# osqp/osqp-python

Hardware: AMD Instinct MI355X
Metric: ADMM iterations/sec, n=100000 m=200000 nnz(A)=1000000 sparse QP (indirect PCG) (higher is better)
Workload: dtype f64

## Files before the change

### include/osqp_hip.h

```cpp
#ifndef OSQP_HIP_H
#define OSQP_HIP_H

#ifdef __cplusplus
extern "C" {
#endif

typedef int    OSQPInt;
typedef double OSQPFloat;

#define OSQP_INFTY ((OSQPFloat)1e30)

enum osqp_linsys_solver_type { OSQP_UNKNOWN_SOLVER = 0, OSQP_DIRECT_SOLVER, OSQP_INDIRECT_SOLVER };

enum osqp_status_type {
  OSQP_SOLVED = 1, OSQP_SOLVED_INACCURATE, OSQP_PRIMAL_INFEASIBLE, OSQP_PRIMAL_INFEASIBLE_INACCURATE,
  OSQP_DUAL_INFEASIBLE, OSQP_DUAL_INFEASIBLE_INACCURATE, OSQP_MAX_ITER_REACHED, OSQP_TIME_LIMIT_REACHED,
  OSQP_NON_CVX, OSQP_SIGINT, OSQP_UNSOLVED
};

enum osqp_error_type {
  OSQP_NO_ERROR = 0, OSQP_DATA_VALIDATION_ERROR, OSQP_SETTINGS_VALIDATION_ERROR, OSQP_LINSYS_SOLVER_INIT_ERROR,
  OSQP_NONCVX_ERROR, OSQP_MEM_ALLOC_ERROR, OSQP_WORKSPACE_NOT_INIT_ERROR, OSQP_ALGEBRA_LOAD_ERROR,
  OSQP_CODEGEN_DEFINES_ERROR, OSQP_DATA_NOT_INITIALIZED, OSQP_FUNC_NOT_IMPLEMENTED
};

enum osqp_precond_type { OSQP_NO_PRECONDITIONER = 0, OSQP_DIAGONAL_PRECONDITIONER };

enum osqp_capabilities_type {
  OSQP_CAPABILITY_DIRECT_SOLVER = 0x01, OSQP_CAPABILITY_INDIRECT_SOLVER = 0x02, OSQP_CAPABILITY_CODEGEN = 0x04,
  OSQP_CAPABILITY_UPDATE_MATRICES = 0x08, OSQP_CAPABILITY_DERIVATIVES = 0x10
};

typedef struct {
  OSQPInt    m;
  OSQPInt    n;
  OSQPInt   *p;
  OSQPInt   *i;
  OSQPFloat *x;
  OSQPInt    nzmax;
  OSQPInt    nz;
} OSQPCscMatrix;

typedef struct {
  OSQPInt device;
  enum osqp_linsys_solver_type linsys_solver;
  OSQPInt verbose;
  OSQPInt warm_starting;
  OSQPInt scaling;
  OSQPInt polishing;
  OSQPFloat rho;
  OSQPInt   rho_is_vec;
  OSQPFloat sigma;
  OSQPFloat alpha;
  OSQPInt   cg_max_iter;
  OSQPInt   cg_tol_reduction;
  OSQPFloat cg_tol_fraction;
  enum osqp_precond_type cg_precond;
  OSQPInt   adaptive_rho;
  OSQPInt   adaptive_rho_interval;
  OSQPFloat adaptive_rho_fraction;
  OSQPFloat adaptive_rho_tolerance;
  OSQPInt   max_iter;
  OSQPFloat eps_abs;
  OSQPFloat eps_rel;
  OSQPFloat eps_prim_inf;
  OSQPFloat eps_dual_inf;
  OSQPInt   scaled_termination;
  OSQPInt   check_termination;
  OSQPInt   check_dualgap;
  OSQPFloat time_limit;
  OSQPFloat delta;
  OSQPInt   polish_refine_iter;
} OSQPSettings;

typedef struct {
  char      status[32];
  OSQPInt   status_val;
  OSQPInt   status_polish;
  OSQPFloat obj_val;
  OSQPFloat dual_obj_val;
  OSQPFloat prim_res;
  OSQPFloat dual_res;
  OSQPFloat duality_gap;
  OSQPInt   iter;
  OSQPInt   rho_updates;
  OSQPFloat rho_estimate;
  OSQPFloat setup_time;
  OSQPFloat solve_time;
  OSQPFloat update_time;
  OSQPFloat polish_time;
  OSQPFloat run_time;
  OSQPFloat primdual_int;
  OSQPFloat rel_kkt_error;
} OSQPInfo;

typedef struct {
  OSQPFloat *x;
  OSQPFloat *y;
  OSQPFloat *prim_inf_cert;
  OSQPFloat *dual_inf_cert;
} OSQPSolution;

typedef struct OSQPWorkspace_ OSQPWorkspace;

typedef struct {
  OSQPSettings  *settings;
  OSQPSolution  *solution;
  OSQPInfo      *info;
  OSQPWorkspace *work;
} OSQPSolver;

typedef struct {
  OSQPInt embedded_mode, float_type, printing_enable, profiling_enable, interrupt_enable, derivatives_enable;
} OSQPCodegenDefines;

OSQPInt osqp_capabilities(void);
void    osqp_set_default_settings(OSQPSettings *settings);
const char *osqp_version(void);

OSQPInt osqp_setup(OSQPSolver **solverp, const OSQPCscMatrix *P, const OSQPFloat *q, const OSQPCscMatrix *A,
                   const OSQPFloat *l, const OSQPFloat *u, OSQPInt m, OSQPInt n, const OSQPSettings *settings);
OSQPInt osqp_solve(OSQPSolver *solver);
OSQPInt osqp_cleanup(OSQPSolver *solver);
OSQPInt osqp_warm_start(OSQPSolver *solver, const OSQPFloat *x, const OSQPFloat *y);
OSQPInt osqp_cold_start(OSQPSolver *solver);
OSQPInt osqp_update_data_vec(OSQPSolver *solver, const OSQPFloat *q_new, const OSQPFloat *l_new,
                             const OSQPFloat *u_new);
OSQPInt osqp_update_data_mat(OSQPSolver *solver, const OSQPFloat *Px_new, const OSQPInt *Px_new_idx, OSQPInt P_new_n,
                             const OSQPFloat *Ax_new, const OSQPInt *Ax_new_idx, OSQPInt A_new_n);
OSQPInt osqp_update_settings(OSQPSolver *solver, const OSQPSettings *new_settings);
OSQPInt osqp_update_rho(OSQPSolver *solver, OSQPFloat rho_new);
void    osqp_get_dimensions(OSQPSolver *solver, OSQPInt *m, OSQPInt *n);

OSQPInt osqp_adjoint_derivative_compute(OSQPSolver *solver, OSQPFloat *dx, OSQPFloat *dy);
OSQPInt osqp_adjoint_derivative_get_mat(OSQPSolver *solver, OSQPCscMatrix *dP, OSQPCscMatrix *dA);
OSQPInt osqp_adjoint_derivative_get_vec(OSQPSolver *solver, OSQPFloat *dq, OSQPFloat *dl, OSQPFloat *du);
OSQPInt osqp_codegen(OSQPSolver *solver, const char *output_dir, const char *prefix, OSQPCodegenDefines *defines);
void    osqp_set_default_codegen_defines(OSQPCodegenDefines *defines);


typedef struct {
  double pcg_iters_total;
  double pcg_iters_max;
  double pcg_unconverged;
  double kernel_launches;
  double graph_launches;
  double gpu_solve_ms;
  double nnzA, nnzB;
  double pcg_fused;
  double batch_direct_bw;
  double cg_cap_escalations;
  double windowed_blocks;
  double row_blocks;
  double slot_topups;
  double f1_replicas;
  double woodbury_rows;
  double woodbury_direct;
  double preconditioner;
  double woodbury_factorisations, woodbury_factor_ms;
  double reordered;
  double reorder_ms;
  double woodbury_cache_hits;
  double f1_far_columns;
  double woodbury_dual_cols;
  double woodbury_fused_iteration;
  double woodbury_one_launch;
  double kform_nnz;
  double batch_wave_split;
} OSQPHipStats;
enum { OSQP_HIP_PRECOND_NONE = 0, OSQP_HIP_PRECOND_JACOBI = 1, OSQP_HIP_PRECOND_JACOBI_WOODBURY = 2, OSQP_HIP_PRECOND_JACOBI_WOODBURY_DENSE = 3 };
OSQPInt osqp_hip_get_stats(OSQPSolver *solver, OSQPHipStats *out);

OSQPInt osqp_hip_time_kernel(OSQPSolver *solver, OSQPInt which, OSQPInt reps, double *mean_ms);

#define OSQP_HIP_BATCH_REC 12
OSQPInt osqp_hip_batch_solve(OSQPSolver *solver, OSQPInt nbatch, const OSQPFloat *q, const OSQPFloat *l, const OSQPFloat *u,
                             OSQPFloat *x, OSQPFloat *y, OSQPFloat *rec, OSQPInt warm);
OSQPInt osqp_hip_batch_solve_device(OSQPSolver *solver, OSQPInt nbatch, const OSQPFloat *q_dev, const OSQPFloat *l_dev, const OSQPFloat *u_dev,
                                    OSQPFloat *x_dev, OSQPFloat *y_dev, OSQPFloat *rec_dev, OSQPInt warm_start, void *stream);

OSQPInt osqp_hip_batch_solve_mat(OSQPSolver *solver, OSQPInt nbatch, const OSQPFloat *Px, const OSQPFloat *Ax, const OSQPFloat *q, const OSQPFloat *l,
                                 const OSQPFloat *u, OSQPFloat *x, OSQPFloat *y, OSQPFloat *rec, OSQPInt warm);
OSQPInt osqp_hip_batch_solve_mat_device(OSQPSolver *solver, OSQPInt nbatch, const OSQPFloat *Px_dev, const OSQPFloat *Ax_dev, const OSQPFloat *q_dev,
                                        const OSQPFloat *l_dev, const OSQPFloat *u_dev, OSQPFloat *x_dev, OSQPFloat *y_dev, OSQPFloat *rec_dev,
                                        OSQPInt warm_start, void *stream);

#define OSQP_HIP_LOCKSTEP_WIDTH 64
#define OSQP_HIP_LOCKSTEP_LAST_REC 8
#define OSQP_HIP_LOCKSTEP_POLISH_LAST_REC 8
OSQPInt osqp_hip_batch_solve_lockstep(OSQPSolver *solver, OSQPInt nbatch, const OSQPFloat *q, const OSQPFloat *l, const OSQPFloat *u,
                                      OSQPFloat *x, OSQPFloat *y, OSQPFloat *rec, OSQPInt warm);
OSQPInt osqp_hip_batch_solve_lockstep_device(OSQPSolver *solver, OSQPInt nbatch, const OSQPFloat *q_dev, const OSQPFloat *l_dev, const OSQPFloat *u_dev,
                                             OSQPFloat *x_dev, OSQPFloat *y_dev, OSQPFloat *rec_dev, OSQPInt warm_start, void *stream);
OSQPInt osqp_hip_lockstep_last_record(OSQPSolver *solver, OSQPFloat *rec);
OSQPInt osqp_hip_lockstep_polish_last_record(OSQPSolver *solver, OSQPFloat *rec);
#define OSQP_HIP_LOCKSTEP_MAT_LAST_REC 8
OSQPInt osqp_hip_batch_solve_lockstep_mat(OSQPSolver *solver, OSQPInt nbatch, const OSQPFloat *Px, const OSQPFloat *Ax, const OSQPFloat *q, const OSQPFloat *l,
                                          const OSQPFloat *u, OSQPFloat *x, OSQPFloat *y, OSQPFloat *rec, OSQPInt warm);
OSQPInt osqp_hip_batch_solve_lockstep_mat_device(OSQPSolver *solver, OSQPInt nbatch, const OSQPFloat *Px_dev, const OSQPFloat *Ax_dev, const OSQPFloat *q_dev,
                                                 const OSQPFloat *l_dev, const OSQPFloat *u_dev, OSQPFloat *x_dev, OSQPFloat *y_dev, OSQPFloat *rec_dev,
                                                 OSQPInt warm_start, void *stream);
OSQPInt osqp_hip_lockstep_mat_last_record(OSQPSolver *solver, OSQPFloat *rec);
OSQPInt osqp_hip_lockstep_mat_scaling(OSQPSolver *solver, OSQPInt b, OSQPFloat *D, OSQPFloat *E, OSQPFloat *c);
#define OSQP_HIP_LOCKSTEP_DIRECT_LAST_REC 8
OSQPInt osqp_hip_batch_solve_lockstep_direct(OSQPSolver *solver, OSQPInt nbatch, const OSQPFloat *q, const OSQPFloat *l, const OSQPFloat *u,
                                             OSQPFloat *x, OSQPFloat *y, OSQPFloat *rec, OSQPInt warm);
OSQPInt osqp_hip_batch_solve_lockstep_direct_device(OSQPSolver *solver, OSQPInt nbatch, const OSQPFloat *q_dev, const OSQPFloat *l_dev, const OSQPFloat *u_dev,
                                                    OSQPFloat *x_dev, OSQPFloat *y_dev, OSQPFloat *rec_dev, OSQPInt warm_start, void *stream);
OSQPInt osqp_hip_lockstep_direct_last_record(OSQPSolver *solver, OSQPFloat *rec);
#define OSQP_HIP_LOCKSTEP_ADJOINT_LAST_REC 8
OSQPInt osqp_hip_batch_adjoint_lockstep(OSQPSolver *solver, OSQPInt nbatch, const OSQPFloat *l, const OSQPFloat *u, const OSQPFloat *x, const OSQPFloat *y,
                                        const OSQPFloat *dx, const OSQPFloat *dy, OSQPFloat *dP, OSQPFloat *dq, OSQPFloat *dA, OSQPFloat *dl, OSQPFloat *du,
                                        OSQPFloat *arec);
OSQPInt osqp_hip_batch_adjoint_lockstep_device(OSQPSolver *solver, OSQPInt nbatch, const OSQPFloat *l_dev, const OSQPFloat *u_dev, const OSQPFloat *x_dev,
                                               const OSQPFloat *y_dev, const OSQPFloat *dx_dev, const OSQPFloat *dy_dev, OSQPFloat *dP_dev, OSQPFloat *dq_dev,
                                               OSQPFloat *dA_dev, OSQPFloat *dl_dev, OSQPFloat *du_dev, OSQPFloat *arec_dev, void *stream);
OSQPInt osqp_hip_lockstep_adjoint_last_record(OSQPSolver *solver, OSQPFloat *rec);
#define OSQP_HIP_LOCKSTEP_DIRECT_ADJOINT_LAST_REC 8
OSQPInt osqp_hip_batch_adjoint_lockstep_direct(OSQPSolver *solver, OSQPInt nbatch, const OSQPFloat *l, const OSQPFloat *u, const OSQPFloat *x, const OSQPFloat *y,
                                               const OSQPFloat *dx, const OSQPFloat *dy, OSQPFloat *dP, OSQPFloat *dq, OSQPFloat *dA, OSQPFloat *dl, OSQPFloat *du,
                                               OSQPFloat *arec);
OSQPInt osqp_hip_batch_adjoint_lockstep_direct_device(OSQPSolver *solver, OSQPInt nbatch, const OSQPFloat *l_dev, const OSQPFloat *u_dev, const OSQPFloat *x_dev,
                                                      const OSQPFloat *y_dev, const OSQPFloat *dx_dev, const OSQPFloat *dy_dev, OSQPFloat *dP_dev, OSQPFloat *dq_dev,
                                                      OSQPFloat *dA_dev, OSQPFloat *dl_dev, OSQPFloat *du_dev, OSQPFloat *arec_dev, void *stream);
OSQPInt osqp_hip_lockstep_direct_adjoint_last_record(OSQPSolver *solver, OSQPFloat *rec);

#define OSQP_HIP_ADJOINT_REC 4
#define OSQP_HIP_ADJOINT_TOL 1e-6
OSQPInt osqp_hip_batch_adjoint(OSQPSolver *solver, OSQPInt nbatch, const OSQPFloat *Px, const OSQPFloat *Ax, const OSQPFloat *l, const OSQPFloat *u,
                               const OSQPFloat *x, const OSQPFloat *y, const OSQPFloat *dx, const OSQPFloat *dy, OSQPFloat *dP, OSQPFloat *dq,
                               OSQPFloat *dA, OSQPFloat *dl, OSQPFloat *du, OSQPFloat *arec);
OSQPInt osqp_hip_batch_adjoint_device(OSQPSolver *solver, OSQPInt nbatch, const OSQPFloat *Px_dev, const OSQPFloat *Ax_dev, const OSQPFloat *l_dev,
                                      const OSQPFloat *u_dev, const OSQPFloat *x_dev, const OSQPFloat *y_dev, const OSQPFloat *dx_dev,
                                      const OSQPFloat *dy_dev, OSQPFloat *dP_dev, OSQPFloat *dq_dev, OSQPFloat *dA_dev, OSQPFloat *dl_dev,
                                      OSQPFloat *du_dev, OSQPFloat *arec_dev, void *stream);
#define OSQP_HIP_ADJOINT_LAST_REC 8
OSQPInt osqp_hip_adjoint_compute_at(OSQPSolver *solver, const OSQPFloat *x, const OSQPFloat *y, const OSQPFloat *dx, const OSQPFloat *dy);
OSQPInt osqp_hip_adjoint_last_record(OSQPSolver *solver, OSQPFloat *rec);
OSQPInt osqp_hip_capabilities(void);

OSQPInt osqp_hip_update_data_vec_device(OSQPSolver *solver, const OSQPFloat *q_dev, const OSQPFloat *l_dev, const OSQPFloat *u_dev, void *stream);
OSQPInt osqp_hip_warm_start_device(OSQPSolver *solver, const OSQPFloat *x_dev, const OSQPFloat *y_dev, void *stream);


typedef struct OSQPHipLinSysSolver_ OSQPHipLinSysSolver;
struct OSQPHipLinSysSolver_ {
  enum osqp_linsys_solver_type type;
  const char *(*name)(OSQPHipLinSysSolver *self);
  OSQPInt (*solve)(OSQPHipLinSysSolver *self, OSQPFloat *b, OSQPInt admm_iter);
  void (*update_settings)(OSQPHipLinSysSolver *self, const OSQPSettings *settings);
  void (*warm_start)(OSQPHipLinSysSolver *self, const OSQPFloat *x);
  OSQPInt (*adjoint_derivative)(OSQPHipLinSysSolver *self);
  void (*free)(OSQPHipLinSysSolver *self);
  OSQPInt (*update_matrices)(OSQPHipLinSysSolver *self, const OSQPCscMatrix *P, const OSQPInt *Px_new_idx, OSQPInt P_new_n,
                             const OSQPCscMatrix *A, const OSQPInt *Ax_new_idx, OSQPInt A_new_n);
  OSQPInt (*update_rho_vec)(OSQPHipLinSysSolver *self, const OSQPFloat *rho_vec, OSQPFloat rho_sc);
  OSQPInt nthreads;
  OSQPInt pcg_iters;
  void *impl;
};
OSQPInt osqp_hip_linsys_init(OSQPHipLinSysSolver **self, const OSQPCscMatrix *P, const OSQPCscMatrix *A, const OSQPFloat *rho_vec,
                             const OSQPSettings *settings, const OSQPFloat *scaled_prim_res, const OSQPFloat *scaled_dual_res,
                             OSQPInt polishing);

typedef struct {
  OSQPInt graph;
  OSQPInt slots;
  OSQPInt pcg_fused;
  OSQPInt f1;
  OSQPInt window;
  OSQPInt woodbury;
  OSQPInt woodbury_direct;
  OSQPInt woodbury_large;
  OSQPInt device_driven;
  OSQPInt small_direct;
  OSQPInt batch_reorder;
  OSQPInt batch_variant;
  OSQPFloat extrap;
  OSQPFloat rho_eq_factor;
  OSQPInt rho_window;
  OSQPFloat rho_window_tol;
  OSQPInt rho_persist;
  OSQPFloat rho_tol_exp;
  OSQPFloat budget_tolerate, budget_sigma; OSQPInt budget_slack, budget_full;
  OSQPInt cg_escalate;
  OSQPInt stall;
  OSQPFloat polish_delta_floor;
  OSQPFloat polish_pcg_tol;
  OSQPInt slot_poll; OSQPInt poll_low; OSQPFloat poll_first, poll_frac, poll_wait;
  OSQPInt finish_pairs; OSQPInt poll_sleep_us;
  OSQPInt slot_log, setup_timing, batch_timing, woodbury_log;
  OSQPFloat woodbury_direct_tol;
  OSQPInt woodbury_fused;
  OSQPInt debug_fail_refactor;
  OSQPInt reorder;
  OSQPInt woodbury_cache;
  OSQPInt kform;
  OSQPInt woodbury_dual;
  OSQPInt woodbury_vendor;
  OSQPInt batch_wave;
} OSQPHipPolicy;
void    osqp_hip_default_policy(OSQPHipPolicy *policy);
OSQPInt osqp_hip_set_policy(OSQPSolver *solver, const OSQPHipPolicy *policy);
OSQPInt osqp_hip_get_policy(OSQPSolver *solver, OSQPHipPolicy *policy);
void    osqp_hip_set_default_policy(const OSQPHipPolicy *policy);

OSQPInt osqp_hip_trace_read(OSQPSolver *solver, unsigned long long *out, OSQPInt count);
OSQPInt osqp_hip_test_spmv(OSQPSolver *solver, OSQPInt which, const OSQPFloat *in, OSQPFloat *out);
typedef struct {
  OSQPInt op, M, N, K;
  OSQPFloat alpha, beta;
  long long as_i, as_k, bs_k, bs_j, cs_i, cs_j;
  long long a_off, b_off, c_off;
  long long a_len, b_len, c_len;
  const OSQPFloat *A, *B;
  OSQPFloat *C;
  OSQPFloat minpiv;
} OSQPHipDenseTest;
OSQPInt osqp_hip_test_dense(OSQPSolver *solver, OSQPHipDenseTest *t);
OSQPInt osqp_hip_set_rho_eq_factor(OSQPSolver *solver, OSQPFloat factor);
OSQPInt osqp_hip_get_scaling(OSQPSolver *solver, OSQPFloat *D, OSQPFloat *E, OSQPFloat *c);
OSQPInt osqp_hip_get_reordering(OSQPSolver *solver, OSQPInt *perm_cols, OSQPInt *perm_rows);
typedef void (*osqp_hip_print_fn)(const char *text, void *user);
void    osqp_hip_set_default_print(osqp_hip_print_fn fn, void *user);
OSQPInt osqp_hip_set_print(OSQPSolver *solver, osqp_hip_print_fn fn, void *user);
const char *osqp_hip_backend(void);

#ifdef __cplusplus
}
#endif
#endif
```

### osqp-python_amd/csrc/backend.h

```cpp
#pragma once
#include <cstddef>
#include <cstdint>
#include <stdexcept>

#include "band_ldl.h"

namespace osqp_hip {

struct DeviceError : std::runtime_error { using std::runtime_error::runtime_error; };

#ifndef OSQP_HIP_KBLOCK
#define OSQP_HIP_KBLOCK 256
#define OSQP_HIP_KGRID 1024
#endif
constexpr int kBlock = OSQP_HIP_KBLOCK;
constexpr int kGrid = OSQP_HIP_KGRID;
constexpr int kChunk = 8 * kBlock;
constexpr int kLongRow = 128;
constexpr int kMaxRowsPerBlock = 1024;
constexpr int kPartSlots = 40;
constexpr int kMaxCg = 1024;
constexpr int kWinCap = 1472;
constexpr int kF1Win = 512;
constexpr int kF1MaxD = 4;
// ... 256 lines not shown
  const double *x = nullptr, *y = nullptr, *dx = nullptr, *dy = nullptr;
  int *code = nullptr;
  double *rx = nullptr, *ry = nullptr;
  double *dP = nullptr, *dA = nullptr, *dl = nullptr, *du = nullptr;
  double *rec = nullptr;
  double c = 1.0, cinv = 1.0;
  int rho_is_vec = 1;
};

constexpr int kLsW = 64;
constexpr int kLsSlots = 32;
constexpr int kLsScal = 16, kLsInt = 12;
inline int lockstep_grid(int n, int m) { const int r = n > m ? n : m, g = (r + 15) / 16; return g < 1 ? 1 : (g > 256 ? 256 : g); }
inline size_t lockstep_ws_doubles(int n, int m) {
  return (size_t)kLsW * (8 * (size_t)n + 9 * (size_t)m + (size_t)kLsSlots * lockstep_grid(n, m) + (size_t)(m + 63) / 64 + 1 + kLsScal + kBatchRec + kLsInt) + 64;
}
struct LockstepParams : BatchSettings {
  int n = 0, m = 0, count = 0;
  DevCsr A, B;
  const double *D = nullptr, *Dinv = nullptr, *E = nullptr, *Einv = nullptr;
  double time_limit = 0;
  const double *q = nullptr, *l = nullptr, *u = nullptr;
  const double *q0 = nullptr, *l0 = nullptr, *u0 = nullptr;
  double *x = nullptr, *y = nullptr, *rec = nullptr;
  const int *pc = nullptr, *pr = nullptr;
  double *ws = nullptr;
  double pcg_rel = 0;
  double rho_tol_single = 0; int rho_persist = 0;
  int polish = 0, pol_min_steps = 1, pol_cg_max = 0;
  double pol_rho = 0, pol_pcg_rel = 0;
  double *pol_ws = nullptr, *pol_stat = nullptr;
  double *mat_ws = nullptr, *mat_stat = nullptr;
  const double *Px = nullptr, *Ax = nullptr;
  const int *pvmap = nullptr, *avmap = nullptr;
  int mat_iters = 0;
};
constexpr int kLsPolStat = 7;
constexpr int kLsMatStat = 2;
constexpr int kLsMatScalC = 11;
inline size_t lockstep_sc_offset(int n, int m) {
  const size_t tm = (size_t)(m + 63) / 64;
  return (size_t)kLsW * (8 * (size_t)n + 9 * (size_t)m + (size_t)kLsSlots * lockstep_grid(n, m) + (tm > 0 ? tm : 1));
}
inline size_t lockstep_mat_ws_doubles(int n, int m, int nzA, int nzB) { return (size_t)kLsW * ((size_t)nzA + (size_t)nzB + 2 * (size_t)n + 2 * (size_t)m) + 64; }
inline size_t lockstep_polish_ws_doubles(int n, int m) { return (size_t)kLsW * ((size_t)n + 4 * (size_t)m) + 64; }

struct LockstepAdjointParams : LockstepParams {
  int nzP = 0, nzA = 0;
  const int *Pi = nullptr, *Pj = nullptr, *Ai = nullptr, *Aj = nullptr;
  const int *Pmap = nullptr, *Amap = nullptr;
  const double *sx = nullptr, *sy = nullptr, *gx = nullptr, *gy = nullptr;
  double *dP = nullptr, *dq = nullptr, *dA = nullptr, *dl = nullptr, *du = nullptr, *arec = nullptr;
  int min_steps = 1, max_steps = 60; double gain = 0.9;
};
inline size_t lockstep_adjoint_ws_doubles(int n, int m) {
  return lockstep_ws_doubles(n, m) + (size_t)kLsW * (3 * (size_t)n + 3 * (size_t)m + ((size_t)m + 1) / 2) + 64;
}

struct LockstepDirectParams : LockstepParams {
  int r = 0;
  DevCsr Av;
  const double *WT = nullptr; const int *rows = nullptr; const unsigned char *islong = nullptr;
};
inline int lockstep_direct_colblock(int n) { const int t = (n + 63) / 64; return 64 * ((t + 127) / 128 > 0 ? (t + 127) / 128 : 1); }
inline size_t lockstep_direct_ws_doubles(int n, int m, int r) {
  const size_t gc = ((size_t)n + lockstep_direct_colblock(n) - 1) / lockstep_direct_colblock(n);
  return (size_t)kLsW * (3 * ((size_t)n + r) + 4 * (size_t)n + 9 * (size_t)m + (size_t)kLsSlots * lockstep_grid(n, m) + (size_t)(m + 63) / 64 + 1 + kLsScal + kBatchRec + kLsInt +
                         (size_t)r * r + 2 * gc * r + r + 1) + 64;
}

struct LockstepDirectAdjointParams : LockstepAdjointParams {
  int r = 0;
  DevCsr Av;
  const double *WT = nullptr; const int *rows = nullptr; const unsigned char *islong = nullptr;
};
inline size_t lockstep_direct_adjoint_ws_doubles(int n, int m, int r) {
  return lockstep_direct_ws_doubles(n, m, r) + (size_t)kLsW * (3 * (size_t)n + 3 * (size_t)m + ((size_t)m + 1) / 2) + 64;
}

namespace be {

int lockstep_direct_chunk(Dev &d, const LockstepDirectParams &p, void *stream, double *stat) __attribute__((weak));
int lockstep_direct_values(Dev &d, int nv, const int *src, double *out, void *stream) __attribute__((weak));
int lockstep_direct_adjoint_chunk(Dev &d, const LockstepDirectAdjointParams &p, void *stream, double *stat) __attribute__((weak));

int lockstep_chunk(Dev &d, const LockstepParams &p, void *stream, double *stat) __attribute__((weak));
int lockstep_adjoint_chunk(Dev &d, const LockstepAdjointParams &p, void *stream, double *stat) __attribute__((weak));

void adjoint_load(Dev &d, const AdjointPcg &a) __attribute__((weak));
void adjoint_residual(Dev &d, const AdjointPcg &a) __attribute__((weak));
void adjoint_gradients(Dev &d, const AdjointPcg &a) __attribute__((weak));

int batch_adjoint(Dev &d, const AdjointParams &p, void *stream) __attribute__((weak));
size_t batch_lds_bytes(int n, int m);
int batch_solve(Dev &d, const BatchParams &p, void *stream = nullptr);
size_t batch_direct_lds_bytes(int n, int m, int nnz, int bw);
bool batch_direct_selected(const BatchParams &p);
void batch_release(Dev &d);
size_t batch_wave_lds_bytes(int n, int m, int steps);
void batch_products(Dev &d, int nprod, const int *a, const int *b, double *out);
int batch_prepare(Dev &d, const BatchParams &p, const double *Px_b, const double *Ax_b, int scaling_iters, void *stream);
void batch_order(Dev &d, int nbatch, const int *iters, int *order, void *stream);

const char *name();
int init(Dev &d, int device);
void destroy(Dev &d);
void *alloc(Dev &d, size_t bytes);
void dfree(Dev &d, void *p);
void h2d(Dev &d, void *dst, const void *src, size_t bytes);
void d2h(Dev &d, void *dst, const void *src, size_t bytes);
void zero(Dev &d, void *dst, size_t bytes);
void sync(Dev &d);
void ev_mark(Dev &d, int which);
double ev_ms(Dev &d);
void activate(Dev &d);
void ext_record(Dev &d, void *stream);
void ext_wait(Dev &d);

void kb_rhs(Dev &d);
void k1(Dev &d, int i);
void k2(Dev &d, int i);
void kv(Dev &d, int i);
void ka(Dev &d, int budget);
bool slots_supported(const Dev &d);
void slot_begin(Dev &d, int target, int cap);
void slot_pair(Dev &d);
int slot_done(Dev &d);
int slot_seq(Dev &d);
inline double slot_launches(const Dev &d, double pcg) { return (d.wb.on && d.wb.exact && d.wb.x.on && d.wb.x.slots) ? 2.16 : (d.f1.on ? pcg + 2.0 : (d.kf.on ? pcg + 3.0 : 2.0 * (pcg + 2.0))); }
bool kf_supported();
void kf_values(Dev &d, int cond = 0);
void f1_refresh(Dev &d);
bool wb_supported();
bool wbx_supported();
void wbx_init(Dev &d);
void wbx_refresh(Dev &d);
void wbx_factor(Dev &d, int cond = 0);
void wbx_slot_pair(Dev &d);
inline bool wbx_active(const Dev &d) { return d.wb.on && d.wb.exact && d.wb.x.on; }
inline bool wbx_slots(const Dev &d) { return wbx_active(d) && d.wb.x.slots; }
void wbx_chunk(Dev &d, int niter);
bool wb_large_supported();
void wb_refresh(Dev &d);
void wb_direct(Dev &d);
inline bool wbf_active(const Dev &d) { return d.wb.on && d.wb.exact && d.wb.dual && d.wb.fused; }
void wbf_iteration(Dev &d);
void wb_apply(Dev &d, int parity, int direct = 0);
bool ctl_supported(const Dev &d);
void ctl_upload(Dev &d, const Ctl &c);
void ctl_begin(Dev &d);
void ctl_group(Dev &d, int diagonal);
void ctl_poll(Dev &d, Ctl *out, int *seq, int *done);
void ctl_download(Dev &d, Ctl *out);
constexpr int kSlotInts = 24;
void slot_poll(Dev &d, int *seq, int *done);

void residuals(Dev &d);
void infeas_primal(Dev &d);
void infeas_dual(Dev &d, double thr, int unscaled);
void fetch_res(Dev &d, double *host_res);
void fetch_flags(Dev &d, int *host_flags);
void fetch_res_flags(Dev &d, double *host_res, int *host_flags);

void set_rho(Dev &d, double rho_bar);
void precond(Dev &d, int diagonal);
void set_pcg_tol(Dev &d, double tol_rel, double tol_abs);

void init_iterates(Dev &d, int full);

void project_normalcone(Dev &d);

bool pcg_fused(const Dev &d);

bool graphs_supported();
void graph_begin(Dev &d);
void *graph_end(Dev &d);
void graph_launch(Dev &d, void *g);
void graph_free(Dev &d, void *g);

bool device_assembly();
void assemble(Dev &d, int scaled, double c, int with_sigma);
double ruiz(Dev &d, int iters);

bool device_vec_updates();
void copy_in(Dev &d, void *dst, const void *src, size_t bytes, int src_on_device);
void stream_wait(Dev &d, void *caller_stream);
void gather(Dev &d, double *dst_dev, const double *src_dev, const int *idx_dev, int cnt);
void scale_q(Dev &d, double c);
void scale_bounds(Dev &d, int rho_is_vec);
int count_bad_bounds(Dev &d, const double *l_dev, const double *u_dev);
void scale_warm(Dev &d, const double *x_dev, const double *y_dev, double c);

bool ktrace_read(Dev &d, unsigned long long *out, int count);
void test_spmv(Dev &d, int which, const double *in_dev, double *out_dev);
struct DenseProbe { int op, M, N, K; double alpha, beta; long as_i, as_k, bs_k, bs_j, cs_i, cs_j; const double *A, *B; double *C; };
double test_dense(Dev &d, const DenseProbe &p) __attribute__((weak));
float time_kernel(Dev &d, int which, int reps);

}
}
```

### osqp-python_amd/csrc/backend_hip.hip

```cpp
#include "hip_common.h"

namespace osqp_hip {
namespace be {

namespace {

struct EKr1 : NoPrefetch {
  const double *z, *y, *dy, *l, *u, *E, *Einv;
  double pu = 0, au = 0, zu = 0, ps = 0, as = 0, zs = 0, du = 0, ds = 0, lhs = 0, sup = 0;
  __device__ __forceinline__ void operator()(int i, const double (&s)[1]) {
    const double ax = s[0], zi = z[i], pr = ax - zi, ei = Einv[i], dyi = dy[i], yi = y[i], li = l[i], ui = u[i];
    pu = nanmax(pu, fabs(ei * pr)); au = nanmax(au, fabs(ei * ax)); zu = nanmax(zu, fabs(ei * zi));
    ps = nanmax(ps, fabs(pr)); as = nanmax(as, fabs(ax)); zs = nanmax(zs, fabs(zi));
    du = nanmax(du, fabs(E[i] * dyi)); ds = nanmax(ds, fabs(dyi));
    lhs += support_term(li, ui, dyi);
    sup += support_finite(li, ui, yi);
  }
};
__device__ __forceinline__ bool ctl_res_due(const Dev &d) { return d.ctl->chunk_done && d.ctl->ch_at_check && d.ctl->status == CTL_RUNNING; }
__global__ __launch_bounds__(kBlock) void k_res_m(Dev d, int cond) {
  __shared__ StreamLdsW<1, double> lds;
  if (cond && !ctl_res_due(d)) return;
  GVec g{d.x};
  EKr1 e{{}, d.z, d.y, d.dy, d.l, d.u, d.E, d.Einv};
  process_rows<1>(d.A, g, e, lds);
  __syncthreads();
  double *red = lds.red;
  put_partial(d.part, SL_RES0 + R_PRI_U, block_max(e.pu, red)); put_partial(d.part, SL_RES0 + R_AX_U, block_max(e.au, red));
  put_partial(d.part, SL_RES0 + R_Z_U, block_max(e.zu, red)); put_partial(d.part, SL_RES0 + R_PRI_S, block_max(e.ps, red));
  put_partial(d.part, SL_RES0 + R_AX_S, block_max(e.as, red)); put_partial(d.part, SL_RES0 + R_Z_S, block_max(e.zs, red));
  put_partial(d.part, SL_RES0 + R_DY_U, block_max(e.du, red)); put_partial(d.part, SL_RES0 + R_DY_S, block_max(e.ds, red));
  put_partial(d.part, SL_RES0 + R_PINF_LHS, block_sum(e.lhs, red)); put_partial(d.part, SL_RES0 + R_SUPP, block_sum(e.sup, red));
}

struct GTwo {
  const double *pn, *pm; int n;
  __device__ __forceinline__ void operator()(int c, double a, double (&pr)[2]) const {
    if (c < n) { pr[0] = a * pn[c]; pr[1] = 0.0; } else { pr[0] = 0.0; pr[1] = a * pm[c - n]; }
  }
};
struct EKr2 : NoPrefetch {
  const double *x, *q, *dx, *D, *Dinv; double sigma;
  double du = 0, pu = 0, au = 0, ds = 0, ps = 0, as = 0, xu = 0, xs = 0, xpx = 0, qx = 0, qdx = 0, qns = 0, qnu = 0;
  __device__ __forceinline__ void operator()(int j, const double (&s)[2]) {
    const double xj = x[j], px = s[0] - sigma * xj, aty = s[1], qj = q[j], dr = px + qj + aty, di = Dinv[j], dxj = dx[j];
    qns = nanmax(qns, fabs(qj)); qnu = nanmax(qnu, fabs(di * qj));
    du = nanmax(du, fabs(di * dr)); pu = nanmax(pu, fabs(di * px)); au = nanmax(au, fabs(di * aty));
    ds = nanmax(ds, fabs(dr)); ps = nanmax(ps, fabs(px)); as = nanmax(as, fabs(aty));
    xu = nanmax(xu, fabs(D[j] * dxj)); xs = nanmax(xs, fabs(dxj));
    xpx += xj * px; qx += qj * xj; qdx += qj * dxj;
  }
};
__global__ __launch_bounds__(kBlock) void k_res_n(Dev d, int cond) {
  __shared__ StreamLds<2> lds;
  if (cond && !ctl_res_due(d)) return;
  GTwo g{d.x, d.y, d.n};
  EKr2 e{{}, d.x, d.q, d.dx, d.D, d.Dinv, d.sigma};
  process_rows<2>(d.B, g, e, lds);
  __syncthreads();
  double *red = lds.red;
  put_partial(d.part, SL_RES0 + R_DUA_U, block_max(e.du, red)); put_partial(d.part, SL_RES0 + R_PX_U, block_max(e.pu, red));
  put_partial(d.part, SL_RES0 + R_ATY_U, block_max(e.au, red)); put_partial(d.part, SL_RES0 + R_DUA_S, block_max(e.ds, red));
  put_partial(d.part, SL_RES0 + R_PX_S, block_max(e.ps, red)); put_partial(d.part, SL_RES0 + R_ATY_S, block_max(e.as, red));
  put_partial(d.part, SL_RES0 + R_DX_U, block_max(e.xu, red)); put_partial(d.part, SL_RES0 + R_DX_S, block_max(e.xs, red));
  put_partial(d.part, SL_RES0 + R_XPX, block_sum(e.xpx, red)); put_partial(d.part, SL_RES0 + R_QX, block_sum(e.qx, red));
  put_partial(d.part, SL_RES0 + R_QDX, block_sum(e.qdx, red));
  put_partial(d.part, SL_RES0 + R_QN_S, block_max(e.qns, red)); put_partial(d.part, SL_RES0 + R_QN_U, block_max(e.qnu, red));
}

__device__ __forceinline__ bool res_is_sum(int q) {
  return q == R_PINF_LHS || q == R_SUPP || q == R_XPX || q == R_QX || q == R_QDX || q == R_ADX_VIOL;
}
__device__ __forceinline__ bool ctl_stage2_due(const Dev &d, int bits) { return d.ctl->status == CTL_RUNNING && (d.ctl->stage2 & bits) != 0; }
__global__ __launch_bounds__(kBlock) void k_res_final(Dev d, int q0, int cond) {
  __shared__ double sred[2 * kWaves];
  if (cond == 1 && !ctl_res_due(d)) return;
  if (cond == 2 && !ctl_stage2_due(d, NEED_PINF | NEED_DINF)) return;
  const int q = q0 + blockIdx.x;
  const double *slot = d.part + (SL_RES0 + q) * kGrid;
  const double v = res_is_sum(q) ? partial_sum(slot, sred) : partial_max(slot, sred);
  if (threadIdx.x == 0) d.res[q] = v;
}

struct GAtOnly { const double *pm; int n; __device__ __forceinline__ void operator()(int c, double a, double (&pr)[1]) const { pr[0] = c >= n ? a * pm[c - n] : 0.0; } };
struct GPOnly { const double *pn; int n; __device__ __forceinline__ void operator()(int c, double a, double (&pr)[1]) const { pr[0] = c < n ? a * pn[c] : 0.0; } };
struct EAbs2 : NoPrefetch {
  const double *scale, *sub; double sigma; double mu = 0, ms = 0;
  __device__ __forceinline__ void operator()(int j, const double (&s)[1]) {
    const double v = s[0] - (sub ? sigma * sub[j] : 0.0);
    mu = nanmax(mu, fabs(scale[j] * v)); ms = nanmax(ms, fabs(v));
  }
};
__global__ __launch_bounds__(kBlock) void k_inf_primal(Dev d, int cond) {
  __shared__ StreamLds<1> lds;
  if (cond && !ctl_stage2_due(d, NEED_PINF)) return;
  GAtOnly g{d.dy, d.n};
  EAbs2 e{{}, d.Dinv, nullptr, 0.0};
  process_rows<1>(d.B, g, e, lds);
  __syncthreads();
  put_partial(d.part, SL_RES0 + R_ATDY_U, block_max(e.mu, lds.red)); put_partial(d.part, SL_RES0 + R_ATDY_S, block_max(e.ms, lds.red));
}
__global__ __launch_bounds__(kBlock) void k_inf_dual_p(Dev d, int cond) {
  __shared__ StreamLds<1> lds;
  if (cond && !ctl_stage2_due(d, NEED_DINF)) return;
  GPOnly g{d.dx, d.n};
  EAbs2 e{{}, d.Dinv, d.dx, d.sigma};
  process_rows<1>(d.B, g, e, lds);
  __syncthreads();
  put_partial(d.part, SL_RES0 + R_PDX_U, block_max(e.mu, lds.red)); put_partial(d.part, SL_RES0 + R_PDX_S, block_max(e.ms, lds.red));
}
struct EViol : NoPrefetch {
  const double *l, *u, *Einv; double thr; int unscaled; double viol = 0;
  __device__ __forceinline__ void operator()(int i, const double (&s)[1]) {
    const double a = unscaled ? Einv[i] * s[0] : s[0];
    if (adx_violates(a, l[i], u[i], thr)) viol += 1.0;
  }
};
__global__ __launch_bounds__(kBlock) void k_inf_dual_a(Dev d, double thr, int unscaled, int cond) {
  __shared__ StreamLdsW<1, double> lds;
  if (cond) { if (!ctl_stage2_due(d, NEED_DINF)) return; thr = d.ctl->inf_thr_d; unscaled = d.ctl->inf_unscaled; }
  GVec g{d.dx};
  EViol e{{}, d.l, d.u, d.Einv, thr, unscaled};
  process_rows<1>(d.A, g, e, lds);
  __syncthreads();
  put_partial(d.part, SL_RES0 + R_ADX_VIOL, block_sum(e.viol, lds.red));
}

__global__ __launch_bounds__(kBlock) void k_set_rho(Dev d, double rho_bar, int cond) {
  if (cond) { if (!d.ctl->rho_flag) return; rho_bar = d.ctl->rho_bar; }
  const int stride = gridDim.x * kBlock;
  for (int i = blockIdx.x * kBlock + threadIdx.x; i < d.m; i += stride) {
    const int t = d.ctype[i];
    const double eqf = d.eq_from_cnt ? eq_weight(d.cnt[0] == 0, d.rho_eq_mixed) : d.rho_eq_factor;
    const double r = row_rho(t, rho_bar, eqf * rho_bar);
    d.rho[i] = r; d.rho_inv[i] = 1.0 / r;
    d.v[i] = r * d.z[i] - d.y[i]; d.ztg[i] = d.zt[i]; d.t0[i] = r * d.zt[i];
  }
}
struct GPrec { const double *rho; int n; __device__ __forceinline__ void operator()(int c, double a, double (&pr)[1]) const { pr[0] = c >= n ? rho[c - n] * a * a : 0.0; } };
__global__ __launch_bounds__(kBlock) void k_precond(Dev d, int cond) {
  __shared__ StreamLds<1> lds;
  if (cond && !d.ctl->rho_flag) return;
  GPrec g{d.rho, d.n};
  EPrec e{{}, d.B.val, d.Bdiag, d.Minv};
  process_rows<1>(d.B, g, e, lds);
}
__global__ __launch_bounds__(kBlock) void k_fill(double *p, int n, double v) {
  const int stride = gridDim.x * kBlock;
  for (int i = blockIdx.x * kBlock + threadIdx.x; i < n; i += stride) p[i] = v;
}
__global__ __launch_bounds__(kBlock) void k_init_n(Dev d) {
  const int stride = gridDim.x * kBlock;
  for (int j = blockIdx.x * kBlock + threadIdx.x; j < d.n; j += stride) { d.xs[j] = d.x[j]; d.dx[j] = 0.0; }
// ... 13 lines not shown
};
__global__ __launch_bounds__(kBlock) void k_init_m(Dev d, int full) {
  __shared__ StreamLdsW<1, double> lds;
  GVec g{d.xs};
  EInit e{{}, d.rho, d.y, d.z, d.zt, d.t0, d.v, d.dy, full, d.ztg};
  process_rows<1>(d.A, g, e, lds);
}
__global__ __launch_bounds__(kBlock) void k_normalcone(Dev d) {
  const int stride = gridDim.x * kBlock;
  for (int i = blockIdx.x * kBlock + threadIdx.x; i < d.m; i += stride) {
    const ConeRow c = normal_cone(d.z[i] + d.y[i], d.l[i], d.u[i]);
    d.z[i] = c.z; d.y[i] = c.y;
  }
}
__global__ void k_set_scal(double *scal, double rel, double ab) { scal[S_TOL_REL] = rel; scal[S_TOL_ABS] = ab; }
__global__ __launch_bounds__(kBlock) void k_scale_q(Dev d, double c) {
  for (int j = blockIdx.x * kBlock + threadIdx.x; j < d.n; j += gridDim.x * kBlock) d.q[j] = c * d.D[j] * d.qraw[j];
}
__global__ __launch_bounds__(kBlock) void k_scale_bounds(Dev d, int rho_is_vec) {
  int ineq = 0;
  for (int i = blockIdx.x * kBlock + threadIdx.x; i < d.m; i += gridDim.x * kBlock) {
    const double ls = d.E[i] * d.lraw[i], us = d.E[i] * d.uraw[i];
    d.l[i] = ls; d.u[i] = us;
    const int t = row_class(ls, us, rho_is_vec);
    d.ctype[i] = t;
    ineq += (t == 0);
  }
  for (int o = 32; o > 0; o >>= 1) ineq += __shfl_down(ineq, o, 64);
  if ((threadIdx.x & 63) == 0 && ineq) atomicAdd(&d.cnt[0], ineq);
}
__global__ __launch_bounds__(kBlock) void k_count_bad(int m, const double *l, const double *u, int *cnt) {
  int bad = 0;
  for (int i = blockIdx.x * kBlock + threadIdx.x; i < m; i += gridDim.x * kBlock) bad += !(l[i] <= u[i]);
  for (int o = 32; o > 0; o >>= 1) bad += __shfl_down(bad, o, 64);
  if ((threadIdx.x & 63) == 0 && bad) atomicAdd(&cnt[1], bad);
}
__global__ __launch_bounds__(kBlock) void k_gather(double *dst, const double *src, const int *idx, int cnt) {
  for (int k = blockIdx.x * kBlock + threadIdx.x; k < cnt; k += gridDim.x * kBlock) dst[k] = src[idx[k]];
}
__global__ __launch_bounds__(kBlock) void k_scale_warm(Dev d, const double *xin, const double *yin, double c) {
  const int stride = gridDim.x * kBlock;
  if (xin) for (int j = blockIdx.x * kBlock + threadIdx.x; j < d.n; j += stride) d.x[j] = d.Dinv[j] * xin[j];
  if (yin) for (int i = blockIdx.x * kBlock + threadIdx.x; i < d.m; i += stride) d.y[i] = c * d.Einv[i] * yin[i];
}



__device__ __forceinline__ double limit_scaling_dev(double v) { return v < 1e-4 ? 1.0 : (v > 1e4 ? 1e4 : v); }
__global__ __launch_bounds__(kBlock) void k_asm_diag(Dev d, double sigma) {
  for (int j = blockIdx.x * kBlock + threadIdx.x; j < d.n; j += gridDim.x * kBlock) d.B.val[d.Bdiag[j]] = sigma;
}
__global__ __launch_bounds__(kBlock) void k_asm_scatter(Dev d, int scaled, double c, double sigma) {
  const int stride = gridDim.x * kBlock;
  for (int k = blockIdx.x * kBlock + threadIdx.x; k < d.nzA; k += stride) {
    double v = d.Araw[k];
    if (scaled) v *= d.E[d.Ai[k]] * d.D[d.Aj[k]];
    d.A.val[d.AmA[k]] = v; d.B.val[d.AmB[k]] = v;
  }
  for (int k = blockIdx.x * kBlock + threadIdx.x; k < d.nzP; k += stride) {
    const int i = d.Pi[k], j = d.Pj[k];
    double v = d.Praw[k];
    if (scaled) v *= c * d.D[i] * d.D[j];
    if (i == j) atomicAdd(&d.B.val[d.Pm1[k]], v);
    else { d.B.val[d.Pm1[k]] = v; d.B.val[d.Pm2[k]] = v; }
  }
}
template <class F>
__device__ __forceinline__ void for_long_rows(const DevCsr &M, F &&f) {
  const int4 *desc = reinterpret_cast<const int4 *>(M.blkdesc);
  for (int b = blockIdx.x; b < M.nblk; b += gridDim.x) { const int4 ds = desc[b]; if (ds.y < 0) f(ds.x, ds.z, ds.w); }
}
__global__ __launch_bounds__(kBlock) void k_rowmax(DevCsr M, int climit, double *out) {
  __shared__ double sred[2 * kWaves];
  for (int r = blockIdx.x * kBlock + threadIdx.x; r < M.nrows; r += gridDim.x * kBlock) {
    const int k0 = M.rowptr[r], k1 = M.rowptr[r + 1];
    if (k1 - k0 > kLongRow) continue;
    double mx = 0.0;
    for (int k = k0; k < k1; k++) if (M.col[k] < climit) mx = fmax(mx, fabs(M.val[k]));
    out[r] = mx;
  }
  for_long_rows(M, [&](int r, int k0, int k1) {
    double mx = 0.0;
    for (int k = k0 + threadIdx.x; k < k1; k += kBlock) if (M.col[k] < climit) mx = fmax(mx, fabs(M.val[k]));
    mx = block_max(mx, sred);
    if (threadIdx.x == 0) out[r] = mx;
  });
}
__global__ __launch_bounds__(kBlock) void k_ruiz_delta(double *v, int cnt) {
  for (int i = blockIdx.x * kBlock + threadIdx.x; i < cnt; i += gridDim.x * kBlock) v[i] = 1.0 / sqrt(limit_scaling_dev(v[i]));
}
__global__ __launch_bounds__(kBlock) void k_ruiz_scale_A(Dev d, const double *dt, const double *et) {
  for (int i = blockIdx.x * kBlock + threadIdx.x; i < d.m; i += gridDim.x * kBlock) {
    const double ei = et[i];
    const int k0 = d.A.rowptr[i], k1 = d.A.rowptr[i + 1];
    if (k1 - k0 <= kLongRow) for (int k = k0; k < k1; k++) d.A.val[k] *= ei * dt[d.A.col[k]];
    d.E[i] *= ei;
  }
  for_long_rows(d.A, [&](int i, int k0, int k1) {
    const double ei = et[i];
    for (int k = k0 + threadIdx.x; k < k1; k += kBlock) d.A.val[k] *= ei * dt[d.A.col[k]];
  });
}
__global__ __launch_bounds__(kBlock) void k_ruiz_scale_B(Dev d, const double *dt, const double *et) {
  for (int j = blockIdx.x * kBlock + threadIdx.x; j < d.n; j += gridDim.x * kBlock) {
    const double dj = dt[j];
    const int k0 = d.B.rowptr[j], k1 = d.B.rowptr[j + 1];
    if (k1 - k0 <= kLongRow)
      for (int k = k0; k < k1; k++) {
        const int c = d.B.col[k];
        d.B.val[k] *= c < d.n ? dt[c] * dj : et[c - d.n] * dj;
      }
    d.q[j] *= dj; d.D[j] *= dj;
  }
  for_long_rows(d.B, [&](int j, int k0, int k1) {
    const double dj = dt[j];
    for (int k = k0 + threadIdx.x; k < k1; k += kBlock) { const int c = d.B.col[k]; d.B.val[k] *= c < d.n ? dt[c] * dj : et[c - d.n] * dj; }
  });
}
__global__ __launch_bounds__(kBlock) void k_ruiz_cost(Dev d, const double *np) {
  __shared__ double sred[2 * kWaves];
  double sum = 0.0, nq = 0.0;
  for (int j = threadIdx.x; j < d.n; j += kBlock) { sum += np[j]; nq = fmax(nq, fabs(d.q[j])); }
  block_sum_max(sum, nq, sred);
  if (threadIdx.x == 0) {
    const double mean = sum / (double)(d.n > 0 ? d.n : 1);
    const double ct = 1.0 / limit_scaling_dev(fmax(limit_scaling_dev(nq), mean));
    d.cs[1] = ct; d.cs[0] *= ct;
  }
}
__global__ __launch_bounds__(kBlock) void k_ruiz_cost_apply(Dev d) {
  const double ct = d.cs[1];
  for (int j = blockIdx.x * kBlock + threadIdx.x; j < d.n; j += gridDim.x * kBlock) {
    for (int k = d.B.rowptr[j]; k < d.B.rowptr[j + 1] && d.B.col[k] < d.n; k++) d.B.val[k] *= ct;
    d.q[j] *= ct;
  }
}
__global__ __launch_bounds__(kBlock) void k_ruiz_finish(Dev d, double sigma) {
  const int stride = gridDim.x * kBlock;
  for (int j = blockIdx.x * kBlock + threadIdx.x; j < d.n; j += stride) { d.Dinv[j] = 1.0 / d.D[j]; d.B.val[d.Bdiag[j]] += sigma; }
  for (int i = blockIdx.x * kBlock + threadIdx.x; i < d.m; i += stride) d.Einv[i] = 1.0 / d.E[i];
}

__device__ __forceinline__ void ctl_begin_chunk(const Dev &d, const Ctl &c, int seq) {
  int *r = d.slot;
  r[SR_PHASE] = P_KB; r[SR_K] = 0; r[SR_ADMM] = 0; r[SR_TARGET] = c.ch_next - c.iter; r[SR_USED] = 0; r[SR_CONV] = 0;
  r[SR_CAP] = c.budget[c.ch_tight]; r[SR_SEQ] = seq;
  r[SR_WORDS + SR_SEQ] = seq - 1; r[SR_WORDS + SR_ADMM] = 0;
  d.scal[S_TOL_REL] = c.tol_rel; d.scal[S_TOL_ABS] = ctl_chunk_tol_abs(c);
  for (int q = F_STAT_SUM; q < F_COUNT; q++) d.flags[q] = 0;
}
__global__ void k_ctl_begin(Dev d, int epoch) {
  Ctl &c = *d.ctl;
  c.chunk_done = 0; c.rho_flag = 0; c.stage2 = 0; c.status = CTL_RUNNING; c.seq_begin = 0;
  ctl_begin_chunk(d, c, 0);
  d.slot[2 * SR_WORDS] = epoch;
}
__global__ __launch_bounds__(64) void k_decide(Dev d, int stage) {
  __shared__ Ctl c;
  __shared__ double res[R_COUNT];
  __shared__ int fl[F_COUNT];
  Ctl *g = d.ctl;
  if (g->status != CTL_RUNNING) return;
  if (stage == 1 ? !g->chunk_done : !g->stage2) {
    if (stage == 1 && threadIdx.x == 0) g->rho_flag = 0;
    return;
  }
  static_assert(sizeof(Ctl) % sizeof(int) == 0, "Ctl is copied word by word");
  constexpr int W = sizeof(Ctl) / sizeof(int);
  const int *gi = reinterpret_cast<const int *>(g);
  int *ci = reinterpret_cast<int *>(&c);
  for (int i = threadIdx.x; i < W; i += 64) ci[i] = gi[i];
  for (int i = threadIdx.x; i < R_COUNT; i += 64) res[i] = d.res[i];
  for (int i = threadIdx.x; i < F_COUNT; i += 64) fl[i] = d.flags[i];
  __syncthreads();
  if (threadIdx.x == 0) {
    int st;
    if (stage == 1) {
      c.chunk_done = 0;
      if (c.boundaries >= 0 && c.boundaries < kCtlHist) c.hist[c.boundaries] = c.seq_end - c.seq_begin;
      for (int q = 0; q < F_COUNT; q++) c.last_flags[q] = fl[q];
      st = ctl_boundary(c, res, fl);
    } else st = ctl_boundary_stage2(c, res, c.last_flags);
    c.status = st;
    if (st == CTL_RUNNING && !c.stage2) { c.seq_begin = d.slot[SR_SEQ]; ctl_begin_chunk(d, c, d.slot[SR_SEQ]); }
  }
  __syncthreads();
  int *go = reinterpret_cast<int *>(g);
  for (int i = threadIdx.x; i < W; i += 64) go[i] = ci[i];
}


}

const char *name() { return "hip-gfx950"; }

int init(Dev &d, int device) {
  int count = 0;
  if (hipGetDeviceCount(&count) != hipSuccess || count <= 0) {
    std::fprintf(stderr, "osqp_hip: no HIP device available -- this engine has no CPU fallback\n");
    return OSQP_ALGEBRA_LOAD_ERROR;
  }
  if (device >= count) return OSQP_SETTINGS_VALIDATION_ERROR;
  d.device = device;
  HIP_CHECK(hipSetDevice(device));
  hipStream_t s;
  HIP_CHECK(hipStreamCreateWithFlags(&s, hipStreamNonBlocking));
  d.stream = s;
  Impl *p = new Impl();
  HIP_CHECK(hipEventCreate(&p->ev0)); HIP_CHECK(hipEventCreate(&p->ev1)); HIP_CHECK(hipEventCreate(&p->ev_s0)); HIP_CHECK(hipEventCreate(&p->ev_s1)); HIP_CHECK(hipEventCreateWithFlags(&p->ev_ext, hipEventDisableTiming)); HIP_CHECK(hipEventCreateWithFlags(&p->ev_wait, hipEventDisableTiming));
  HIP_CHECK(hipHostMalloc(reinterpret_cast<void **>(&p->pin_res), sizeof(double) * R_COUNT, hipHostMallocDefault));
  HIP_CHECK(hipHostMalloc(reinterpret_cast<void **>(&p->pin_flags), sizeof(int) * (F_COUNT + 16), hipHostMallocDefault));
  HIP_CHECK(hipHostMalloc(reinterpret_cast<void **>(&p->pin_poll), sizeof(int) * kSlotInts, hipHostMallocDefault));
  HIP_CHECK(hipStreamCreateWithFlags(&p->side, hipStreamNonBlocking));
  HIP_CHECK(hipHostMalloc(reinterpret_cast<void **>(&p->pin_ctl), sizeof(Ctl), hipHostMallocDefault));
  HIP_CHECK(hipHostMalloc(reinterpret_cast<void **>(&p->pin_ctl2), sizeof(Ctl), hipHostMallocDefault));
  d.impl = p;
  return OSQP_NO_ERROR;
}
void destroy(Dev &d) {
  if (!d.impl) return;
  (void)hipSetDevice(d.device);
  Impl &p = im(d);
  (void)hipEventDestroy(p.ev0); (void)hipEventDestroy(p.ev1); (void)hipEventDestroy(p.ev_s0); (void)hipEventDestroy(p.ev_s1); (void)hipEventDestroy(p.ev_ext); (void)hipEventDestroy(p.ev_wait); (void)hipHostFree(p.pin_res); (void)hipHostFree(p.pin_flags);
  (void)hipHostFree(p.pin_poll); if (p.side) (void)hipStreamDestroy(p.side);
  (void)hipHostFree(p.pin_ctl); (void)hipHostFree(p.pin_ctl2);
  if (p.blas) wb_release_blas(p.blas);
  batch_release(d);
  for (int k = 1; k < DevWb::kCache; k++) if (d.wb.cache_buf[k]) { (void)hipFree(d.wb.cache_buf[k]); d.wb.cache_buf[k] = nullptr; }
  dev_release(d);
  delete &p; d.impl = nullptr;
  if (d.stream) { (void)hipStreamDestroy(st(d)); d.stream = nullptr; }
}
void *alloc(Dev &d, size_t bytes) {
  HIP_CHECK(hipSetDevice(d.device));
  void *p = nullptr;
  HIP_CHECK(hipMalloc(&p, bytes));
  HIP_CHECK(hipMemsetAsync(p, 0, bytes, st(d)));
  return p;
}
void dfree(Dev &d, void *p) { (void)hipSetDevice(d.device); (void)hipFree(p); }
void h2d(Dev &d, void *dst, const void *src, size_t b) {
  if (!b) return;
  HIP_CHECK(hipSetDevice(d.device));
  HIP_CHECK(hipMemcpyAsync(dst, src, b, hipMemcpyHostToDevice, st(d)));
  HIP_CHECK(hipStreamSynchronize(st(d)));
}
void d2h(Dev &d, void *dst, const void *src, size_t b) {
  if (!b) return;
  HIP_CHECK(hipSetDevice(d.device));
  HIP_CHECK(hipMemcpyAsync(dst, src, b, hipMemcpyDeviceToHost, st(d)));
  HIP_CHECK(hipStreamSynchronize(st(d)));
}
void zero(Dev &d, void *dst, size_t b) { if (!b) return; HIP_CHECK(hipSetDevice(d.device)); HIP_CHECK(hipMemsetAsync(dst, 0, b, st(d))); }
void sync(Dev &d) { HIP_CHECK(hipSetDevice(d.device)); HIP_CHECK(hipStreamSynchronize(st(d))); }
void ev_mark(Dev &d, int which) { HIP_CHECK(hipSetDevice(d.device)); Impl &p = im(d); HIP_CHECK(hipEventRecord(which ? p.ev_s1 : p.ev_s0, st(d))); }
double ev_ms(Dev &d) { Impl &p = im(d); float ms = 0.f; HIP_CHECK(hipEventSynchronize(p.ev_s1)); HIP_CHECK(hipEventElapsedTime(&ms, p.ev_s0, p.ev_s1)); return (double)ms; }
void activate(Dev &d) { HIP_CHECK(hipSetDevice(d.device)); }
void ext_record(Dev &d, void *stream) {
  if (!stream || !d.impl) return;
  HIP_CHECK(hipSetDevice(d.device));
  HIP_CHECK(hipEventRecord(im(d).ev_ext, static_cast<hipStream_t>(stream)));
  im(d).ext_pending = true;
}
void ext_wait(Dev &d) {
  if (!d.impl || !im(d).ext_pending) return;
  HIP_CHECK(hipSetDevice(d.device));
  HIP_CHECK(hipEventSynchronize(im(d).ev_ext));
  im(d).ext_pending = false;
}

bool ctl_supported(const Dev &d) { return d.ctl != nullptr && d.slot != nullptr; }
void ctl_upload(Dev &d, const Ctl &c) {
  HIP_CHECK(hipSetDevice(d.device));
  Impl &p = im(d);
  std::memcpy(p.pin_ctl, &c, sizeof(Ctl));
  HIP_CHECK(hipMemcpyAsync(d.ctl, p.pin_ctl, sizeof(Ctl), hipMemcpyHostToDevice, st(d)));
  HIP_CHECK(hipStreamSynchronize(st(d)));
}
void ctl_begin(Dev &d) { HIP_CHECK(hipSetDevice(d.device)); dev_publish(d); hipLaunchKernelGGL(k_ctl_begin, dim3(1), dim3(1), 0, st(d), d, ++im(d).epoch); }
void ctl_group(Dev &d, int diagonal) {
  LAUNCH(k_res_m, d, d, 1);
  LAUNCH(k_res_n, d, d, 1);
  hipLaunchKernelGGL(k_res_final, dim3(R_QN_U + 1), dim3(kBlock), 0, st(d), d, 0, 1);
  hipLaunchKernelGGL(k_decide, dim3(1), dim3(64), 0, st(d), d, 1);
  LAUNCH(k_inf_primal, d, d, 1);
  LAUNCH(k_inf_dual_p, d, d, 1);
  LAUNCH(k_inf_dual_a, d, d, 0.0, 0, 1);
  hipLaunchKernelGGL(k_res_final, dim3(5), dim3(kBlock), 0, st(d), d, (int)R_ATDY_U, 2);
  hipLaunchKernelGGL(k_decide, dim3(1), dim3(64), 0, st(d), d, 2);
  LAUNCH(k_set_rho, d, d, 0.0, 1);
  LAUNCH(k_init_guess, d, d, 1);
  if (diagonal) LAUNCH(k_precond, d, d, 1);
  kf_values(d, 1);
  if (wbx_slots(d)) wb_factor_device(d, 1);
}
void ctl_poll(Dev &d, Ctl *out, int *seq, int *done) {
  HIP_CHECK(hipSetDevice(d.device));
  Impl &p = im(d);
  HIP_CHECK(hipMemcpyAsync(p.pin_poll, d.slot, sizeof(int) * kSlotInts, hipMemcpyDeviceToHost, p.side));
  HIP_CHECK(hipMemcpyAsync(p.pin_ctl2, d.ctl, sizeof(Ctl), hipMemcpyDeviceToHost, p.side));
  HIP_CHECK(hipStreamSynchronize(p.side));
  std::memcpy(out, p.pin_ctl2, sizeof(Ctl));
  if (p.pin_poll[2 * SR_WORDS] != p.epoch) { *seq = 0; *done = 0; out->status = CTL_RUNNING; return; }
  const int *ra = p.pin_poll, *rb = p.pin_poll + SR_WORDS;
  const int *nw = ra[SR_SEQ] >= rb[SR_SEQ] ? ra : rb;
  *seq = nw[SR_SEQ]; *done = nw[SR_ADMM];
}
void ctl_download(Dev &d, Ctl *out) {
  HIP_CHECK(hipSetDevice(d.device));
  Impl &p = im(d);
  HIP_CHECK(hipMemcpyAsync(p.pin_ctl2, d.ctl, sizeof(Ctl), hipMemcpyDeviceToHost, st(d)));
  HIP_CHECK(hipStreamSynchronize(st(d)));
  std::memcpy(out, p.pin_ctl2, sizeof(Ctl));
}

void residuals(Dev &d) {
  HIP_CHECK(hipSetDevice(d.device));
  LAUNCH(k_res_m, d, d, 0);
  LAUNCH(k_res_n, d, d, 0);
  hipLaunchKernelGGL(k_res_final, dim3(R_QN_U + 1), dim3(kBlock), 0, st(d), d, 0, 0);
}
void infeas_primal(Dev &d) {
  HIP_CHECK(hipSetDevice(d.device));
  LAUNCH(k_inf_primal, d, d, 0);
  hipLaunchKernelGGL(k_res_final, dim3(2), dim3(kBlock), 0, st(d), d, (int)R_ATDY_U, 0);
}
void infeas_dual(Dev &d, double thr, int unscaled) {
  HIP_CHECK(hipSetDevice(d.device));
  LAUNCH(k_inf_dual_p, d, d, 0);
  LAUNCH(k_inf_dual_a, d, d, thr, unscaled, 0);
  hipLaunchKernelGGL(k_res_final, dim3(3), dim3(kBlock), 0, st(d), d, (int)R_PDX_U, 0);
}
void fetch_res(Dev &d, double *h) {
  HIP_CHECK(hipSetDevice(d.device));
  HIP_CHECK(hipMemcpyAsync(im(d).pin_res, d.res, sizeof(double) * R_COUNT, hipMemcpyDeviceToHost, st(d)));
  HIP_CHECK(hipStreamSynchronize(st(d)));
  std::memcpy(h, im(d).pin_res, sizeof(double) * R_COUNT);
}
void fetch_flags(Dev &d, int *h) {
  HIP_CHECK(hipSetDevice(d.device));
  HIP_CHECK(hipMemcpyAsync(im(d).pin_flags, d.flags, sizeof(int) * F_COUNT, hipMemcpyDeviceToHost, st(d)));
  if (d.slot) HIP_CHECK(hipMemcpyAsync(im(d).pin_flags + F_COUNT, d.slot, sizeof(int) * 16, hipMemcpyDeviceToHost, st(d)));
  HIP_CHECK(hipMemsetAsync(d.flags + F_STAT_SUM, 0, sizeof(int) * (F_COUNT - F_STAT_SUM), st(d)));
  HIP_CHECK(hipStreamSynchronize(st(d)));
  std::memcpy(h, im(d).pin_flags, sizeof(int) * F_COUNT);
}
void fetch_res_flags(Dev &d, double *hr, int *hf) {
  HIP_CHECK(hipSetDevice(d.device));
  HIP_CHECK(hipMemcpyAsync(im(d).pin_res, d.res, sizeof(double) * R_COUNT, hipMemcpyDeviceToHost, st(d)));
  HIP_CHECK(hipMemcpyAsync(im(d).pin_flags, d.flags, sizeof(int) * F_COUNT, hipMemcpyDeviceToHost, st(d)));
  if (d.slot) HIP_CHECK(hipMemcpyAsync(im(d).pin_flags + F_COUNT, d.slot, sizeof(int) * 16, hipMemcpyDeviceToHost, st(d)));
  HIP_CHECK(hipMemsetAsync(d.flags + F_STAT_SUM, 0, sizeof(int) * (F_COUNT - F_STAT_SUM), st(d)));
  HIP_CHECK(hipStreamSynchronize(st(d)));
  std::memcpy(hr, im(d).pin_res, sizeof(double) * R_COUNT);
  std::memcpy(hf, im(d).pin_flags, sizeof(int) * F_COUNT);
}

void set_rho(Dev &d, double rho_bar) { HIP_CHECK(hipSetDevice(d.device)); d.wb.rho_key = rho_bar; LAUNCH(k_set_rho, d, d, rho_bar, 0); LAUNCH(k_init_guess, d, d, 0); }
void precond(Dev &d, int diagonal) {
  HIP_CHECK(hipSetDevice(d.device));
  if (diagonal) LAUNCH(k_precond, d, d, 0);
  else LAUNCH(k_fill, d, d.Minv, d.n, 1.0);
  kf_values(d, 0);
  if (d.wb.on) wb_factor(d);
}
void set_pcg_tol(Dev &d, double rel, double ab) {
  HIP_CHECK(hipSetDevice(d.device));
  hipLaunchKernelGGL(k_set_scal, dim3(1), dim3(1), 0, st(d), d.scal, rel, ab);
}
void init_iterates(Dev &d, int full) {
  HIP_CHECK(hipSetDevice(d.device));
  if (full) LAUNCH(k_init_n, d, d);
  LAUNCH(k_init_guess, d, d, 0);
  LAUNCH(k_init_m, d, d, full == 1 ? 1 : 0);
}

bool device_vec_updates() { return true; }
void copy_in(Dev &d, void *dst, const void *src, size_t bytes, int src_on_device) {
  if (!bytes) return;
  HIP_CHECK(hipSetDevice(d.device));
  HIP_CHECK(hipMemcpyAsync(dst, src, bytes, src_on_device ? hipMemcpyDeviceToDevice : hipMemcpyHostToDevice, st(d)));
  if (!src_on_device) HIP_CHECK(hipStreamSynchronize(st(d)));
}
void stream_wait(Dev &d, void *caller_stream) {
  if (!caller_stream || caller_stream == d.stream) return;
  HIP_CHECK(hipSetDevice(d.device));
  HIP_CHECK(hipEventRecord(im(d).ev_wait, static_cast<hipStream_t>(caller_stream)));
  HIP_CHECK(hipStreamWaitEvent(st(d), im(d).ev_wait, 0));
}
void gather(Dev &d, double *dst, const double *src, const int *idx, int cnt) { if (cnt <= 0) return; HIP_CHECK(hipSetDevice(d.device)); LAUNCH(k_gather, d, dst, src, idx, cnt); }
void scale_q(Dev &d, double c) { HIP_CHECK(hipSetDevice(d.device)); LAUNCH(k_scale_q, d, d, c); }
void scale_bounds(Dev &d, int rho_is_vec) {
  HIP_CHECK(hipSetDevice(d.device));
  HIP_CHECK(hipMemsetAsync(d.cnt, 0, sizeof(int), st(d)));
  if (d.m > 0) LAUNCH(k_scale_bounds, d, d, rho_is_vec);
}
int count_bad_bounds(Dev &d, const double *l, const double *u) {
  if (d.m == 0) return 0;
  HIP_CHECK(hipSetDevice(d.device));
  HIP_CHECK(hipMemsetAsync(d.cnt + 1, 0, sizeof(int), st(d)));
  LAUNCH(k_count_bad, d, d.m, l, u, d.cnt);
  int bad = 0;
  HIP_CHECK(hipMemcpyAsync(&bad, d.cnt + 1, sizeof(int), hipMemcpyDeviceToHost, st(d)));
  HIP_CHECK(hipStreamSynchronize(st(d)));
  return bad;
}
void scale_warm(Dev &d, const double *x, const double *y, double c) { HIP_CHECK(hipSetDevice(d.device)); LAUNCH(k_scale_warm, d, d, x, y, c); }

void project_normalcone(Dev &d) { HIP_CHECK(hipSetDevice(d.device)); LAUNCH(k_normalcone, d, d); }


bool device_assembly() { return true; }
void assemble(Dev &d, int scaled, double c, int with_sigma) {
  HIP_CHECK(hipSetDevice(d.device));
  const double sg = with_sigma ? d.sigma : 0.0;
  LAUNCH(k_asm_diag, d, d, sg);
  LAUNCH(k_asm_scatter, d, d, scaled, c, sg);
}
double ruiz(Dev &d, int iters) {
  HIP_CHECK(hipSetDevice(d.device));
  const double one[2] = {1.0, 1.0};
  HIP_CHECK(hipMemcpyAsync(d.cs, one, sizeof(one), hipMemcpyHostToDevice, st(d)));
  LAUNCH(k_fill, d, d.D, d.n, 1.0);
  if (d.m > 0) LAUNCH(k_fill, d, d.E, d.m, 1.0);
  double *dt = d.w, *np = d.p, *et = d.t;
  for (int it = 0; it < iters; it++) {
    LAUNCH(k_rowmax, d, d.B, d.n + d.m, dt);
    LAUNCH(k_ruiz_delta, d, dt, d.n);
    if (d.m > 0) { LAUNCH(k_rowmax, d, d.A, d.n, et); LAUNCH(k_ruiz_delta, d, et, d.m); LAUNCH(k_ruiz_scale_A, d, d, dt, et); }
    LAUNCH(k_ruiz_scale_B, d, d, dt, et);
    LAUNCH(k_rowmax, d, d.B, d.n, np);
    hipLaunchKernelGGL(k_ruiz_cost, dim3(1), dim3(kBlock), 0, st(d), d, np);
    LAUNCH(k_ruiz_cost_apply, d, d);
  }
  LAUNCH(k_ruiz_finish, d, d, d.sigma);
  double cs[2];
  HIP_CHECK(hipMemcpyAsync(cs, d.cs, sizeof(cs), hipMemcpyDeviceToHost, st(d)));
  HIP_CHECK(hipStreamSynchronize(st(d)));
  return cs[0];
}

bool graphs_supported() { return true; }
void graph_begin(Dev &d) { HIP_CHECK(hipSetDevice(d.device)); HIP_CHECK(hipStreamBeginCapture(st(d), hipStreamCaptureModeThreadLocal)); }
void *graph_end(Dev &d) {
  hipGraph_t g = nullptr; hipGraphExec_t ex = nullptr;
  HIP_CHECK(hipStreamEndCapture(st(d), &g));
  HIP_CHECK(hipGraphInstantiate(&ex, g, nullptr, nullptr, 0));
  HIP_CHECK(hipGraphDestroy(g));
  return ex;
}
void graph_launch(Dev &d, void *g) { HIP_CHECK(hipSetDevice(d.device)); HIP_CHECK(hipGraphLaunch(static_cast<hipGraphExec_t>(g), st(d))); }
void graph_free(Dev &d, void *g) { if (g) { (void)hipSetDevice(d.device); (void)hipGraphExecDestroy(static_cast<hipGraphExec_t>(g)); } }

void test_spmv(Dev &d, int which, const double *in, double *out) {
  HIP_CHECK(hipSetDevice(d.device));
  LAUNCH(k_test_spmv, d, which == 0 ? d.A : d.B, in, out);
}


}
}
```

### osqp-python_amd/csrc/engine.cpp

```cpp


#include "engine_internal.hpp"

#include <atomic>
#include <cstdarg>

namespace osqp_hip {

const BatchEnv &batch_env() {
  static const BatchEnv e = [] {
    auto num = [](const char *name, int dflt) { const char *v = std::getenv(name); return v ? std::atoi(v) : dflt; };
    return BatchEnv{num("OSQP_HIP_WAVE_SPLIT", -1), num("OSQP_HIP_WAVE_CUS", -1), num("OSQP_HIP_BATCH_WIDE_ROUNDS", 1 << 20)};
  }();
  return e;
}
namespace {
thread_local OSQPHipPolicy g_default_policy;
thread_local bool g_default_policy_set = false;

void policy_from_env(OSQPHipPolicy &p, bool runtime_only) {
  if (!runtime_only) { if (g_default_policy_set) p = g_default_policy; else Engine::default_policy(&p); }
  auto on = [](const char *name, OSQPInt &v) { if (const char *e = std::getenv(name)) v = e[0] != '0'; };
  auto num = [](const char *name, OSQPInt &v) { if (const char *e = std::getenv(name)) v = std::atoi(e); };
  auto real = [](const char *name, OSQPFloat &v) { if (const char *e = std::getenv(name)) v = std::atof(e); };
  on("OSQP_HIP_SMALL_DIRECT", p.small_direct); num("OSQP_HIP_DEVICE_DRIVEN", p.device_driven); on("OSQP_HIP_BATCH_REORDER", p.batch_reorder);
  num("OSQP_HIP_BATCH_WAVE", p.batch_wave);
  num("OSQP_HIP_RHO_WINDOW", p.rho_window); real("OSQP_HIP_RHO_WINDOW_TOL", p.rho_window_tol); on("OSQP_HIP_RHO_PERSIST", p.rho_persist);
  if (const char *e = std::getenv("OSQP_HIP_RHO_TOL_EXP")) { const double v = std::atof(e); p.rho_tol_exp = v > 0 && v <= 1 ? v : 0.5; }
  real("OSQP_HIP_BUDGET_TOLERATE", p.budget_tolerate); real("OSQP_HIP_BUDGET_SIGMA", p.budget_sigma); num("OSQP_HIP_BUDGET_SLACK", p.budget_slack);
  if (std::getenv("OSQP_HIP_BUDGET_FULL")) p.budget_full = 1;
  on("OSQP_HIP_CG_ESCALATE", p.cg_escalate); on("OSQP_HIP_STALL", p.stall);
  real("OSQP_HIP_POLISH_DELTA_FLOOR", p.polish_delta_floor); real("OSQP_HIP_POLISH_PCG_TOL", p.polish_pcg_tol);
  on("OSQP_HIP_SLOT_POLL", p.slot_poll); num("OSQP_HIP_POLL_LOW", p.poll_low); real("OSQP_HIP_POLL_FIRST", p.poll_first);
  real("OSQP_HIP_POLL_FRAC", p.poll_frac); real("OSQP_HIP_POLL_WAIT", p.poll_wait);
  num("OSQP_HIP_FINISH_PAIRS", p.finish_pairs); num("OSQP_HIP_POLL_SLEEP_US", p.poll_sleep_us);
  if (std::getenv("OSQP_HIP_SLOT_LOG")) p.slot_log = 1;
  if (std::getenv("OSQP_HIP_BATCH_TIMING")) p.batch_timing = 1;
  if (std::getenv("OSQP_HIP_WB_LOG")) p.woodbury_log = 1;
  if (const char *e = std::getenv("OSQP_HIP_BATCH_VARIANT")) {
    static const char *names[] = {"", "direct", "direct256", "w64", "w256", "generic"};
    p.batch_variant = 0;
    for (int k = 1; k <= 5; k++) if (!std::strcmp(e, names[k])) p.batch_variant = k;
  }
  if (runtime_only) return;
  num("OSQP_HIP_WOODBURY_FUSED", p.woodbury_fused); real("OSQP_HIP_WOODBURY_DIRECT_TOL", p.woodbury_direct_tol);
  on("OSQP_HIP_WOODBURY", p.woodbury); on("OSQP_HIP_WOODBURY_DIRECT", p.woodbury_direct); on("OSQP_HIP_WOODBURY_LARGE", p.woodbury_large);
  num("OSQP_HIP_REORDER", p.reorder); on("OSQP_HIP_WOODBURY_CACHE", p.woodbury_cache); on("OSQP_HIP_KFORM", p.kform); on("OSQP_HIP_WOODBURY_DUAL", p.woodbury_dual); on("OSQP_HIP_WOODBURY_VENDOR", p.woodbury_vendor);
  on("OSQP_HIP_GRAPH", p.graph); on("OSQP_HIP_SLOTS", p.slots); on("OSQP_HIP_PCG_FUSED", p.pcg_fused); num("OSQP_HIP_F1", p.f1); on("OSQP_HIP_WINDOW", p.window);
  real("OSQP_HIP_EXTRAP", p.extrap);
  if (const char *e = std::getenv("OSQP_HIP_RHO_EQ_FACTOR")) { const double v = std::atof(e); if (v >= 1.0) p.rho_eq_factor = v; }
  if (std::getenv("OSQP_HIP_SETUP_TIMING")) p.setup_timing = 1;
}
}

void Engine::default_policy(OSQPHipPolicy *p) {
  if (!p) return;
  *p = OSQPHipPolicy();
  p->graph = p->slots = p->pcg_fused = p->f1 = p->window = p->device_driven = p->small_direct = p->batch_reorder = 1; p->batch_variant = 0;
  p->extrap = 0.9; p->rho_eq_factor = 0.0;
  p->rho_window = 10; p->rho_window_tol = 0.1; p->rho_persist = 1; p->rho_tol_exp = 0.5;
  p->budget_tolerate = 0.0; p->budget_sigma = 3.0; p->budget_slack = 0; p->budget_full = 0; p->cg_escalate = 1; p->stall = 1;
  p->polish_delta_floor = 1e-3; p->polish_pcg_tol = 1e-15; p->woodbury = 1; p->woodbury_direct = 1; p->woodbury_large = 1; p->woodbury_cache = 1;
  p->slot_poll = 1; p->poll_low = 6; p->poll_first = 0.8; p->poll_frac = 0.75; p->poll_wait = 0.7;
  p->finish_pairs = 12; p->poll_sleep_us = 30;
  p->reorder = 1; p->kform = 0; p->woodbury_dual = 1; p->woodbury_vendor = 0; p->woodbury_fused = 1; p->woodbury_direct_tol = 1e-6; p->debug_fail_refactor = 0; p->batch_wave = 0;
}
void Engine::set_default_policy(const OSQPHipPolicy *p) {
  g_default_policy_set = p != nullptr;
  if (p) g_default_policy = *p;
}
int Engine::get_policy(OSQPHipPolicy *p) const { if (!p) return OSQP_DATA_VALIDATION_ERROR; *p = pol_; return OSQP_NO_ERROR; }
int Engine::set_policy(const OSQPHipPolicy *p) {
  if (!p) return OSQP_DATA_VALIDATION_ERROR;
  if (!(p->extrap >= 0 && p->extrap <= 2) || p->rho_window < 0 || !(p->rho_window_tol > 0) || !(p->rho_tol_exp > 0 && p->rho_tol_exp <= 1) ||
      !(p->budget_sigma >= 0) || p->finish_pairs < 1 || p->batch_variant < 0 || p->batch_variant > 5 || p->batch_wave < -1 || p->batch_wave > 1 ||
      !(p->rho_eq_factor == 0 || p->rho_eq_factor >= 1) || p->reorder < 0 || p->reorder > 2 || !(p->woodbury_direct_tol > 0 && p->woodbury_direct_tol < 1) || !(p->polish_delta_floor > 0) || !(p->polish_pcg_tol > 0 && p->polish_pcg_tol < 1))
    return OSQP_SETTINGS_VALIDATION_ERROR;
  const OSQPHipPolicy old = pol_;
  pol_ = *p; pol_explicit_ = true;
  pol_.slots = old.slots; pol_.pcg_fused = old.pcg_fused; pol_.f1 = old.f1; pol_.window = old.window; pol_.woodbury = old.woodbury; pol_.woodbury_direct = old.woodbury_direct; pol_.woodbury_large = old.woodbury_large; pol_.reorder = old.reorder; pol_.woodbury_cache = old.woodbury_cache; pol_.woodbury_fused = old.woodbury_fused; pol_.woodbury_direct_tol = old.woodbury_direct_tol; pol_.kform = old.kform; pol_.woodbury_dual = old.woodbury_dual; pol_.woodbury_vendor = old.woodbury_vendor;
  if (pol_.graph != old.graph) { use_graph_ = pol_.graph != 0; if (dev_ready_) { be::activate(d_); be::sync(d_); drop_graphs(); } }
  if (dev_ready_) d_.theta = pol_.extrap;
  if (dev_ready_ && d_.wb.dbg && pol_.debug_fail_refactor != old.debug_fail_refactor) { be::activate(d_); const int v = pol_.debug_fail_refactor; be::h2d(d_, d_.wb.dbg, &v, sizeof(int)); }
  if (dev_ready_ && pol_.rho_eq_factor >= 1.0 && pol_.rho_eq_factor != old.rho_eq_factor) return set_rho_eq_factor(pol_.rho_eq_factor);
  return OSQP_NO_ERROR;
}

namespace {
std::atomic<osqp_hip_print_fn> g_print_fn{nullptr};
std::atomic<void *> g_print_user{nullptr};
}
void Engine::set_default_print(osqp_hip_print_fn fn, void *user) { g_print_user.store(user); g_print_fn.store(fn); }
void Engine::say(const char *fmt, ...) const {
  char buf[1024];
  va_list ap;
  va_start(ap, fmt);
  std::vsnprintf(buf, sizeof(buf), fmt, ap);
  va_end(ap);
  if (print_fn_) print_fn_(buf, print_user_);
  else { std::fputs(buf, stdout); std::fflush(stdout); }
}
void Engine::print_summary_line(int iter, double obj, double pri, double dua, double rho, double t0) const {
  say("%4d  %11.4e   %8.2e   %8.2e   %8.2e  %8.2es\n", iter, obj, pri, dua, rho, (first_run_ ? info.setup_time : info.update_time) + (now_s() - t0));
}
void Engine::print_log(const Ctl &c, double t0) {
  if (!settings.verbose) return;
  if (c.nlog - log_printed_ > kCtlLog) log_printed_ = c.nlog - kCtlLog;
  for (; log_printed_ < c.nlog; log_printed_++) {
    const double *e = c.log[log_printed_ % kCtlLog];
    print_summary_line((int)e[0], e[1], e[2], e[3], e[4], t0);
  }
}

Engine::Engine() {
  print_fn_ = g_print_fn.load(); print_user_ = g_print_user.load();
  pub.settings = &settings; pub.solution = &solution; pub.info = &info; pub.work = reinterpret_cast<OSQPWorkspace *>(this);
  policy_from_env(pol_, false);
  use_graph_ = pol_.graph != 0; use_slots_ = pol_.slots != 0;
  if (pol_.rho_eq_factor >= 1.0) { eq_factor_mixed_ = pol_.rho_eq_factor; eq_factor_env_ = true; }
}
Engine::~Engine() { free_all(); }

void Engine::drop_graphs() {
  for (auto &kv : graphs_) be::graph_free(d_, kv.second);
  graphs_.clear();
  for (auto &kv : sgraphs_) be::graph_free(d_, kv.second);
  sgraphs_.clear();
}

void Engine::sync_graph_scalars() {
  const double sig[7] = {d_.theta, d_.alpha, d_.sigma, d_.rho_eq_factor, d_.rho_eq_mixed, (double)d_.eq_from_cnt, (double)reinterpret_cast<uintptr_t>(d_.wb.Sinv)};
  if (std::memcmp(sig, graph_sig_, sizeof(sig)) == 0) return;
  if (!graphs_.empty() || !sgraphs_.empty()) { be::sync(d_); drop_graphs(); }
  std::memcpy(graph_sig_, sig, sizeof(sig));
}

void Engine::free_all() {
  if (!dev_ready_) return;
  try { be::activate(d_); be::ext_wait(d_); be::sync(d_); } catch (const DeviceError &) {}
  drop_graphs();
  if (bbuf_) { be::dfree(d_, bbuf_); bbuf_ = nullptr; bbuf_cap_ = 0; }
  if (bmat_) { be::dfree(d_, bmat_); bmat_ = nullptr; bmat_cap_ = 0; }
  if (abuf_) { be::dfree(d_, abuf_); abuf_ = nullptr; abuf_cap_ = 0; }
  if (adjw_) { be::dfree(d_, adjw_); adjw_ = nullptr; adjw_cap_ = 0; }
  adj_ok_ = false;
  if (d_batch_order_) { be::dfree(d_, d_batch_order_); d_batch_order_ = nullptr; batch_order_cap_ = 0; }
  if (d_batch_iters_) { be::dfree(d_, d_batch_iters_); d_batch_iters_ = nullptr; d_batch_iters_n_ = 0; }
  batch_order_.clear();
  if (ckpt_) { be::dfree(d_, ckpt_); ckpt_ = nullptr; }
  if (lsw_) { be::dfree(d_, lsw_); lsw_ = nullptr; }
  if (lspw_) { be::dfree(d_, lspw_); lspw_ = nullptr; }
  if (lsmw_) { be::dfree(d_, lsmw_); lsmw_ = nullptr; }
  lsm_last_count_ = 0; std::fill(lsm_rec_, lsm_rec_ + OSQP_HIP_LOCKSTEP_MAT_LAST_REC, 0.0);
  if (lsaw_) { be::dfree(d_, lsaw_); lsaw_ = nullptr; }
  if (lsdw_) { be::dfree(d_, lsdw_); lsdw_ = nullptr; }
  if (lsdaw_) { be::dfree(d_, lsdaw_); lsdaw_ = nullptr; }
  if (lsdabuf_) { be::dfree(d_, lsdabuf_); lsdabuf_ = nullptr; lsdabuf_cap_ = 0; }
  if (lsd_vval_) { be::dfree(d_, lsd_vval_); lsd_vval_ = nullptr; }
  if (lsd_vrp_) { be::dfree(d_, lsd_vrp_); be::dfree(d_, lsd_vcol_); be::dfree(d_, lsd_vsrc_); lsd_vrp_ = lsd_vcol_ = lsd_vsrc_ = nullptr; lsd_nv_ = 0; }
  wb_k0diag_ = false;
  if (lsabuf_) { be::dfree(d_, lsabuf_); lsabuf_ = nullptr; lsabuf_cap_ = 0; }
  if (d_pvmap_) { be::dfree(d_, d_pvmap_); d_pvmap_ = nullptr; }
  if (d_avmap_) { be::dfree(d_, d_avmap_); d_avmap_ = nullptr; }
  free_batch_direct(); free_batch_spectral(); free_batch_wave();
  if (d_.f1.va) {
    d_.Minv = d_.xs = d_.p = d_.r = d_.s = d_.rho = d_.f1.pval = nullptr; d_.f1.pcol = d_.f1.prp = nullptr; d_.f1.cptr = nullptr;
  }
  if (d_.wb.cache_buf[0]) d_.wb.Sinv = d_.wb.cache_buf[0];
  void *ptrs[] = {d_.A.rowptr, d_.A.col, d_.A.blkdesc, d_.A.val, d_.B.rowptr, d_.B.col, d_.B.blkdesc, d_.B.val, d_.Bdiag, d_.A.runinfo, d_.B.runinfo, d_.A.blkwin, d_.B.blkwin, d_.A.lcol, d_.B.lcol, d_.qraw, d_.lraw, d_.uraw, d_.cnt,
                  d_.q, d_.l, d_.u, d_.D, d_.Dinv, d_.E, d_.Einv, d_.rho, d_.rho_inv, d_.ctype, d_.x, d_.z, d_.y, d_.dx,
                  d_.dy, d_.xs, d_.xg, d_.xsp, d_.ztg, d_.zt, d_.t0, d_.v, d_.r, d_.uu, d_.p, d_.s, d_.w, d_.t, d_.Minv, d_.uu2, d_.ms, d_.part, d_.res,
                  d_.scal, d_.flags, d_.slot, d_.Praw, d_.Araw, d_.cs, d_.Pi, d_.Pj, d_.Pm1, d_.Pm2, d_.Ai, d_.Aj, d_.AmA, d_.AmB,
                  d_.wb.AL.rowptr, d_.wb.AL.col, d_.wb.AL.blkdesc, d_.wb.AL.runinfo, d_.wb.AL.val, d_.wb.ALT.rowptr, d_.wb.ALT.col, d_.wb.ALT.blkdesc, d_.wb.ALT.runinfo, d_.wb.ALT.val,
                  d_.wb.al_src, d_.wb.alt_src, d_.wb.islong, d_.wb.rows, d_.wb.WT, d_.wb.S, d_.wb.Sinv, d_.wb.g, d_.wb.h, d_.wb.Dinv0, d_.wb.colmap, d_.wb.W, d_.wb.pv, d_.wb.info, d_.wb.dbg, d_.wb.x.tile, d_.wb.x.tile2, d_.wb.x.partG, d_.wb.x.partZ, d_.wb.x.ls0, d_.wb.x.ls1, d_.wb.x.lz0, d_.wb.x.lz1, d_.wb.x.sinvp, d_.wb.x.sc_ptr, d_.wb.x.sc_row, d_.wb.x.sc_src, d_.wb.x.sc_val, d_.wb.x.bjj,
                  d_.ctl, d_.f1.blk, d_.f1.stream, d_.f1.cptr, d_.f1.prp, d_.f1.pcol, d_.f1.psrc, d_.f1.pval, d_.f1.va, d_.f1.fcol, d_.f1.fq, d_.f1.sp_ptr, d_.f1.spk, d_.f1.spill, d_pc_, d_pr_,
                  d_.wb.gjwork, d_.wb.cc, d_.wb.sig, d_.wb.lidx, d_.wb.Ad, d_.wb.ud, d_.wb.ccd, d_.wb.gp, d_.wb.bq_ptr, d_.wb.bq_idx, d_.wb.bq_col, d_.wb.Bd.blkdesc, d_.wb.Bn.blkdesc, d_.wb.As.blkdesc, d_.wb.kind, d_.wb.dcol, d_.wb.srow, d_.wb.ssrc, d_.wb.sval, d_.wb.sg_ptr, d_.wb.sg_col, d_.wb.wv, d_.wb.den, d_.wb.beta, d_.wb.wbeta, d_.wb.rt, d_.wb.uz,
                  d_.kf.K.rowptr, d_.kf.K.col, d_.kf.K.blkdesc, d_.kf.K.runinfo, d_.kf.K.val, d_.kf.tptr, d_.kf.trow, d_.kf.ta, d_.kf.tb, d_.kf.rec};
  for (void *p : ptrs) if (p) be::dfree(d_, p);
  be::destroy(d_);
  d_ = Dev(); d_pc_ = d_pr_ = nullptr;
  dev_ready_ = false;
}

int Engine::validate_settings(const OSQPSettings *s, bool at_setup) {
  if (!s) return OSQP_SETTINGS_VALIDATION_ERROR;
  bool ok = s->device >= 0 && s->scaling >= 0 && s->rho > 0 && s->sigma > 0 && s->alpha > 0 && s->alpha < 2 &&
            s->cg_max_iter > 0 && s->cg_tol_reduction > 0 && s->cg_tol_fraction > 0 && s->cg_tol_fraction < 1 &&
            s->adaptive_rho_interval >= 0 && s->adaptive_rho_fraction > 0 && s->adaptive_rho_tolerance >= 1 &&
// ... 117 lines not shown
  be::set_rho(d_, rho_bar_);
  be::precond(d_, settings.cg_precond == OSQP_DIAGONAL_PRECONDITIONER);
  return OSQP_NO_ERROR;
}

void Engine::upload_bounds_and_types() {
  std::vector<double> ls(m), us(m);
  for (int i = 0; i < m; i++) { ls[i] = E_[i] * l0_[i]; us[i] = E_[i] * u0_[i]; }
  apply_scaled_bounds(ls, us);
}

void Engine::apply_scaled_bounds(const std::vector<double> &ls, const std::vector<double> &us) {
  ls_ = ls; us_ = us;
  classify_constraints(ls, us);
  be::h2d(d_, d_.l, ls.data(), sizeof(double) * m);
  be::h2d(d_, d_.u, us.data(), sizeof(double) * m);
  be::h2d(d_, d_.ctype, ctype_.data(), sizeof(int) * m);
}

void Engine::upload_q() {
  std::vector<double> qs(n);
  for (int j = 0; j < n; j++) qs[j] = c_ * D_[j] * q0_[j];
  be::h2d(d_, d_.q, qs.data(), sizeof(double) * n);
}

void Engine::fill_matrix_values(const std::vector<double> &Px, const std::vector<double> &Ax) {
  std::fill(Bval_.begin(), Bval_.end(), 0.0);
  for (int j = 0; j < n; j++) Bval_[bdiag_[j]] = settings.sigma;
  for (int k = 0; k < P_.nnz(); k++) {
    Bval_[Pmap1_[k]] += Px[k];
    if (Pmap2_[k] >= 0) Bval_[Pmap2_[k]] = Px[k];
  }
  for (int k = 0; k < A_.nnz(); k++) { Aval_[AmapA_[k]] = Ax[k]; Bval_[AmapB_[k]] = Ax[k]; }
  be::h2d(d_, d_.A.val, Aval_.data(), sizeof(double) * Aval_.size());
  be::h2d(d_, d_.B.val, Bval_.data(), sizeof(double) * Bval_.size());
}


void Engine::set_status(int st) {
  info.status_val = st;
  const char *s = "unsolved";
  switch (st) {
    case OSQP_SOLVED: s = "solved"; break;
    case OSQP_SOLVED_INACCURATE: s = "solved inaccurate"; break;
    case OSQP_PRIMAL_INFEASIBLE: s = "primal infeasible"; break;
    case OSQP_PRIMAL_INFEASIBLE_INACCURATE: s = "primal infeasible inaccurate"; break;
    case OSQP_DUAL_INFEASIBLE: s = "dual infeasible"; break;
    case OSQP_DUAL_INFEASIBLE_INACCURATE: s = "dual infeasible inaccurate"; break;
    case OSQP_MAX_ITER_REACHED: s = "maximum iterations reached"; break;
    case OSQP_TIME_LIMIT_REACHED: s = "run time limit reached"; break;
    case OSQP_NON_CVX: s = "problem non convex"; break;
    case OSQP_SIGINT: s = "interrupted"; break;
    default: break;
  }
  std::snprintf(info.status, sizeof(info.status), "%s", s);
}

void Engine::run_chunk(int niter, int budget) {
  const bool fused = be::pcg_fused(d_), wb = d_.wb.on != 0;
  const bool xy = wb && d_.wb.exact && d_.wb.x.on;
  auto enqueue = [&](int count) {
    if (xy) { be::wbx_chunk(d_, count); return; }
    for (int it = 0; it < count; it++) {
      if (be::wbf_active(d_)) { be::wbf_iteration(d_); continue; }
      be::kb_rhs(d_);
      if (wb) be::wb_apply(d_, 0, d_.wb.exact);
      if (wb && d_.wb.exact) { be::ka(d_, budget); continue; }
      for (int i = 0; i < budget; i++) { be::k1(d_, i); be::k2(d_, i); if (!fused || i == budget - 1) { be::kv(d_, i); if (wb) be::wb_apply(d_, (i + 1) & 1); } }
      be::ka(d_, budget);
    }
  };
  stats_.kernel_launches += xy ? ((d_.wb.x.one && !d_.wb.x.slots) ? niter + 1.0 : 2.0 * niter + 1) : (double)niter * ((wb && d_.wb.exact) ? (d_.wb.dual ? 7 : 5) : (fused ? 3 + 2 * budget : 2 + 3 * budget + (wb ? 3 * (budget + 1) : 0)));
  if (!(use_graph_ && be::graphs_supported())) { enqueue(niter); return; }
  constexpr int kMaxGraphNodes = 8192;
  const int per = std::max(1, kMaxGraphNodes / (2 + 3 * budget + (wb ? 3 * (budget + 1) : 0)));
  for (int left = niter; left > 0;) {
    const int cnt = std::min(left, per);
    auto key = std::make_pair(cnt, budget | ((wb && d_.wb.exact) ? (1 << 24) : 0) | (xy ? (1 << 25) : 0) | (be::wbf_active(d_) ? (1 << 26) : 0));
    auto it = graphs_.find(key);
    if (it == graphs_.end()) {
      be::graph_begin(d_);
      enqueue(cnt);
      it = graphs_.emplace(key, be::graph_end(d_)).first;
    }
    be::graph_launch(d_, it->second);
    stats_.graph_launches += 1;
    left -= cnt;
  }
}

void Engine::run_slots(int begin_target, int pairs, int cap) {
  stats_.kernel_launches += 2.0 * pairs + (begin_target > 0 ? 1 : 0);
  if (begin_target > 0) be::slot_begin(d_, begin_target, cap);
  if (!(use_graph_ && be::graphs_supported())) { for (int k = 0; k < pairs; k++) be::slot_pair(d_); return; }
  for (int left = pairs; left > 0;) {
    int unit = 1;
    for (int u : {256, 192, 128, 96, 64, 48, 32, 24, 16, 12, 8, 6, 4, 3, 2}) if (left >= u) { unit = u; break; }
    const std::array<int, 3> key = {unit, 0, 0};
    auto it = sgraphs_.find(key);
    if (it == sgraphs_.end()) {
      be::graph_begin(d_);
      for (int k = 0; k < unit; k++) be::slot_pair(d_);
      it = sgraphs_.emplace(key, be::graph_end(d_)).first;
    }
    be::graph_launch(d_, it->second);
    stats_.graph_launches += 1;
    left -= unit;
  }
}

void Engine::finish(int st) {
  set_status(st);
  if (st == OSQP_NON_CVX) info.obj_val = kNaN;
  else if (term_is_pinf(st)) info.obj_val = OSQP_INFTY;
  else if (term_is_dinf(st)) info.obj_val = -OSQP_INFTY;
}

void Engine::run_stage2(int need, double *res) {
  if (need & NEED_PINF) be::infeas_primal(d_);
  if (need & NEED_DINF) be::infeas_dual(d_, ctl_.inf_thr_d, ctl_.inf_unscaled);
  double r2[R_COUNT]; be::fetch_res(d_, r2);
  for (int q = R_ATDY_U; q <= R_ADX_VIOL; q++) res[q] = r2[q];
}

void Engine::integrate_gap(double t0) {
  const double t = now_s() - t0;
  info.primdual_int += std::fabs(info.duality_gap) * std::max(0.0, t - gap_time_);
  gap_time_ = t;
}

int Engine::solve() {
  if (!dev_ready_) return OSQP_WORKSPACE_NOT_INIT_ERROR;
  be::activate(d_);
  be::ev_mark(d_, 0);
  const int err = solve_impl();
  be::ev_mark(d_, 1);
  stats_.gpu_solve_ms = be::ev_ms(d_);
  return err;
}

int Engine::solve_impl() {
  const double t0 = now_s();
  if (!pol_explicit_) policy_from_env(pol_, true);
  if (clear_update_time_) { info.update_time = 0; }
  info.update_time += update_time_acc_; update_time_acc_ = 0;
  if (!settings.warm_starting) cold_start();
  info.rho_updates = 0; info.status_polish = 0; info.polish_time = 0; info.primdual_int = 0; gap_time_ = 0;
  set_status(OSQP_UNSOLVED);
  if (small_direct_applicable()) {
    const int err = solve_small_direct(t0);
    if (err != OSQP_FUNC_NOT_IMPLEMENTED) return err;
  }
  stats_.pcg_iters_total = stats_.pcg_iters_max = stats_.pcg_unconverged = 0;
  stats_.kernel_launches = stats_.graph_launches = 0; stats_.cg_cap_escalations = 0; stats_.slot_topups = 0;
  stats_.woodbury_factorisations = 0; stats_.woodbury_factor_ms = 0; stats_.woodbury_cache_hits = 0;
  double res[R_COUNT];
  admm_core(t0, res);
  info.rho_estimate = pol_rho_estimate(rho_bar_, res);
  info.solve_time = now_s() - t0;
  if (settings.polishing && info.status_val == OSQP_SOLVED) polish();
  store_solution();
  be::sync(d_);
  info.run_time = (first_run_ ? info.setup_time : info.update_time) + info.solve_time + info.polish_time;
  first_run_ = false; clear_update_time_ = true;
  if (settings.verbose) print_footer();
  return OSQP_NO_ERROR;
}

void Engine::print_footer() const {
  say("\nstatus:               %s\n", info.status);
  if (settings.polishing && info.status_val == OSQP_SOLVED) {
    if (info.status_polish == 1) say("solution polish:      successful\n");
    else if (info.status_polish == -1) say("solution polish:      unsuccessful\n");
  }
  say("number of iterations: %d\n", info.iter);
  if (info.status_val == OSQP_SOLVED || info.status_val == OSQP_SOLVED_INACCURATE) {
    say("optimal objective:    %.4f\n", info.obj_val);
    say("run time:             %.2es\n", info.run_time);
  }
  say("optimal rho estimate: %.2e\n\n", info.rho_estimate);
}

int Engine::has_quad() const {
  for (double v : P_.x) if (v != 0.0) return 1;
  return 0;
}

void Engine::ctl_setup() {
  Ctl &c = ctl_;
  c = Ctl();
  const int ari = settings.adaptive_rho ? auto_rho_interval() : 0;
  c.ct = settings.check_termination; c.ari = ari; c.max_iter = settings.max_iter;
  c.tightW = (ari > 1 && pol_.rho_window > 0) ? std::min(pol_.rho_window, ari - 1) : 0;
  c.tightF = pol_.rho_window_tol; c.persist = pol_.rho_persist; c.tol_exp = pol_.rho_tol_exp;
  c.m = m; c.scaling = settings.scaling; c.scaled_termination = settings.scaled_termination; c.check_dualgap = settings.check_dualgap;
  c.has_quad = has_quad();
  c.esc_on = pol_.cg_escalate; c.stall_on = pol_.stall; c.full_budget = pol_.budget_full; c.cap_max = kMaxCg;
  c.cg_tol_fraction = settings.cg_tol_fraction; c.cg_tol_reduction = settings.cg_tol_reduction; c.rho_tolerance = settings.adaptive_rho_tolerance;
  c.eps_abs = settings.eps_abs; c.eps_rel = settings.eps_rel; c.eps_pinf = settings.eps_prim_inf; c.eps_dinf = settings.eps_dual_inf;
  c.c = c_; c.cinv = cinv_;
  c.budget_tolerate = pol_.budget_tolerate; c.budget_sigma = pol_.budget_sigma; c.budget_slack = pol_.budget_slack; c.budget_min = d_.wb.on ? 1 : 2;
  c.iter = 0; c.cap = std::min(settings.cg_max_iter, kMaxCg);
  c.budget[0] = c.budget[1] = c.cap;
  c.stall = 1.0; c.best_dua = INFINITY; c.prev_aobj = INFINITY; c.rho_bar = rho_bar_;
  c.status = CTL_RUNNING;
}

void Engine::apply_rho(double rho) {
  rho_bar_ = rho; settings.rho = rho;
  be::set_rho(d_, rho_bar_);
  const double tf = d_.wb.on ? now_s() : 0.0;
  struct Tally { Engine *e; double t0; int hits0; ~Tally() { if (t0 > 0) { if (e->d_.wb.cache_hits > hits0) e->stats_.woodbury_cache_hits += 1; else e->stats_.woodbury_factorisations += 1; e->stats_.woodbury_factor_ms += 1e3 * (now_s() - t0); } } } tally{this, tf, d_.wb.cache_hits};
  try { be::precond(d_, settings.cg_precond == OSQP_DIAGONAL_PRECONDITIONER); }
  catch (const DeviceError &err) {
    if (!d_.wb.on) throw;
    std::fprintf(stderr, "osqp_hip: Woodbury correction switched off for this handle at rho = %.3e (%s)\n", rho, err.what());
    d_.wb.on = 0; d_.wb.exact = 0;
    be::sync(d_); drop_graphs();
    be::precond(d_, settings.cg_precond == OSQP_DIAGONAL_PRECONDITIONER);
  }
}

void Engine::info_from_ctl() {
  const Ctl &c = ctl_;
  info.iter = c.iter; info.obj_val = c.obj_val; info.prim_res = c.prim_res; info.dual_res = c.dual_res;
  info.dual_obj_val = c.dual_obj_val; info.duality_gap = c.duality_gap; info.rel_kkt_error = c.rel_kkt_error;
  info.rho_updates = c.rho_updates;
  if (c.rho_estimate > 0) info.rho_estimate = c.rho_estimate;
  rho_at_last_check_ = rho_bar_;
}

void Engine::exec_chunk_sync(int cnt, int lim, bool with_res, int kind, double *res, int *flags) {
  sync_graph_scalars();
  const bool slots = use_slots_ && be::slots_supported(d_);
  if (!slots) {
    run_chunk(cnt, lim);
    if (with_res) { be::residuals(d_); be::fetch_res_flags(d_, res, flags); } else be::fetch_flags(d_, flags);
    return;
  }
  double *pred = slot_pred_;
  int tot[F_COUNT] = {0}, f[F_COUNT];
  int launched_pairs = 0;
  auto pairs_for = [&](double its, double pcg) { return 0.5 * its * be::slot_launches(d_, pcg); };
  const double t_chunk = now_s();
  const int max_pairs = (int)std::ceil(pairs_for(cnt, lim)) + 8;
  if (pol_.slot_poll) {
    const int kLow = pol_.poll_low; const double kFirst = pol_.poll_first, kFrac = pol_.poll_frac, kWait = pol_.poll_wait;
    const double p0 = std::min<double>(pred[kind], lim);
    { const int np = (int)std::ceil(pairs_for(cnt, 0)) + std::max(2, (int)std::floor(kFirst * (pairs_for(cnt, p0) - pairs_for(cnt, 0)))); run_slots(cnt, np, lim); launched_pairs += np; }
    double pair_s = 9e-6, t_prev = now_s();
    int seq_prev = 0;
    for (int seq = 0, done = 0;;) {
      be::slot_poll(d_, &seq, &done);
      if (done >= cnt) break;
      const double t_now = now_s();
      if (t_now - t_chunk > settings.time_limit || launched_pairs > max_pairs) break;
      if (seq - seq_prev >= 8) { pair_s = std::max(5e-6, 2.0 * (t_now - t_prev) / (seq - seq_prev)); t_prev = t_now; seq_prev = seq; }
      const int ahead = launched_pairs - seq / 2;
      if (ahead > kLow) {
        std::this_thread::sleep_for(std::chrono::duration<double>(std::min(2e-3, kWait * (ahead - kLow) * pair_s)));
        continue;
      }
      const int rem = cnt - done;
      const double rate = done > 0 ? std::min<double>(pairs_for(1, lim), (0.5 * seq) / done) : pairs_for(1, p0);
      const int need = (int)std::ceil(rem * rate) + 1 - ahead;
      const bool outrun = done == 0 && launched_pairs > 2 * (int)std::ceil(pairs_for(cnt, p0)) + 8;
      const int np = std::max(std::max(2, need > 12 ? (int)std::ceil(kFrac * need) : need), outrun ? launched_pairs / 4 : 0);
      run_slots(0, np, lim); launched_pairs += np;
      stats_.slot_topups += 1;
    }
  } else {
    const double pm = std::min<double>(pred[kind], lim);
    const int np = (int)std::ceil(pairs_for(cnt, 0) + 1.05 * (pairs_for(cnt, pm) - pairs_for(cnt, 0))) + 2; run_slots(cnt, np, lim); launched_pairs += np;
  }
  for (;;) {
    if (with_res) { be::residuals(d_); be::fetch_res_flags(d_, res, f); } else be::fetch_flags(d_, f);
    tot[F_STAT_SUM] += f[F_STAT_SUM]; tot[F_STAT_SUMSQ] += f[F_STAT_SUMSQ]; tot[F_STAT_N] += f[F_STAT_N]; tot[F_STAT_UNCONV] += f[F_STAT_UNCONV]; tot[F_STAT_STAG] += f[F_STAT_STAG];
    tot[F_STAT_MAX] = std::max(tot[F_STAT_MAX], f[F_STAT_MAX]);
    const int done = be::slot_done(d_);
    if (be::slot_seq(d_) != 2 * launched_pairs) {
      char msg[160];
      std::snprintf(msg, sizeof(msg), "osqp_hip: slot record hand-over broken: %d slots launched, record counts %d", 2 * launched_pairs, be::slot_seq(d_));
      throw DeviceError(msg);
    }
    if (done >= cnt) break;
    if (launched_pairs > max_pairs) throw DeviceError("osqp_hip: a chunk of ADMM iterations does not finish");
    const int rem = cnt - done;
    const double seen = tot[F_STAT_N] > 0 ? (double)tot[F_STAT_SUM] / tot[F_STAT_N] : pred[kind];
    const double pm = std::min<double>(std::max(seen, pred[kind]), lim);
    const int np = std::max((int)std::ceil(pairs_for(rem, 0) + 1.25 * (pairs_for(rem, pm) - pairs_for(rem, 0))) + 8, launched_pairs / 2);
    run_slots(0, np, lim); launched_pairs += np;
    stats_.slot_topups += 1;
  }
  for (int k = 0; k < F_COUNT; k++) flags[k] = tot[k];
  if (pol_.slot_log)
    std::fprintf(stderr, "chunk %p it %d cnt %d kind %d lim %d pred %.2f used-mean %.2f topups %d unconv %d rho %.4e\n", (void *)this, ctl_.iter, cnt, kind, lim, pred[kind],
                 tot[F_STAT_N] > 0 ? (double)tot[F_STAT_SUM] / tot[F_STAT_N] : 0.0, (int)stats_.slot_topups, tot[F_STAT_UNCONV], rho_bar_);
  if (tot[F_STAT_N] > 0) pred[kind] = (double)tot[F_STAT_SUM] / tot[F_STAT_N];
}

static int one_string(int want, int limit) {
  static const int units[] = {2, 3, 4, 6, 8, 12, 16, 24, 32, 48, 64, 96, 128, 192, 256};
  for (int u : units) if (u >= want) return u <= limit ? u : want;
  return want;
}

int Engine::run_device_driven(double t0, double *res, int *flags) {
  Ctl &c = ctl_;
  c.status = CTL_RUNNING; c.chunk_done = 0; c.rho_flag = 0; c.stage2 = 0;
  be::ctl_upload(d_, c);
  be::ctl_begin(d_);
  stats_.kernel_launches += 1;
  const int diagonal = settings.cg_precond == OSQP_DIAGONAL_PRECONDITIONER;
  auto pairs_for = [&](double its, double pcg) { return 0.5 * its * be::slot_launches(d_, pcg); };
  auto pred_for = [&](const Ctl &s, int kind, int tight) {
    const double pm = s.kind_n[kind] > 0 ? s.kind_sum[kind] / s.kind_n[kind] : slot_pred_[kind];
    return std::min<double>(pm, s.budget[tight]);
  };
  Ctl snap = c;
  long launched = 0;
  int seq = 0, done = 0;
  int kLow = pol_.poll_low, kFinish = pol_.finish_pairs;
  double cycle_s = 0.0, pair_s = 22e-6, t_cycle = now_s(), t_rate = t_cycle; long seq_rate = 0;
  bool timed_out = false;
  auto cycle_done = [&]() {
    const double t_now = now_s(), c = t_now - t_cycle;
    cycle_s = cycle_s > 0 ? 0.7 * cycle_s + 0.3 * c : c; t_cycle = t_now;
    kLow = std::min(96, std::max<int>(pol_.poll_low, (int)std::ceil(3.0 * cycle_s / pair_s)));
    kFinish = std::max<int>(pol_.finish_pairs, 2 * kLow);
  };
  bool use_hist = pol_.slot_poll != 0 && !feed_hist_.empty();
  int fed = snap.boundaries;
  long fed_end_seq = 0;
  auto feed_from_history = [&](int upto) {
    while (use_hist && fed < upto) {
      if (fed >= (int)feed_hist_.size()) break;
      if (feed_hist_[fed] <= 0) { use_hist = false; break; }
      const int np = (feed_hist_[fed] + 1) / 2;
      run_slots(0, np, 0); launched += np;
      run_group(diagonal);
      fed += 1; fed_end_seq = 2 * launched;
    }
  };
  if (pol_.slot_log) { std::fprintf(stderr, "feed: history of %zu chunks:", feed_hist_.size()); for (int h : feed_hist_) std::fprintf(stderr, " %d", h); std::fprintf(stderr, "\n"); }
  feed_from_history(snap.boundaries + 2);
  if (!use_hist && launched == 0) {
    const int cnt = snap.ch_next - snap.iter;
    const double full = pairs_for(cnt, pred_for(snap, snap.ch_kind, snap.ch_tight));
    const int np = one_string(std::max(2, (int)std::floor(pol_.poll_first * full)), (int)std::floor(0.95 * full));
    run_slots(0, np, 0); launched += np; }
  for (;;) {
    be::ctl_poll(d_, &snap, &seq, &done);
    print_log(snap, t0);
    if (snap.status != CTL_RUNNING) break;
    if (now_s() - t0 > settings.time_limit) { timed_out = true; break; }
    if (use_hist) {
      if ((snap.boundaries < fed && seq >= fed_end_seq && !snap.chunk_done) || (fed >= (int)feed_hist_.size() && snap.boundaries >= fed)) {
        use_hist = false;
        if (pol_.slot_log) std::fprintf(stderr, "feed: history mode ends: device in chunk %d (iter %d, %d of its iterations done), chunks fed %d, launches executed %d of %ld fed\n", snap.boundaries, snap.iter, done, fed, seq, fed_end_seq);
      }
      else {
        feed_from_history(snap.boundaries + 2);
        if (use_hist) { std::this_thread::sleep_for(std::chrono::microseconds(std::max(pol_.poll_sleep_us, 100))); continue; }
      }
    }
    const long ahead = launched - seq / 2;
    { const double t_now = now_s();
      if (seq - seq_rate >= 16) { pair_s = std::max(5e-6, 2.0 * (t_now - t_rate) / (double)(seq - seq_rate)); t_rate = t_now; seq_rate = seq; } }
    if (ahead > kLow) { std::this_thread::sleep_for(std::chrono::microseconds(pol_.poll_sleep_us)); t_cycle = now_s(); continue; }
    const int cnt = snap.ch_next - snap.iter, rem = std::max(0, cnt - done);
    const double pm = pred_for(snap, snap.ch_kind, snap.ch_tight);
    const double rate = done >= 2 ? std::min<double>(pairs_for(1, snap.budget[snap.ch_tight]), 0.5 * (double)std::max(0, seq - snap.seq_begin) / done) : 1.1 * pairs_for(1, pm);
    const int need = (int)std::ceil(rem * rate) + 2 - (int)ahead;
    if (need > kFinish) {
      const int np = one_string(std::max(2, (int)std::ceil(pol_.poll_frac * need)), need - 2);
      run_slots(0, np, 0); launched += np;
      stats_.slot_topups += 1;
      cycle_done();
      continue;
    }
    const int np = std::max(1, need);
    run_slots(0, np, 0); launched += np;
    run_group(diagonal);
    {
      Ctl nx = snap; nx.iter = snap.ch_next; ctl_next_chunk(nx);
      const int ncnt = nx.ch_next - nx.iter;
      if (ncnt > 0) {
        const double full = pairs_for(ncnt, pred_for(snap, nx.ch_kind, nx.ch_tight));
        const int nq = one_string(std::max(2, (int)std::floor(pol_.poll_first * full)), (int)std::floor(0.95 * full));
        run_slots(0, nq, 0); launched += nq;
      }
    }
    cycle_done();
    if (pol_.slot_log) std::fprintf(stderr, "group: device iter %d chunk %d..%d kind %d done %d rem %d rate %.2f ahead %ld pairs %d (launched %ld, seq %d) budget %d/%d tol %.3e rho %.4e; host cycle %.0f us, pair %.1f us, low-water %d\n",
                                    snap.iter, snap.iter, snap.ch_next, snap.ch_kind, done, rem, rate, ahead, np, launched, seq, snap.budget[0], snap.budget[1], snap.tol_abs, snap.rho_bar, 1e6 * cycle_s, 1e6 * pair_s, kLow);
  }
  be::sync(d_);
  be::ctl_download(d_, &c);
  for (int q = 0; q < R_COUNT; q++) res[q] = c.res[q];
  for (int q = 0; q < F_COUNT; q++) flags[q] = c.last_flags[q];
  for (int k = 0; k < 3; k++) if (c.kind_n[k] > 0) slot_pred_[k] = c.kind_sum[k] / c.kind_n[k];
  feed_hist_.assign(c.hist, c.hist + std::min(std::max(c.boundaries, 0), (int)kCtlHist));
  if (pol_.slot_log) { std::fprintf(stderr, "feed: this solve's chunks consumed:"); for (int h : feed_hist_) std::fprintf(stderr, " %d", h); std::fprintf(stderr, "  (boundaries %d, launches enqueued %ld)\n", c.boundaries, 2 * launched); }
  if (c.rho_bar != rho_bar_) { rho_bar_ = c.rho_bar; settings.rho = rho_bar_; }
  if (timed_out && c.status == CTL_RUNNING) return -2;
  return c.status;
}

void Engine::run_group(int diagonal) {
  stats_.kernel_launches += 11 + (diagonal ? 1 : 0);
  if (!(use_graph_ && be::graphs_supported())) { be::ctl_group(d_, diagonal); return; }
  const std::array<int, 3> key = {0, 1, diagonal};
  auto it = sgraphs_.find(key);
  if (it == sgraphs_.end()) {
    be::graph_begin(d_);
    be::ctl_group(d_, diagonal);
    it = sgraphs_.emplace(key, be::graph_end(d_)).first;
  }
  be::graph_launch(d_, it->second);
  stats_.graph_launches += 1;
}

void Engine::admm_core(double t0, double *res) {
  Ctl &c = ctl_;
  ctl_setup();
  sync_graph_scalars();
  be::zero(d_, d_.flags + F_STAT_SUM, sizeof(int) * (F_COUNT - F_STAT_SUM));
  {
    double r0[R_COUNT];
    be::residuals(d_); be::fetch_res(d_, r0);
    ctl_init_tol(c, r0);
  }
  have_tol_ = false;
  ctl_next_chunk(c);
  log_printed_ = 0;
  if (settings.verbose) say("iter   objective    pri res    dua res    rho       time\n");
  int flags[F_COUNT] = {0};
  for (;;) {
    int st;
    d_.wb.x.slots = (pol_.device_driven >= 2) ? 1 : 0;
    const bool slots = use_slots_ && be::slots_supported(d_);
    const bool device_driven = slots && pol_.device_driven && be::ctl_supported(d_);
    const bool first_chunk = c.iter == 0;
    if (first_chunk || !device_driven) {
      be::set_pcg_tol(d_, c.tol_rel, ctl_chunk_tol_abs(c));
      const bool ckpt_chunk = first_chunk && c.cap < kMaxCg && c.esc_on;
      if (ckpt_chunk) {
        if (!ckpt_) ckpt_ = dev_vec<double>(d_, 2 * (size_t)n + 2 * (size_t)m);
        be::copy_in(d_, ckpt_, d_.x, sizeof(double) * n, 1); be::copy_in(d_, ckpt_ + n, d_.xs, sizeof(double) * n, 1);
        be::copy_in(d_, ckpt_ + 2 * (size_t)n, d_.z, sizeof(double) * m, 1); be::copy_in(d_, ckpt_ + 2 * (size_t)n + m, d_.y, sizeof(double) * m, 1);
      }
      const int lim = c.budget[c.ch_tight], tight = c.ch_tight;
      const double rho_was = rho_bar_;
      exec_chunk_sync(c.ch_next - c.iter, lim, c.ch_at_check && !ckpt_chunk, c.ch_kind, res, flags);
      cg_budget_ = lim;
      if (ckpt_chunk) {
        if (lim >= c.cap && flags[F_STAT_STAG] * 2 > std::max(1, flags[F_STAT_N])) {
          be::copy_in(d_, d_.x, ckpt_, sizeof(double) * n, 1); be::copy_in(d_, d_.xs, ckpt_ + n, sizeof(double) * n, 1);
          be::copy_in(d_, d_.z, ckpt_ + 2 * (size_t)n, sizeof(double) * m, 1); be::copy_in(d_, d_.y, ckpt_ + 2 * (size_t)n + m, sizeof(double) * m, 1);
          be::zero(d_, d_.dx, sizeof(double) * n); be::zero(d_, d_.dy, sizeof(double) * m);
          be::init_iterates(d_, 0);
          c.cap = std::min(kMaxCg, 4 * c.cap); c.budget[0] = c.budget[1] = c.cap;
          c.escalations += 1;
          stats_.kernel_launches = 0; stats_.graph_launches = 0;
          continue;
        }
        if (c.ch_at_check) { be::residuals(d_); be::fetch_res(d_, res); }
      }
      const bool was_check = c.ch_at_check;
      st = ctl_boundary(c, res, flags);
      if (st == CTL_RUNNING && c.stage2) {
        run_stage2(c.stage2, res);
        st = ctl_boundary_stage2(c, res, flags);
      }
      if (was_check) {
        info_from_ctl(); integrate_gap(t0);
        print_log(c, t0);
      }
      (void)tight; (void)rho_was;
      if (st == CTL_RUNNING && c.rho_flag) apply_rho(c.rho_bar);
    } else {
      st = run_device_driven(t0, res, flags);
      info_from_ctl(); integrate_gap(t0);
      print_log(c, t0);
      if (st == -2) { set_status(OSQP_TIME_LIMIT_REACHED); break; }
    }
    if (st == CTL_DONE) { finish(c.osqp_status); break; }
    if (st == CTL_NEED_HOST && (c.need & NEED_REFACTOR)) {
      c.need &= ~NEED_REFACTOR; c.status = CTL_RUNNING;
      d_.wb.exact = 0;
      be::sync(d_); drop_graphs();
      apply_rho(c.rho_bar);
      c.rho_flag = 0;
      continue;
    }
    if (st == CTL_NEED_HOST) {
      int os = ctl_stage1(c, res, true, nullptr, nullptr);
      if (os < 0) { run_stage2(c.need, res); os = ctl_stage2(c, res, true); }
      finish(os > 0 ? os : (int)OSQP_MAX_ITER_REACHED);
      break;
    }
    if (now_s() - t0 > settings.time_limit) { set_status(OSQP_TIME_LIMIT_REACHED); break; }
  }
  if (settings.verbose && info.iter % kCtlPrintInterval != 0) print_summary_line(info.iter, info.obj_val, info.prim_res, info.dual_res, rho_at_last_check_, t0);
  info.rho_updates = c.rho_updates;
  stats_.pcg_iters_total = c.pcg_total; stats_.pcg_iters_max = c.pcg_max; stats_.pcg_unconverged = c.pcg_unconv;
  stats_.cg_cap_escalations = c.escalations;
}

void Engine::recurrence_save(RecurrenceSave &s) const {
  s.stats = stats_; s.rho = rho_bar_; s.alpha = d_.alpha; s.eq_from_cnt = d_.eq_from_cnt; s.eq_factor = d_.rho_eq_factor;
  for (int k = 0; k < 3; k++) s.pred[k] = slot_pred_[k];
}

int Engine::run_recurrence(const RecurrenceRule &rule, double *res) {
  const bool rhs_norm = rule.rhs_norm;
  const int kRecurrenceMaxSteps = rule.max_steps;
  const double gain = rule.gain;
  const double de = std::max(settings.delta, pol_.polish_delta_floor);
  d_.rho_eq_factor = 1.0; d_.eq_from_cnt = 0;
  rho_bar_ = clamp_rho(1.0 / de);
  be::set_rho(d_, rho_bar_);
  be::precond(d_, settings.cg_precond == OSQP_DIAGONAL_PRECONDITIONER);
  be::init_iterates(d_, 0);
  d_.alpha = 1.0; drop_graphs();
  int flags[F_COUNT];
  double best = std::numeric_limits<double>::infinity();
  int worse = 0, steps = 0;
  const int min_steps = 1 + std::max(0, settings.polish_refine_iter);
  for (int s = 0; s < kRecurrenceMaxSteps; s++) {
    be::set_pcg_tol(d_, pol_.polish_pcg_tol, 1e-15);
    exec_chunk_sync(1, kMaxCg, true, 1, res, flags);
    steps = s + 1;
    const double err = rhs_norm ? recurrence_err_rhs(res[R_PRI_S], res[R_DUA_S], res[R_QN_S], res[R_Z_S])
                                : recurrence_err_polish(res[R_PRI_S], res[R_AX_S], res[R_Z_S], res[R_DUA_S], res[R_ATY_S], res[R_PX_S], res[R_QN_S]);
    if (recurrence_ends(err, gain, steps, min_steps, kRecurrenceMaxSteps, &best, &worse)) break;
  }
  return steps;
}

void Engine::recurrence_restore_launch(const RecurrenceSave &s) {
  d_.alpha = s.alpha; drop_graphs();
  for (int k = 0; k < 3; k++) slot_pred_[k] = s.pred[k];
  stats_ = s.stats;
}

void Engine::recurrence_restore_rho(const RecurrenceSave &s) {
  rho_bar_ = s.rho; settings.rho = s.rho;
  d_.eq_from_cnt = s.eq_from_cnt; if (s.eq_from_cnt) d_.rho_eq_factor = s.eq_factor;
  be::set_rho(d_, rho_bar_);
  be::precond(d_, settings.cg_precond == OSQP_DIAGONAL_PRECONDITIONER);
}

void Engine::polish() {
  const double tp = now_s();
  ensure_host_vectors();
  std::vector<double> z(m), y(m);
  be::d2h(d_, z.data(), d_.z, sizeof(double) * m);
  be::d2h(d_, y.data(), d_.y, sizeof(double) * m);
  const OSQPInfo info0 = info;
  RecurrenceSave keep;
  recurrence_save(keep);
  const double rho0 = keep.rho;
  const std::vector<double> ls0 = ls_, us0 = us_, y0 = y, z0 = z;
  std::vector<double> hx(n);
  be::d2h(d_, hx.data(), d_.x, sizeof(double) * n);
  std::vector<double> lp(m), up(m);
  for (int i = 0; i < m; i++) {
    const RowActive act = polish_active(z[i], ls0[i], us0[i], y[i]);
    const bool low = act.low || ctype_[i] == 1, upp = !low && act.upp;
    if (low) { lp[i] = up[i] = ls0[i]; z[i] = ls0[i]; }
    else if (upp) { lp[i] = up[i] = us0[i]; z[i] = us0[i]; }
    else { lp[i] = -OSQP_INFTY; up[i] = OSQP_INFTY; y[i] = 0.0; }
  }
  auto restore = [&]() { recurrence_restore_launch(keep); };
  double res[R_COUNT];
  try {
    apply_scaled_bounds(lp, up);
    be::h2d(d_, d_.z, z.data(), sizeof(double) * m);
    be::h2d(d_, d_.y, y.data(), sizeof(double) * m);
    run_recurrence(RecurrenceRule{false, 0.5, 30}, res);
  } catch (...) {
    restore();
    info = info0; rho_bar_ = rho0; settings.rho = rho0; ls_ = ls0; us_ = us0;
    classify_constraints(ls_, us_);
    throw;
  }
  restore();
  info = info0;
  apply_scaled_bounds(ls0, us0);
  be::init_iterates(d_, 1);
  be::project_normalcone(d_);
  be::residuals(d_); be::fetch_res(d_, res);
  Ctl pol = ctl_;
  ctl_info(pol, res);
  const bool ok = polish_accept(pol.prim_res, pol.dual_res, info0.prim_res, info0.dual_res);
  recurrence_restore_rho(keep);
  if (ok) {
    info.obj_val = pol.obj_val; info.prim_res = pol.prim_res; info.dual_res = pol.dual_res; info.status_polish = 1;
    info.dual_obj_val = pol.dual_obj_val; info.duality_gap = pol.duality_gap; info.rel_kkt_error = pol.rel_kkt_error;
  } else {
    info.status_polish = -1;
    be::h2d(d_, d_.x, hx.data(), sizeof(double) * n);
    be::h2d(d_, d_.y, y0.data(), sizeof(double) * m);
    be::init_iterates(d_, 1);
    be::h2d(d_, d_.z, z0.data(), sizeof(double) * m);
  }
  be::init_iterates(d_, 0);
  info.polish_time = now_s() - tp;
  if (settings.verbose) say("plsh  %11.4e   %8.2e   %8.2e   --------  %8.2es\n", pol.obj_val, pol.prim_res, pol.dual_res,
                            (first_run_ ? info.setup_time : info.update_time) + info.solve_time + info.polish_time);
}

void Engine::store_solution() {
  const int st = info.status_val;
  const bool pinf = term_is_pinf(st), dinf = term_is_dinf(st);
  const bool unsc = settings.scaling && !settings.scaled_termination;
  std::fill(sol_pc_.begin(), sol_pc_.end(), kNaN); std::fill(sol_dc_.begin(), sol_dc_.end(), kNaN);
  if (!pinf && !dinf) {
    be::d2h(d_, sol_x_.data(), d_.x, sizeof(double) * n);
    be::d2h(d_, sol_y_.data(), d_.y, sizeof(double) * m);
    if (settings.scaling) {
      for (int j = 0; j < n; j++) sol_x_[j] *= D_[j];
      for (int i = 0; i < m; i++) sol_y_[i] *= cinv_ * E_[i];
    }
  } else {
    std::fill(sol_x_.begin(), sol_x_.end(), kNaN); std::fill(sol_y_.begin(), sol_y_.end(), kNaN);
    if (pinf) {
      be::d2h(d_, sol_pc_.data(), d_.dy, sizeof(double) * m);
      if (unsc) for (int i = 0; i < m; i++) sol_pc_[i] *= E_[i];
    } else {
      be::d2h(d_, sol_dc_.data(), d_.dx, sizeof(double) * n);
      if (unsc) for (int j = 0; j < n; j++) sol_dc_[j] *= D_[j];
    }
  }
  if (reordered_) {
    std::vector<double> o;
    auto back = [&o](std::vector<double> &v, const std::vector<int> &perm) { o.resize(v.size()); for (size_t k = 0; k < v.size(); k++) o[perm[k]] = v[k]; std::copy(o.begin(), o.end(), v.begin()); };
    back(sol_x_, pc_); back(sol_dc_, pc_); back(sol_y_, pr_); back(sol_pc_, pr_);
  }
}


}
```

### osqp-python_amd/csrc/engine.hpp

```cpp
#pragma once
#include <array>
#include <map>
#include <string>
#include <utility>
#include <vector>

#include "../../include/osqp_hip.h"
#include "backend.h"
#include "policy.h"

namespace osqp_hip {

struct HostCsc {
  int nr = 0, nc = 0;
  std::vector<int> p, i;
  std::vector<double> x;
  int nnz() const { return (int)i.size(); }
};

class Engine {
 public:
  Engine();
  ~Engine();
  int setup(const OSQPCscMatrix *P, const double *q, const OSQPCscMatrix *A, const double *l, const double *u, int m,
// ... 83 lines not shown
  std::vector<double> q0_, l0_, u0_;
  std::vector<double> D_, E_, Dinv_, Einv_; double c_ = 1.0, cinv_ = 1.0;
  std::vector<int> ctype_;
  std::vector<double> ls_, us_;
  std::vector<double> sol_x_, sol_y_, sol_pc_, sol_dc_;
  std::vector<int> Pmap1_, Pmap2_, AmapA_, AmapB_, bdiag_;
  std::vector<double> Aval_, Bval_;
  Dev d_;
  bool dev_ready_ = false;
  double rho_bar_ = 0.1;
  double eq_factor_mixed_ = 10.0;
  bool eq_factor_env_ = false;
  double mixed_eq_factor() const;
  bool eq_factor_set_ = false;
  int cg_budget_ = 0;
  bool first_run_ = true;
  bool have_tol_ = false;
  bool use_graph_ = true;
  std::map<std::pair<int, int>, void *> graphs_;
  double *bbuf_ = nullptr; size_t bbuf_cap_ = 0;
  double *bmat_ = nullptr; size_t bmat_cap_ = 0;
  double *lsw_ = nullptr;
  double ls_rec_[OSQP_HIP_LOCKSTEP_LAST_REC] = {0, 0, 0, 0, 0, 0, 0, 0};
  double *lspw_ = nullptr;
  double ls_pol_rec_[OSQP_HIP_LOCKSTEP_POLISH_LAST_REC] = {0, 0, 0, 0, 0, 0, 0, 0};
  int run_lockstep(int nbatch, const double *q, const double *l, const double *u, double *x, double *y, double *rec, int warm, void *stream,
                   bool mat = false, const double *Px = nullptr, const double *Ax = nullptr);
  double *lsmw_ = nullptr;
  double lsm_rec_[OSQP_HIP_LOCKSTEP_MAT_LAST_REC] = {0, 0, 0, 0, 0, 0, 0, 0};
  int lsm_last_count_ = 0;
  bool lockstep_mat_applies();
  bool wb_k0diag_ = false;
  double *lsdw_ = nullptr, *lsd_vval_ = nullptr;
  int *lsd_vrp_ = nullptr, *lsd_vcol_ = nullptr, *lsd_vsrc_ = nullptr; int lsd_nv_ = 0;
  double lsd_rec_[OSQP_HIP_LOCKSTEP_DIRECT_LAST_REC] = {0, 0, 0, 0, 0, 0, 0, 0};
  bool lockstep_direct_applies();
  int prepare_lockstep_direct_view();
  int run_lockstep_direct(int nbatch, const double *q, const double *l, const double *u, double *x, double *y, double *rec, int warm, void *stream);
  double *lsaw_ = nullptr;
  double *lsabuf_ = nullptr; size_t lsabuf_cap_ = 0;
  int *d_pvmap_ = nullptr, *d_avmap_ = nullptr;
  double lsa_rec_[OSQP_HIP_LOCKSTEP_ADJOINT_LAST_REC] = {0, 0, 0, 0, 0, 0, 0, 0};
  bool lockstep_adjoint_applies();
  int run_lockstep_adjoint(int nbatch, const double *l, const double *u, const double *x, const double *y, const double *dx, const double *dy,
                           double *dP, double *dq, double *dA, double *dl, double *du, double *arec, void *stream);
  double *lsdaw_ = nullptr;
  double *lsdabuf_ = nullptr; size_t lsdabuf_cap_ = 0;
  double lsda_rec_[OSQP_HIP_LOCKSTEP_DIRECT_ADJOINT_LAST_REC] = {0, 0, 0, 0, 0, 0, 0, 0};
  bool lockstep_direct_adjoint_applies();
  int run_lockstep_direct_adjoint(int nbatch, const double *l, const double *u, const double *x, const double *y, const double *dx, const double *dy,
                                  double *dP, double *dq, double *dA, double *dl, double *du, double *arec, void *stream);
  bool batch_applies();
  bool batch_applies_prepared();
  bool lockstep_applies();
  int batch_enter(int nbatch, bool query, const double *x, const double *y, const double *rec, bool (Engine::*applies)());
  struct BatchStage;
  double *abuf_ = nullptr; size_t abuf_cap_ = 0;
  bool adjoint_applicable();
  void fill_adjoint_params(AdjointParams &p, int nbatch);
  std::vector<double> adj_dP_, adj_dA_, adj_dq_, adj_dl_, adj_du_; bool adj_ok_ = false;
  bool adjoint_pcg_applicable() const;
  int adjoint_compute_pcg(const double *x, const double *y, const double *dx, const double *dy);
  double *adjw_ = nullptr; size_t adjw_cap_ = 0;
  double adj_rec_[OSQP_HIP_ADJOINT_LAST_REC] = {0, 0, 0, 0, 0, 0, 0, 0};
  int *d_batch_iters_ = nullptr; int d_batch_iters_n_ = 0;
  std::vector<int> batch_order_; int *d_batch_order_ = nullptr; size_t batch_order_cap_ = 0;
  double *ckpt_ = nullptr;
  std::vector<double> ls_rho_;
  std::vector<int> Arp_, Arj_, Brp_, Bj_;
  struct BatchDirect {
    bool tried = false, ok = false;
    int bw = -1, nents = 0, nprod = 0, ntri = 0;
    int bw_symbolic = -1;
    int *perm = nullptr, *bp_slot = nullptr, *ke_slot = nullptr, *ke_ptr = nullptr, *kp_row = nullptr, *kp_a = nullptr, *kp_b = nullptr, *tri = nullptr;
    double *kp_val = nullptr;
  } bd_;
  void prepare_batch_direct();
  struct BatchWave {
    bool tried = false, ok = false;
    int aend[4] = {0, 0, 0, 0}, tend[2] = {0, 0};
    int *Aidx = nullptr, *Acol = nullptr, *Tidx = nullptr, *Tcol = nullptr, *row = nullptr, *queue = nullptr;
  } bwv_;
  void prepare_batch_wave();
  void free_batch_wave();
  void attach_batch_wave(BatchParams &p, int nbatch);
  int batch_wave_last_ = -1;
  void reserve_batch_order(int nbatch);
  int launch_batch(BatchParams &p, int nbatch, const double *Px, const double *Ax, void *stream, bool wait_solver);
  struct BatchSpectral {
    bool ok = false; int mat_epoch = -1;
    bool failed = false;
    double rho_ref = 0, eqf = 0, sigma = 0; int rho_is_vec = -1;
    std::vector<int> ctype;
    double *V = nullptr, *lam = nullptr; int *d_ctype = nullptr;
    std::vector<double> Vh, lamh;
    double *K0 = nullptr; double k0_rho = 0; bool k0_ok = false;
  } bs_;
  void prepare_batch_k0(double rho0);
  int mat_epoch_ = 0;
  bool prepare_batch_spectral(double rho_ref, double eqf, bool allow_build);
  void free_batch_spectral();
  void prepare_wb(const std::vector<int> &Arp, const std::vector<int> &Arj);
  std::vector<int> wb_kind_;
  void build_wbf_views(const std::vector<int> &rbA, const std::vector<int> &rbB, const std::vector<int> &Arp, const std::vector<int> &Arj, const std::vector<int> &Brp, const std::vector<int> &Bj);
  struct F1Plan {
    bool ok = false; int D = 0, pnnz = 0;
    std::vector<int> blk, prp, pcol, psrc; std::vector<unsigned int> ent; std::vector<unsigned short> cptr;
    int mix = 0; size_t nsp = 0; std::vector<int> fcol, fq, sp_ptr;
  };
  bool reordered_ = false, no_reorder_ = false;
  std::vector<int> pc_, pr_, ipc_, ipr_;
  std::vector<int> PvalMap_, AvalMap_;
  int *d_pc_ = nullptr, *d_pr_ = nullptr;
  double reorder_ms_ = 0;
  bool compute_reorder(const std::vector<int> &Arp, const std::vector<int> &Arj, const std::vector<int> &Brp, const std::vector<int> &Bj);
  void apply_reorder();
  void clear_reorder();
  template <class T> std::vector<T> to_internal_n(const T *v) const { std::vector<T> o(n); for (int j = 0; j < n; j++) o[j] = v[pc_[j]]; return o; }
  template <class T> std::vector<T> to_internal_m(const T *v) const { std::vector<T> o(m); for (int i = 0; i < m; i++) o[i] = v[pr_[i]]; return o; }
  bool plan_f1(const std::vector<int> &rb, const std::vector<int> &Arp, const std::vector<int> &Arj, const std::vector<int> &Brp, const std::vector<int> &Bj, F1Plan &pl);
  void upload_f1(const F1Plan &pl, const std::vector<int> &Arp);
  void prepare_kf(const std::vector<int> &Arp, const std::vector<int> &Arj, const std::vector<int> &Brp, const std::vector<int> &Bj);
  bool small_direct_applicable();
  int solve_small_direct(double t0);
  void attach_batch_direct(BatchParams &p, bool spectral);
  void free_batch_direct();
  OSQPHipStats stats_{};
  double update_time_acc_ = 0;
  bool clear_update_time_ = false;

  void free_all();
  void compute_scaling(std::vector<double> &Px_s, std::vector<double> &Ax_s, std::vector<double> &q_s);
  void scale_matrix_values(std::vector<double> &Px_s, std::vector<double> &Ax_s) const;
  void classify_constraints(const std::vector<double> &l_s, const std::vector<double> &u_s);
  void upload_bounds_and_types();
  void device_scale_vectors(bool q, bool bounds);
  void ensure_host_vectors();
  bool raw_stale_ = false, scaled_stale_ = false;
  void upload_q();
  void fill_matrix_values(const std::vector<double> &Px_s, const std::vector<double> &Ax_s);
  void run_chunk(int niter, int budget);
  void run_slots(int begin_target, int pairs, int cap);
  bool use_slots_ = true;
  double slot_pred_[3] = {6.0, 6.0, 14.0};
  std::map<std::array<int, 3>, void *> sgraphs_;
  void admm_core(double t0, double *res);
  OSQPHipPolicy pol_{};
  bool pol_explicit_ = false;
  Ctl ctl_{};
  int has_quad() const;
  void ctl_setup();
  void apply_rho(double rho);
  void info_from_ctl();
  void exec_chunk_sync(int cnt, int lim, bool with_res, int kind, double *res, int *flags);
  int run_device_driven(double t0, double *res, int *flags);
  void run_group(int diagonal);
  std::vector<int> feed_hist_;
  void polish();
  struct RecurrenceSave { OSQPHipStats stats; double rho, alpha, eq_factor; int eq_from_cnt; double pred[3]; };
  void recurrence_save(RecurrenceSave &s) const;
  struct RecurrenceRule { bool rhs_norm; double gain; int max_steps; };
  int run_recurrence(const RecurrenceRule &rule, double *res);
  void recurrence_restore_launch(const RecurrenceSave &s);
  void recurrence_restore_rho(const RecurrenceSave &s);
  void apply_scaled_bounds(const std::vector<double> &ls, const std::vector<double> &us);
  void drop_graphs();
  double graph_sig_[7] = {0, 0, 0, 0, 0, 0, 0};
  void sync_graph_scalars();
  void run_stage2(int need, double *res);
  void integrate_gap(double t0);
  double gap_time_ = 0;
  void store_solution();
  void set_status(int status);
  void finish(int status);
  int auto_rho_interval() const;
};

}
```

### osqp-python_amd/csrc/hip_common.h

```cpp
#pragma once
#include <hip/hip_runtime.h>

#include <cstdio>
#include <cstdlib>
#include <cstring>
#include <algorithm>
#include <chrono>
#include <type_traits>
#include <vector>
#include <cmath>

#include "../../include/osqp_hip.h"
#include "backend.h"
#include "policy.h"
#include "step_rules.h"

namespace osqp_hip {
namespace be {

#define HIP_CHECK(expr)                                                                                       \
  do {                                                                                                        \
    hipError_t e_ = (expr);                                                                                   \
    if (e_ != hipSuccess) {                                                                                   \
      char msg_[512];                                                                                         \
      std::snprintf(msg_, sizeof(msg_), "osqp_hip: HIP error %s at %s:%d (%s)", hipGetErrorString(e_), __FILE__, __LINE__, #expr); \
      std::fprintf(stderr, "%s\n", msg_);                                                                     \
      throw DeviceError(msg_);                                                                                \
    }                                                                                                         \
  } while (0)

namespace {

#ifdef OSQP_HIP_KTRACE
constexpr int kTraceSlots = 16;
__device__ unsigned long long g_ktrace[kGrid * kTraceSlots];
#define KT(p) do { if (threadIdx.x == 0) g_ktrace[blockIdx.x * kTraceSlots + (p)] = wall_clock64(); } while (0)
#else
#define KT(p) do { } while (0)
#endif
#ifndef OSQP_HIP_KNOCK
#define OSQP_HIP_KNOCK 0
#endif
#define KNOCKED(bit) ((OSQP_HIP_KNOCK & (bit)) != 0)
enum Slot { SL_GAMMA0 = 0, SL_GAMMA1, SL_RN0, SL_RN1, SL_BN, SL_DELTA, SL_DELTA1 , SL_RES0  };
static_assert(SL_RES0 + R_COUNT <= kPartSlots, "Dev::part is too small");

struct Impl {
  hipEvent_t ev0 = nullptr, ev1 = nullptr, ev_ext = nullptr, ev_wait = nullptr;
  hipEvent_t ev_s0 = nullptr, ev_s1 = nullptr;
  bool ext_pending = false;
  double *pin_res = nullptr;
  int *pin_flags = nullptr;
  hipStream_t side = nullptr;
  int *pin_poll = nullptr;
  Ctl *pin_ctl = nullptr, *pin_ctl2 = nullptr;
  int epoch = 0;
  void *blas = nullptr;
  void *dev_block = nullptr; unsigned char *pin_block = nullptr; unsigned char *shadow_block = nullptr;
};
inline Impl &im(Dev &d) { return *static_cast<Impl *>(d.impl); }
inline hipStream_t st(Dev &d) { return static_cast<hipStream_t>(d.stream); }

#if defined(__HIP_DEVICE_COMPILE__)
#define OSQP_GLOBAL_AS __attribute__((address_space(1)))
#else
#define OSQP_GLOBAL_AS
#endif
template <class T> using gp = OSQP_GLOBAL_AS T *;
template <class T> __device__ __forceinline__ gp<T> gptr(T *p) { return (gp<T>)p; }
template <int CTRL, int ROW_MASK = 0xf>
__device__ __forceinline__ double dpp(double v) {
  const int lo = __builtin_amdgcn_update_dpp(0, __double2loint(v), CTRL, ROW_MASK, 0xf, false);
  const int hi = __builtin_amdgcn_update_dpp(0, __double2hiint(v), CTRL, ROW_MASK, 0xf, false);
  return __hiloint2double(hi, lo);
}
constexpr int kReduceLane = 63;
__device__ __forceinline__ double wave_sum(double v) {
  v += dpp<0xb1>(v);
  v += dpp<0x4e>(v);
  v += dpp<0x114>(v);
  v += dpp<0x118>(v);
  v += dpp<0x142, 0xa>(v);
  v += dpp<0x143, 0xc>(v);
  return v;
}
__device__ __forceinline__ double wave_max(double v) {
  v = nanmax(v, dpp<0xb1>(v)); v = nanmax(v, dpp<0x4e>(v)); v = nanmax(v, dpp<0x114>(v)); v = nanmax(v, dpp<0x118>(v));
  v = nanmax(v, dpp<0x142, 0xa>(v)); v = nanmax(v, dpp<0x143, 0xc>(v));
  return v;
}
constexpr int kWaves = kBlock / 64;
__device__ __forceinline__ double sred_sum(const double *s) { double t = 0; for (int w = 0; w < kWaves; w += 2) t += s[w] + s[w + 1]; return t; }
__device__ __forceinline__ double sred_max(const double *s) { double t = s[0]; for (int w = 1; w < kWaves; w++) t = nanmax(t, s[w]); return t; }
__device__ __forceinline__ double block_sum(double v, double *sred) {
  v = wave_sum(v);
  if ((threadIdx.x & 63) == kReduceLane) sred[threadIdx.x >> 6] = v;
  __syncthreads();
  double t = sred_sum(sred);
  __syncthreads();
  return t;
}
__device__ __forceinline__ double block_max(double v, double *sred) {
  v = wave_max(v);
  if ((threadIdx.x & 63) == kReduceLane) sred[threadIdx.x >> 6] = v;
  __syncthreads();
  double t = sred_max(sred);
  __syncthreads();
  return t;
}
__device__ __forceinline__ void block_sum2(double &a, double &b, double *sred) {
  a = wave_sum(a); b = wave_sum(b);
  if ((threadIdx.x & 63) == kReduceLane) { sred[threadIdx.x >> 6] = a; sred[kWaves + (threadIdx.x >> 6)] = b; }
  __syncthreads();
  a = sred_sum(sred); b = sred_sum(sred + kWaves);
  __syncthreads();
}
__device__ __forceinline__ void block_max2(double &a, double &b, double *sred) {
  a = wave_max(a); b = wave_max(b);
  if ((threadIdx.x & 63) == kReduceLane) { sred[threadIdx.x >> 6] = a; sred[kWaves + (threadIdx.x >> 6)] = b; }
  __syncthreads();
  a = sred_max(sred); b = sred_max(sred + kWaves);
  __syncthreads();
}
__device__ __forceinline__ void block_sum_max(double &a, double &b, double *sred) {
  a = wave_sum(a); b = wave_max(b);
  if ((threadIdx.x & 63) == kReduceLane) { sred[threadIdx.x >> 6] = a; sred[kWaves + (threadIdx.x >> 6)] = b; }
  __syncthreads();
  a = sred_sum(sred); b = sred_max(sred + kWaves);
  __syncthreads();
}
constexpr int kPart = kGrid >= kBlock ? kGrid / kBlock : 1;
static_assert(kGrid >= kBlock ? kGrid % kBlock == 0 : kBlock % kGrid == 0, "kGrid and kBlock must divide one another");
static_assert(kWaves % 2 == 0, "block reductions pair the waves");
struct PartRegs { double v[kPart]; };
template <class P>
__device__ __forceinline__ PartRegs partial_load(P slot) {
  PartRegs r;
  if (kPart % 2 == 0) {
    typedef typename std::conditional<std::is_same<P, gp<const double>>::value || std::is_same<P, gp<double>>::value, gp<const double2>, const double2 *>::type P2;
    P2 s2 = (P2)slot + (kPart / 2) * threadIdx.x;
#pragma unroll
    for (int k = 0; k < kPart / 2; k++) { const double2 a = s2[k]; r.v[2 * k] = a.x; r.v[2 * k + 1] = a.y; }
  } else {
    r.v[0] = (kGrid >= kBlock || (int)threadIdx.x < kGrid) ? slot[threadIdx.x] : 0.0;
  }
  return r;
}
__device__ __forceinline__ double partial_fold_sum(const PartRegs &r) { double v = 0; for (int k = 0; k < kPart; k++) v += r.v[k]; return v; }
__device__ __forceinline__ double partial_fold_max(const PartRegs &r) { double v = 0; for (int k = 0; k < kPart; k++) v = nanmax(v, r.v[k]); return v; }
__device__ __forceinline__ double partial_sum(const double *slot, double *sred) { return block_sum(partial_fold_sum(partial_load(slot)), sred); }
__device__ __forceinline__ double partial_max(const double *slot, double *sred) { return block_max(partial_fold_max(partial_load(slot)), sred); }
__device__ __forceinline__ void stw(int wt, double *p, double v) {
  if (wt) __hip_atomic_store(p, v, __ATOMIC_RELAXED, __HIP_MEMORY_SCOPE_AGENT); else *p = v;
}
template <class P>
__device__ __forceinline__ void put_partial(P part, int slot, double v) {
  if (threadIdx.x == 0) part[slot * kGrid + blockIdx.x] = v;
}

template <int NS, int NBUF = (NS == 1 ? 2 : 1)>
struct StreamLds { static constexpr int kBuf = NBUF; static constexpr bool kWin = false; double prod[NBUF][NS][kChunk]; double red[3 * kWaves]; };
template <int NS, class T>
struct StreamLdsW { static constexpr int kBuf = 1; static constexpr bool kWin = true; double prod[1][NS][kChunk]; T win[kWinCap]; double red[3 * kWaves]; };
struct NoPre { [[maybe_unused]] static constexpr int kTraceBase = 0; __device__ __forceinline__ bool operator()() const { return true; } };

__device__ __forceinline__ bool wg_has_rows(const DevCsr &M) {
  const int per = (M.nblk + 7) >> 3;
  const int sl = blockIdx.x >> 3;
  return sl < per && (int)(blockIdx.x & 7) * per + sl < M.nblk;
}
template <class T, class = void> struct has_ops : std::false_type {};
template <class T> struct has_ops<T, std::void_t<typename T::Ops>> : std::true_type {};
template <class T, class = void> struct has_tok : std::false_type {};
template <class T> struct has_tok<T, std::void_t<typename T::Tok>> : std::true_type {};
template <class G, bool = has_ops<G>::value> struct GatherOps {
  struct Ops {};
  static __device__ __forceinline__ Ops fetch(const G &, int) { return Ops(); }
  template <int NS> static __device__ __forceinline__ void prod(const G &g, const Ops &, int c, double a, double (&pr)[NS]) { g(c, a, pr); }
};
template <class G> struct GatherOps<G, true> {
  using Ops = typename G::Ops;
  static __device__ __forceinline__ Ops fetch(const G &g, int c) { return g.fetch(c); }
  template <int NS> static __device__ __forceinline__ void prod(const G &g, const Ops &o, int, double a, double (&pr)[NS]) { g.prod(o, a, pr); }
};
template <class P, bool = has_tok<P>::value> struct PreOps {
  struct Tok {};
  static __device__ __forceinline__ Tok begin(const P &) { return Tok(); }
  static __device__ __forceinline__ bool finish(const P &p, const Tok &) { return p(); }
};
template <class P> struct PreOps<P, true> {
  using Tok = typename P::Tok;
  static __device__ __forceinline__ Tok begin(const P &p) { return p.begin(); }
  static __device__ __forceinline__ bool finish(const P &p, const Tok &t) { return p.finish(t); }
};
template <class T, class = void> struct is_late : std::false_type {};
template <class T> struct is_late<T, std::void_t<decltype(T::kLate)>> : std::bool_constant<T::kLate> {};
template <class P, bool = is_late<P>::value> struct LateOps {
  static __device__ __forceinline__ typename PreOps<P>::Tok begin(const P &) { return typename PreOps<P>::Tok(); }
  template <int NS> static __device__ __forceinline__ bool finish(const P &, const typename PreOps<P>::Tok &, const double (&)[NS], bool) { return true; }
};
template <class P> struct LateOps<P, true> {
  static __device__ __forceinline__ typename P::Tok begin(const P &p) { return p.begin(); }
  template <int NS> static __device__ __forceinline__ bool finish(const P &p, const typename P::Tok &t, const double (&acc)[NS], bool owner) { return p.finish(t, acc, owner); }
};
struct FirstDesc { int4 ds, ws; };
template <bool WIN>
__device__ __forceinline__ FirstDesc first_desc(const DevCsr &M) {
  const int xcd = blockIdx.x & 7, slot0 = blockIdx.x >> 3, per = (M.nblk + 7) >> 3;
  const int b0 = xcd * per + slot0;
  FirstDesc f{make_int4(0, 0, 0, 0), make_int4(0, -1, 0, 0)};
  if (slot0 < per && b0 < M.nblk) {
// ... 281 lines not shown
```

### osqp-python_amd/osqp_amd/_lib.py

```python
import ctypes as C
import os

_HERE = os.path.dirname(os.path.abspath(__file__))
LIB_PATH = os.environ.get('OSQP_HIP_LIBRARY') or os.path.join(_HERE, 'libosqp_hip.so')

c_int_p = C.POINTER(C.c_int)
c_double_p = C.POINTER(C.c_double)


class CscStruct(C.Structure):
    _fields_ = [('m', C.c_int), ('n', C.c_int), ('p', c_int_p), ('i', c_int_p), ('x', c_double_p),
                ('nzmax', C.c_int), ('nz', C.c_int)]


SETTINGS_FIELDS = [
    ('device', C.c_int), ('linsys_solver', C.c_int), ('verbose', C.c_int), ('warm_starting', C.c_int),
    ('scaling', C.c_int), ('polishing', C.c_int), ('rho', C.c_double), ('rho_is_vec', C.c_int),
    ('sigma', C.c_double), ('alpha', C.c_double), ('cg_max_iter', C.c_int), ('cg_tol_reduction', C.c_int),
    ('cg_tol_fraction', C.c_double), ('cg_precond', C.c_int), ('adaptive_rho', C.c_int),
    ('adaptive_rho_interval', C.c_int), ('adaptive_rho_fraction', C.c_double), ('adaptive_rho_tolerance', C.c_double),
    ('max_iter', C.c_int), ('eps_abs', C.c_double), ('eps_rel', C.c_double), ('eps_prim_inf', C.c_double),
    ('eps_dual_inf', C.c_double), ('scaled_termination', C.c_int), ('check_termination', C.c_int),
    ('check_dualgap', C.c_int), ('time_limit', C.c_double), ('delta', C.c_double), ('polish_refine_iter', C.c_int)]


class SettingsStruct(C.Structure):
    _fields_ = SETTINGS_FIELDS


INFO_FIELDS = [
    ('status', C.c_char * 32), ('status_val', C.c_int), ('status_polish', C.c_int), ('obj_val', C.c_double),
    ('dual_obj_val', C.c_double), ('prim_res', C.c_double), ('dual_res', C.c_double), ('duality_gap', C.c_double),
    ('iter', C.c_int), ('rho_updates', C.c_int), ('rho_estimate', C.c_double), ('setup_time', C.c_double),
    ('solve_time', C.c_double), ('update_time', C.c_double), ('polish_time', C.c_double), ('run_time', C.c_double),
    ('primdual_int', C.c_double), ('rel_kkt_error', C.c_double)]


class InfoStruct(C.Structure):
    _fields_ = INFO_FIELDS


class SolutionStruct(C.Structure):
    _fields_ = [('x', c_double_p), ('y', c_double_p), ('prim_inf_cert', c_double_p), ('dual_inf_cert', c_double_p)]


class SolverStruct(C.Structure):
    _fields_ = [('settings', C.POINTER(SettingsStruct)), ('solution', C.POINTER(SolutionStruct)),
                ('info', C.POINTER(InfoStruct)), ('work', C.c_void_p)]


class StatsStruct(C.Structure):
    _fields_ = [(k, C.c_double) for k in ('pcg_iters_total', 'pcg_iters_max', 'pcg_unconverged', 'kernel_launches',
                                          'graph_launches', 'gpu_solve_ms', 'nnzA', 'nnzB', 'pcg_fused', 'batch_direct_bw',
                                          'cg_cap_escalations', 'windowed_blocks', 'row_blocks', 'slot_topups', 'f1_replicas', 'woodbury_rows', 'woodbury_direct', 'preconditioner', 'woodbury_factorisations', 'woodbury_factor_ms', 'reordered', 'reorder_ms', 'woodbury_cache_hits', 'f1_far_columns', 'woodbury_dual_cols', 'woodbury_fused_iteration', 'woodbury_one_launch', 'kform_nnz', 'batch_wave_split')]


class PolicyStruct(C.Structure):
    _fields_ = ([(k, C.c_int) for k in ('graph', 'slots', 'pcg_fused', 'f1', 'window', 'woodbury', 'woodbury_direct', 'woodbury_large', 'device_driven', 'small_direct', 'batch_reorder', 'batch_variant')] +
                [('extrap', C.c_double), ('rho_eq_factor', C.c_double), ('rho_window', C.c_int), ('rho_window_tol', C.c_double), ('rho_persist', C.c_int),
                 ('rho_tol_exp', C.c_double), ('budget_tolerate', C.c_double), ('budget_sigma', C.c_double), ('budget_slack', C.c_int), ('budget_full', C.c_int),
                 ('cg_escalate', C.c_int), ('stall', C.c_int), ('polish_delta_floor', C.c_double), ('polish_pcg_tol', C.c_double), ('slot_poll', C.c_int), ('poll_low', C.c_int), ('poll_first', C.c_double),
                 ('poll_frac', C.c_double), ('poll_wait', C.c_double), ('finish_pairs', C.c_int), ('poll_sleep_us', C.c_int),
                 ('slot_log', C.c_int), ('setup_timing', C.c_int), ('batch_timing', C.c_int), ('woodbury_log', C.c_int), ('woodbury_direct_tol', C.c_double), ('woodbury_fused', C.c_int), ('debug_fail_refactor', C.c_int), ('reorder', C.c_int), ('woodbury_cache', C.c_int), ('kform', C.c_int), ('woodbury_dual', C.c_int), ('woodbury_vendor', C.c_int), ('batch_wave', C.c_int)])


class DenseTestStruct(C.Structure):
    _fields_ = ([(k, C.c_int) for k in ('op', 'M', 'N', 'K')] + [('alpha', C.c_double), ('beta', C.c_double)] +
                [(k, C.c_longlong) for k in ('as_i', 'as_k', 'bs_k', 'bs_j', 'cs_i', 'cs_j', 'a_off', 'b_off', 'c_off', 'a_len', 'b_len', 'c_len')] +
                [('A', c_double_p), ('B', c_double_p), ('C', c_double_p), ('minpiv', C.c_double)])


SolverP = C.POINTER(SolverStruct)


class LinSysStruct(C.Structure):
    pass


LinSysP = C.POINTER(LinSysStruct)
LinSysStruct._fields_ = [
    ('type', C.c_int),
    ('name', C.CFUNCTYPE(C.c_char_p, LinSysP)),
    ('solve', C.CFUNCTYPE(C.c_int, LinSysP, c_double_p, C.c_int)),
    ('update_settings', C.CFUNCTYPE(None, LinSysP, C.POINTER(SettingsStruct))),
    ('warm_start', C.CFUNCTYPE(None, LinSysP, c_double_p)),
    ('adjoint_derivative', C.CFUNCTYPE(C.c_int, LinSysP)),
    ('free', C.CFUNCTYPE(None, LinSysP)),
    ('update_matrices', C.CFUNCTYPE(C.c_int, LinSysP, C.POINTER(CscStruct), c_int_p, C.c_int, C.POINTER(CscStruct), c_int_p, C.c_int)),
    ('update_rho_vec', C.CFUNCTYPE(C.c_int, LinSysP, c_double_p, C.c_double)),
    ('nthreads', C.c_int), ('pcg_iters', C.c_int), ('impl', C.c_void_p)]

PROTOTYPES = {
    'osqp_capabilities': (C.c_int, []),
    'osqp_set_default_settings': (None, [C.POINTER(SettingsStruct)]),
    'osqp_version': (C.c_char_p, []),
    'osqp_setup': (C.c_int, [C.POINTER(SolverP), C.POINTER(CscStruct), c_double_p, C.POINTER(CscStruct), c_double_p,
                             c_double_p, C.c_int, C.c_int, C.POINTER(SettingsStruct)]),
    'osqp_solve': (C.c_int, [SolverP]),
    'osqp_cleanup': (C.c_int, [SolverP]),
    'osqp_warm_start': (C.c_int, [SolverP, c_double_p, c_double_p]),
    'osqp_cold_start': (C.c_int, [SolverP]),
    'osqp_update_data_vec': (C.c_int, [SolverP, c_double_p, c_double_p, c_double_p]),
    'osqp_update_data_mat': (C.c_int, [SolverP, c_double_p, c_int_p, C.c_int, c_double_p, c_int_p, C.c_int]),
    'osqp_update_settings': (C.c_int, [SolverP, C.POINTER(SettingsStruct)]),
    'osqp_update_rho': (C.c_int, [SolverP, C.c_double]),
    'osqp_get_dimensions': (None, [SolverP, c_int_p, c_int_p]),
    'osqp_adjoint_derivative_compute': (C.c_int, [SolverP, c_double_p, c_double_p]),
    'osqp_adjoint_derivative_get_mat': (C.c_int, [SolverP, C.POINTER(CscStruct), C.POINTER(CscStruct)]),
    'osqp_adjoint_derivative_get_vec': (C.c_int, [SolverP, c_double_p, c_double_p, c_double_p]),
    'osqp_codegen': (C.c_int, [SolverP, C.c_char_p, C.c_char_p, C.c_void_p]),
    'osqp_set_default_codegen_defines': (None, [C.c_void_p]),
    'osqp_hip_set_default_print': (None, [C.c_void_p, C.c_void_p]),
    'osqp_hip_set_print': (C.c_int, [SolverP, C.c_void_p, C.c_void_p]),
    'osqp_hip_get_stats': (C.c_int, [SolverP, C.POINTER(StatsStruct)]),
    'osqp_hip_time_kernel': (C.c_int, [SolverP, C.c_int, C.c_int, c_double_p]),
    'osqp_hip_trace_read': (C.c_int, [SolverP, C.POINTER(C.c_ulonglong), C.c_int]),
    'osqp_hip_test_spmv': (C.c_int, [SolverP, C.c_int, c_double_p, c_double_p]),
    'osqp_hip_test_dense': (C.c_int, [SolverP, C.POINTER(DenseTestStruct)]),
    'osqp_hip_set_rho_eq_factor': (C.c_int, [SolverP, C.c_double]),
    'osqp_hip_default_policy': (None, [C.POINTER(PolicyStruct)]),
    'osqp_hip_set_default_policy': (None, [C.POINTER(PolicyStruct)]),
    'osqp_hip_set_policy': (C.c_int, [SolverP, C.POINTER(PolicyStruct)]),
    'osqp_hip_get_policy': (C.c_int, [SolverP, C.POINTER(PolicyStruct)]),
    'osqp_hip_batch_solve': (C.c_int, [SolverP, C.c_int, c_double_p, c_double_p, c_double_p, c_double_p, c_double_p, c_double_p, C.c_int]),
    'osqp_hip_batch_solve_device': (C.c_int, [SolverP, C.c_int, C.c_void_p, C.c_void_p, C.c_void_p, C.c_void_p, C.c_void_p, C.c_void_p, C.c_int, C.c_void_p]),
    'osqp_hip_batch_solve_mat': (C.c_int, [SolverP, C.c_int, c_double_p, c_double_p, c_double_p, c_double_p, c_double_p, c_double_p, c_double_p, c_double_p, C.c_int]),
    'osqp_hip_batch_solve_mat_device': (C.c_int, [SolverP, C.c_int, C.c_void_p, C.c_void_p, C.c_void_p, C.c_void_p, C.c_void_p, C.c_void_p, C.c_void_p, C.c_void_p, C.c_int, C.c_void_p]),
    'osqp_hip_adjoint_compute_at': (C.c_int, [SolverP] + [c_double_p] * 4),
    'osqp_hip_adjoint_last_record': (C.c_int, [SolverP, c_double_p]),
    'osqp_hip_batch_solve_lockstep': (C.c_int, [SolverP, C.c_int, c_double_p, c_double_p, c_double_p, c_double_p, c_double_p, c_double_p, C.c_int]),
    'osqp_hip_batch_solve_lockstep_device': (C.c_int, [SolverP, C.c_int, C.c_void_p, C.c_void_p, C.c_void_p, C.c_void_p, C.c_void_p, C.c_void_p, C.c_int, C.c_void_p]),
    'osqp_hip_lockstep_last_record': (C.c_int, [SolverP, c_double_p]),
    'osqp_hip_lockstep_polish_last_record': (C.c_int, [SolverP, c_double_p]),
    'osqp_hip_batch_solve_lockstep_mat': (C.c_int, [SolverP, C.c_int] + [c_double_p] * 8 + [C.c_int]),
    'osqp_hip_batch_solve_lockstep_mat_device': (C.c_int, [SolverP, C.c_int] + [C.c_void_p] * 8 + [C.c_int, C.c_void_p]),
    'osqp_hip_lockstep_mat_last_record': (C.c_int, [SolverP, c_double_p]),
    'osqp_hip_lockstep_mat_scaling': (C.c_int, [SolverP, C.c_int, c_double_p, c_double_p, c_double_p]),
    'osqp_hip_batch_solve_lockstep_direct': (C.c_int, [SolverP, C.c_int, c_double_p, c_double_p, c_double_p, c_double_p, c_double_p, c_double_p, C.c_int]),
    'osqp_hip_batch_solve_lockstep_direct_device': (C.c_int, [SolverP, C.c_int, C.c_void_p, C.c_void_p, C.c_void_p, C.c_void_p, C.c_void_p, C.c_void_p, C.c_int, C.c_void_p]),
    'osqp_hip_lockstep_direct_last_record': (C.c_int, [SolverP, c_double_p]),
    'osqp_hip_batch_adjoint_lockstep': (C.c_int, [SolverP, C.c_int] + [c_double_p] * 12),
    'osqp_hip_batch_adjoint_lockstep_device': (C.c_int, [SolverP, C.c_int] + [C.c_void_p] * 13),
    'osqp_hip_lockstep_adjoint_last_record': (C.c_int, [SolverP, c_double_p]),
    'osqp_hip_batch_adjoint_lockstep_direct': (C.c_int, [SolverP, C.c_int] + [c_double_p] * 12),
    'osqp_hip_batch_adjoint_lockstep_direct_device': (C.c_int, [SolverP, C.c_int] + [C.c_void_p] * 13),
    'osqp_hip_lockstep_direct_adjoint_last_record': (C.c_int, [SolverP, c_double_p]),
    'osqp_hip_batch_adjoint': (C.c_int, [SolverP, C.c_int] + [c_double_p] * 14),
    'osqp_hip_batch_adjoint_device': (C.c_int, [SolverP, C.c_int] + [C.c_void_p] * 15),
    'osqp_hip_capabilities': (C.c_int, []),
    'osqp_hip_update_data_vec_device': (C.c_int, [SolverP, C.c_void_p, C.c_void_p, C.c_void_p, C.c_void_p]),
    'osqp_hip_warm_start_device': (C.c_int, [SolverP, C.c_void_p, C.c_void_p, C.c_void_p]),
    'osqp_hip_get_scaling': (C.c_int, [SolverP, c_double_p, c_double_p, c_double_p]),
    'osqp_hip_get_reordering': (C.c_int, [SolverP, c_int_p, c_int_p]),
    'osqp_hip_backend': (C.c_char_p, []),
    'osqp_hip_linsys_init': (C.c_int, [C.POINTER(LinSysP), C.POINTER(CscStruct), C.POINTER(CscStruct), c_double_p,
                                       C.POINTER(SettingsStruct), c_double_p, c_double_p, C.c_int]),
}


PRINT_FN = C.CFUNCTYPE(None, C.c_char_p, C.c_void_p)


def _py_print(text, _user):
    import sys
    try:
        sys.stdout.write(text.decode('utf-8', 'replace'))
    except Exception:
        pass


_print_cb = PRINT_FN(_py_print)


def _bind(lib):
    for name, (res, args) in PROTOTYPES.items():
        fn = getattr(lib, name)
        fn.restype = res
        fn.argtypes = args
    lib.osqp_hip_set_default_print(C.cast(_print_cb, C.c_void_p), None)
    return lib


_handle = None


def _preload_torch_hip_runtime():
    import importlib.util
    import sys
    if 'torch' in sys.modules or importlib.util.find_spec('torch') is None:
        return
    import torch


def handle():
    global _handle
    if _handle is None:
        if not os.path.exists(LIB_PATH):
            raise ImportError(
                'libosqp_hip.so not found at %s -- build the HIP engine first (python -c "import __graft_entry__ as g; '
                'g.build()" or make -C osqp-python_amd).  There is no CPU fallback.' % LIB_PATH)
        _preload_torch_hip_runtime()
        _handle = _bind(C.CDLL(LIB_PATH))
    return _handle
```

Measured before the change: 12610.

## Overlap solution export with end of device-driven solve and drop upload syncs

At the end of the device-driven loop, the control block and the x/y solution are copied asynchronously into pinned host buffers, and the host waits on a single event. This replaces a stream sync followed by separate control and solution downloads, and store_solution reuses the exported buffers. The control-block upload no longer blocks the stream; it only waits on an event if the previous upload is still in flight. The first chunk can also replay the recorded slot-pair count, and host-sync and idle-launch counters are added. Risks are stale pinned-buffer reuse and the partial Ctl upload that stops at seq_end.

After: 12670 (median of 6 runs). No clear change (+0.4%).

```diff
diff --git a/include/osqp_hip.h b/include/osqp_hip.h
--- a/include/osqp_hip.h
+++ b/include/osqp_hip.h
@@ -167,6 +167,8 @@
   double woodbury_one_launch;
   double kform_nnz;
   double batch_wave_split;
+  double slot_launches_idle;
+  double host_syncs;
 } OSQPHipStats;
 enum { OSQP_HIP_PRECOND_NONE = 0, OSQP_HIP_PRECOND_JACOBI = 1, OSQP_HIP_PRECOND_JACOBI_WOODBURY = 2, OSQP_HIP_PRECOND_JACOBI_WOODBURY_DENSE = 3 };
 OSQPInt osqp_hip_get_stats(OSQPSolver *solver, OSQPHipStats *out);
@@ -299,6 +301,7 @@
   OSQPInt woodbury_dual;
   OSQPInt woodbury_vendor;
   OSQPInt batch_wave;
+  OSQPInt end_wait;
 } OSQPHipPolicy;
 void    osqp_hip_default_policy(OSQPHipPolicy *policy);
 OSQPInt osqp_hip_set_policy(OSQPSolver *solver, const OSQPHipPolicy *policy);
diff --git a/osqp-python_amd/csrc/backend.h b/osqp-python_amd/csrc/backend.h
--- a/osqp-python_amd/csrc/backend.h
+++ b/osqp-python_amd/csrc/backend.h
@@ -432,6 +432,9 @@
 void ctl_group(Dev &d, int diagonal);
 void ctl_poll(Dev &d, Ctl *out, int *seq, int *done);
 void ctl_download(Dev &d, Ctl *out);
+void sol_export(Dev &d) __attribute__((weak));
+void sol_export_wait(Dev &d, int sleep_us, Ctl *out, const double **x, const double **y) __attribute__((weak));
+long host_syncs(Dev &d) __attribute__((weak));
 constexpr int kSlotInts = 24;
 void slot_poll(Dev &d, int *seq, int *done);
 
diff --git a/osqp-python_amd/csrc/backend_hip.hip b/osqp-python_amd/csrc/backend_hip.hip
--- a/osqp-python_amd/csrc/backend_hip.hip
+++ b/osqp-python_amd/csrc/backend_hip.hip
@@ -1,4 +1,7 @@
 #include "hip_common.h"
+
+#include <cstddef>
+#include <thread>
 
 namespace osqp_hip {
 namespace be {
@@ -318,6 +321,7 @@
 __global__ void k_ctl_begin(Dev d, int epoch) {
   Ctl &c = *d.ctl;
   c.chunk_done = 0; c.rho_flag = 0; c.stage2 = 0; c.status = CTL_RUNNING; c.seq_begin = 0;
+  if (c.boundaries == 1) c.hist[0] = c.seq_end;
   ctl_begin_chunk(d, c, 0);
   d.slot[2 * SR_WORDS] = epoch;
 }
@@ -380,6 +384,8 @@
   HIP_CHECK(hipStreamCreateWithFlags(&p->side, hipStreamNonBlocking));
   HIP_CHECK(hipHostMalloc(reinterpret_cast<void **>(&p->pin_ctl), sizeof(Ctl), hipHostMallocDefault));
   HIP_CHECK(hipHostMalloc(reinterpret_cast<void **>(&p->pin_ctl2), sizeof(Ctl), hipHostMallocDefault));
+  HIP_CHECK(hipHostMalloc(reinterpret_cast<void **>(&p->pin_ctl3), sizeof(Ctl), hipHostMallocDefault));
+  HIP_CHECK(hipEventCreateWithFlags(&p->ev_exp, hipEventDisableTiming | hipEventBlockingSync)); HIP_CHECK(hipEventCreateWithFlags(&p->ev_up, hipEventDisableTiming));
   d.impl = p;
   return OSQP_NO_ERROR;
 }
@@ -389,7 +395,8 @@
   Impl &p = im(d);
   (void)hipEventDestroy(p.ev0); (void)hipEventDestroy(p.ev1); (void)hipEventDestroy(p.ev_s0); (void)hipEventDestroy(p.ev_s1); (void)hipEventDestroy(p.ev_ext); (void)hipEventDestroy(p.ev_wait); (void)hipHostFree(p.pin_res); (void)hipHostFree(p.pin_flags);
   (void)hipHostFree(p.pin_poll); if (p.side) (void)hipStreamDestroy(p.side);
-  (void)hipHostFree(p.pin_ctl); (void)hipHostFree(p.pin_ctl2);
+  (void)hipHostFree(p.pin_ctl); (void)hipHostFree(p.pin_ctl2); (void)hipHostFree(p.pin_ctl3); if (p.pin_sol) (void)hipHostFree(p.pin_sol);
+  (void)hipEventDestroy(p.ev_exp); (void)hipEventDestroy(p.ev_up);
   if (p.blas) wb_release_blas(p.blas);
   batch_release(d);
   for (int k = 1; k < DevWb::kCache; k++) if (d.wb.cache_buf[k]) { (void)hipFree(d.wb.cache_buf[k]); d.wb.cache_buf[k] = nullptr; }
@@ -409,16 +416,16 @@
   if (!b) return;
   HIP_CHECK(hipSetDevice(d.device));
   HIP_CHECK(hipMemcpyAsync(dst, src, b, hipMemcpyHostToDevice, st(d)));
-  HIP_CHECK(hipStreamSynchronize(st(d)));
+  im(d).syncs += 1; HIP_CHECK(hipStreamSynchronize(st(d)));
 }
 void d2h(Dev &d, void *dst, const void *src, size_t b) {
   if (!b) return;
   HIP_CHECK(hipSetDevice(d.device));
   HIP_CHECK(hipMemcpyAsync(dst, src, b, hipMemcpyDeviceToHost, st(d)));
-  HIP_CHECK(hipStreamSynchronize(st(d)));
+  im(d).syncs += 1; HIP_CHECK(hipStreamSynchronize(st(d)));
 }
 void zero(Dev &d, void *dst, size_t b) { if (!b) return; HIP_CHECK(hipSetDevice(d.device)); HIP_CHECK(hipMemsetAsync(dst, 0, b, st(d))); }
-void sync(Dev &d) { HIP_CHECK(hipSetDevice(d.device)); HIP_CHECK(hipStreamSynchronize(st(d))); }
+void sync(Dev &d) { HIP_CHECK(hipSetDevice(d.device)); im(d).syncs += 1; HIP_CHECK(hipStreamSynchronize(st(d))); }
 void ev_mark(Dev &d, int which) { HIP_CHECK(hipSetDevice(d.device)); Impl &p = im(d); HIP_CHECK(hipEventRecord(which ? p.ev_s1 : p.ev_s0, st(d))); }
 double ev_ms(Dev &d) { Impl &p = im(d); float ms = 0.f; HIP_CHECK(hipEventSynchronize(p.ev_s1)); HIP_CHECK(hipEventElapsedTime(&ms, p.ev_s0, p.ev_s1)); return (double)ms; }
 void activate(Dev &d) { HIP_CHECK(hipSetDevice(d.device)); }
@@ -439,11 +446,42 @@
 void ctl_upload(Dev &d, const Ctl &c) {
   HIP_CHECK(hipSetDevice(d.device));
   Impl &p = im(d);
-  std::memcpy(p.pin_ctl, &c, sizeof(Ctl));
-  HIP_CHECK(hipMemcpyAsync(d.ctl, p.pin_ctl, sizeof(Ctl), hipMemcpyHostToDevice, st(d)));
-  HIP_CHECK(hipStreamSynchronize(st(d)));
+  if (p.up_pending && hipEventQuery(p.ev_up) != hipSuccess) { p.syncs += 1; HIP_CHECK(hipEventSynchronize(p.ev_up)); }
+  std::memcpy(p.pin_ctl, &c, offsetof(Ctl, seq_end));
+  HIP_CHECK(hipMemcpyAsync(d.ctl, p.pin_ctl, offsetof(Ctl, seq_end), hipMemcpyHostToDevice, st(d)));
+  HIP_CHECK(hipEventRecord(p.ev_up, st(d)));
+  p.up_pending = true;
 }
 void ctl_begin(Dev &d) { HIP_CHECK(hipSetDevice(d.device)); dev_publish(d); hipLaunchKernelGGL(k_ctl_begin, dim3(1), dim3(1), 0, st(d), d, ++im(d).epoch); }
+void sol_export(Dev &d) {
+  HIP_CHECK(hipSetDevice(d.device));
+  Impl &p = im(d);
+  const size_t need = (size_t)d.n + (size_t)d.m;
+  if (p.pin_sol_doubles < need) {
+    if (p.pin_sol) { HIP_CHECK(hipStreamSynchronize(st(d))); HIP_CHECK(hipHostFree(p.pin_sol)); p.pin_sol = nullptr; p.pin_sol_doubles = 0; }
+    HIP_CHECK(hipHostMalloc(reinterpret_cast<void **>(&p.pin_sol), sizeof(double) * std::max<size_t>(need, 1), hipHostMallocDefault));
+    p.pin_sol_doubles = need;
+  }
+  HIP_CHECK(hipMemcpyAsync(p.pin_ctl3, d.ctl, sizeof(Ctl), hipMemcpyDeviceToHost, st(d)));
+  if (d.n > 0) HIP_CHECK(hipMemcpyAsync(p.pin_sol, d.x, sizeof(double) * d.n, hipMemcpyDeviceToHost, st(d)));
+  if (d.m > 0) HIP_CHECK(hipMemcpyAsync(p.pin_sol + d.n, d.y, sizeof(double) * d.m, hipMemcpyDeviceToHost, st(d)));
+  HIP_CHECK(hipEventRecord(p.ev_exp, st(d)));
+}
+void sol_export_wait(Dev &d, int sleep_us, Ctl *out, const double **x, const double **y) {
+  HIP_CHECK(hipSetDevice(d.device));
+  Impl &p = im(d);
+  p.syncs += 1;
+  if (sleep_us <= 0) HIP_CHECK(hipEventSynchronize(p.ev_exp));
+  else for (;;) {
+    const hipError_t e = hipEventQuery(p.ev_exp);
+    if (e == hipSuccess) break;
+    if (e != hipErrorNotReady) HIP_CHECK(e);
+    std::this_thread::sleep_for(std::chrono::microseconds(sleep_us));
+  }
+  std::memcpy(out, p.pin_ctl3, sizeof(Ctl));
+  *x = p.pin_sol; *y = p.pin_sol + d.n;
+}
+long host_syncs(Dev &d) { return d.impl ? im(d).syncs : 0; }
 void ctl_group(Dev &d, int diagonal) {
   LAUNCH(k_res_m, d, d, 1);
   LAUNCH(k_res_n, d, d, 1);
@@ -476,7 +514,7 @@
   HIP_CHECK(hipSetDevice(d.device));
   Impl &p = im(d);
   HIP_CHECK(hipMemcpyAsync(p.pin_ctl2, d.ctl, sizeof(Ctl), hipMemcpyDeviceToHost, st(d)));
-  HIP_CHECK(hipStreamSynchronize(st(d)));
+  im(d).syncs += 1; HIP_CHECK(hipStreamSynchronize(st(d)));
   std::memcpy(out, p.pin_ctl2, sizeof(Ctl));
 }
 
@@ -500,7 +538,7 @@
 void fetch_res(Dev &d, double *h) {
   HIP_CHECK(hipSetDevice(d.device));
   HIP_CHECK(hipMemcpyAsync(im(d).pin_res, d.res, sizeof(double) * R_COUNT, hipMemcpyDeviceToHost, st(d)));
-  HIP_CHECK(hipStreamSynchronize(st(d)));
+  im(d).syncs += 1; HIP_CHECK(hipStreamSynchronize(st(d)));
   std::memcpy(h, im(d).pin_res, sizeof(double) * R_COUNT);
 }
 void fetch_flags(Dev &d, int *h) {
@@ -508,7 +546,7 @@
   HIP_CHECK(hipMemcpyAsync(im(d).pin_flags, d.flags, sizeof(int) * F_COUNT, hipMemcpyDeviceToHost, st(d)));
   if (d.slot) HIP_CHECK(hipMemcpyAsync(im(d).pin_flags + F_COUNT, d.slot, sizeof(int) * 16, hipMemcpyDeviceToHost, st(d)));
   HIP_CHECK(hipMemsetAsync(d.flags + F_STAT_SUM, 0, sizeof(int) * (F_COUNT - F_STAT_SUM), st(d)));
-  HIP_CHECK(hipStreamSynchronize(st(d)));
+  im(d).syncs += 1; HIP_CHECK(hipStreamSynchronize(st(d)));
   std::memcpy(h, im(d).pin_flags, sizeof(int) * F_COUNT);
 }
 void fetch_res_flags(Dev &d, double *hr, int *hf) {
@@ -517,7 +555,7 @@
   HIP_CHECK(hipMemcpyAsync(im(d).pin_flags, d.flags, sizeof(int) * F_COUNT, hipMemcpyDeviceToHost, st(d)));
   if (d.slot) HIP_CHECK(hipMemcpyAsync(im(d).pin_flags + F_COUNT, d.slot, sizeof(int) * 16, hipMemcpyDeviceToHost, st(d)));
   HIP_CHECK(hipMemsetAsync(d.flags + F_STAT_SUM, 0, sizeof(int) * (F_COUNT - F_STAT_SUM), st(d)));
-  HIP_CHECK(hipStreamSynchronize(st(d)));
+  im(d).syncs += 1; HIP_CHECK(hipStreamSynchronize(st(d)));
   std::memcpy(hr, im(d).pin_res, sizeof(double) * R_COUNT);
   std::memcpy(hf, im(d).pin_flags, sizeof(int) * F_COUNT);
 }
@@ -546,7 +584,7 @@
   if (!bytes) return;
   HIP_CHECK(hipSetDevice(d.device));
   HIP_CHECK(hipMemcpyAsync(dst, src, bytes, src_on_device ? hipMemcpyDeviceToDevice : hipMemcpyHostToDevice, st(d)));
-  if (!src_on_device) HIP_CHECK(hipStreamSynchronize(st(d)));
+  if (!src_on_device) { im(d).syncs += 1; HIP_CHECK(hipStreamSynchronize(st(d))); }
 }
 void stream_wait(Dev &d, void *caller_stream) {
   if (!caller_stream || caller_stream == d.stream) return;
diff --git a/osqp-python_amd/csrc/engine.cpp b/osqp-python_amd/csrc/engine.cpp
--- a/osqp-python_amd/csrc/engine.cpp
+++ b/osqp-python_amd/csrc/engine.cpp
@@ -33,7 +33,7 @@
   real("OSQP_HIP_POLISH_DELTA_FLOOR", p.polish_delta_floor); real("OSQP_HIP_POLISH_PCG_TOL", p.polish_pcg_tol);
   on("OSQP_HIP_SLOT_POLL", p.slot_poll); num("OSQP_HIP_POLL_LOW", p.poll_low); real("OSQP_HIP_POLL_FIRST", p.poll_first);
   real("OSQP_HIP_POLL_FRAC", p.poll_frac); real("OSQP_HIP_POLL_WAIT", p.poll_wait);
-  num("OSQP_HIP_FINISH_PAIRS", p.finish_pairs); num("OSQP_HIP_POLL_SLEEP_US", p.poll_sleep_us);
+  num("OSQP_HIP_FINISH_PAIRS", p.finish_pairs); num("OSQP_HIP_POLL_SLEEP_US", p.poll_sleep_us); num("OSQP_HIP_END_WAIT", p.end_wait);
   if (std::getenv("OSQP_HIP_SLOT_LOG")) p.slot_log = 1;
   if (std::getenv("OSQP_HIP_BATCH_TIMING")) p.batch_timing = 1;
   if (std::getenv("OSQP_HIP_WB_LOG")) p.woodbury_log = 1;
@@ -457,7 +457,9 @@
     if (err != OSQP_FUNC_NOT_IMPLEMENTED) return err;
   }
   stats_.pcg_iters_total = stats_.pcg_iters_max = stats_.pcg_unconverged = 0;
-  stats_.kernel_launches = stats_.graph_launches = 0; stats_.cg_cap_escalations = 0; stats_.slot_topups = 0;
+  stats_.kernel_launches = stats_.graph_launches = 0; stats_.cg_cap_escalations = 0; stats_.slot_topups = 0; stats_.slot_launches_idle = 0;
+  const long syncs0 = be::host_syncs ? be::host_syncs(d_) : 0;
+  sol_ex_x_ = sol_ex_y_ = nullptr;
   stats_.woodbury_factorisations = 0; stats_.woodbury_factor_ms = 0; stats_.woodbury_cache_hits = 0;
   double res[R_COUNT];
   admm_core(t0, res);
@@ -466,6 +468,7 @@
   if (settings.polishing && info.status_val == OSQP_SOLVED) polish();
   store_solution();
   be::sync(d_);
+  stats_.host_syncs = be::host_syncs ? (double)(be::host_syncs(d_) - syncs0) : 0.0;
   info.run_time = (first_run_ ? info.setup_time : info.update_time) + info.solve_time + info.polish_time;
   first_run_ = false; clear_update_time_ = true;
   if (settings.verbose) print_footer();
@@ -535,7 +538,7 @@
   rho_at_last_check_ = rho_bar_;
 }
 
-void Engine::exec_chunk_sync(int cnt, int lim, bool with_res, int kind, double *res, int *flags) {
+void Engine::exec_chunk_sync(int cnt, int lim, bool with_res, int kind, double *res, int *flags, int recorded) {
   sync_graph_scalars();
   const bool slots = use_slots_ && be::slots_supported(d_);
   if (!slots) {
@@ -549,7 +552,9 @@
   auto pairs_for = [&](double its, double pcg) { return 0.5 * its * be::slot_launches(d_, pcg); };
   const double t_chunk = now_s();
   const int max_pairs = (int)std::ceil(pairs_for(cnt, lim)) + 8;
-  if (pol_.slot_poll) {
+  if (pol_.slot_poll && recorded > 0) {
+    const int np = std::min((recorded + 1) / 2, max_pairs); run_slots(cnt, np, lim); launched_pairs += np;
+  } else if (pol_.slot_poll) {
     const int kLow = pol_.poll_low; const double kFirst = pol_.poll_first, kFrac = pol_.poll_frac, kWait = pol_.poll_wait;
     const double p0 = std::min<double>(pred[kind], lim);
     { const int np = (int)std::ceil(pairs_for(cnt, 0)) + std::max(2, (int)std::floor(kFirst * (pairs_for(cnt, p0) - pairs_for(cnt, 0)))); run_slots(cnt, np, lim); launched_pairs += np; }
@@ -598,6 +603,7 @@
     stats_.slot_topups += 1;
   }
   for (int k = 0; k < F_COUNT; k++) flags[k] = tot[k];
+  slot_enq_ += 2L * launched_pairs;
   if (pol_.slot_log)
     std::fprintf(stderr, "chunk %p it %d cnt %d kind %d lim %d pred %.2f used-mean %.2f topups %d unconv %d rho %.4e\n", (void *)this, ctl_.iter, cnt, kind, lim, pred[kind],
                  tot[F_STAT_N] > 0 ? (double)tot[F_STAT_SUM] / tot[F_STAT_N] : 0.0, (int)stats_.slot_topups, tot[F_STAT_UNCONV], rho_bar_);
@@ -635,6 +641,10 @@
     kFinish = std::max<int>(pol_.finish_pairs, 2 * kLow);
   };
   bool use_hist = pol_.slot_poll != 0 && !feed_hist_.empty();
+  const bool can_export = be::sol_export && be::sol_export_wait;
+  bool have_export = false;
+  const double *ex = nullptr, *ey = nullptr;
+  sol_ex_x_ = sol_ex_y_ = nullptr;
   int fed = snap.boundaries;
   long fed_end_seq = 0;
   auto feed_from_history = [&](int upto) {
@@ -655,6 +665,14 @@
     const int np = one_string(std::max(2, (int)std::floor(pol_.poll_first * full)), (int)std::floor(0.95 * full));
     run_slots(0, np, 0); launched += np; }
   for (;;) {
+    if (use_hist && can_export && fed >= (int)feed_hist_.size()) {
+      be::sol_export(d_);
+      be::sol_export_wait(d_, pol_.end_wait > 0 ? std::max(pol_.poll_sleep_us, 1) : 0, &snap, &ex, &ey);
+      print_log(snap, t0);
+      if (snap.status != CTL_RUNNING) { have_export = true; break; }
+      use_hist = false;
+      if (pol_.slot_log) std::fprintf(stderr, "feed: history mode ends behind the record: device in chunk %d (iter %d), chunks fed %d\n", snap.boundaries, snap.iter, fed);
+    }
     be::ctl_poll(d_, &snap, &seq, &done);
     print_log(snap, t0);
     if (snap.status != CTL_RUNNING) break;
@@ -700,8 +718,13 @@
     if (pol_.slot_log) std::fprintf(stderr, "group: device iter %d chunk %d..%d kind %d done %d rem %d rate %.2f ahead %ld pairs %d (launched %ld, seq %d) budget %d/%d tol %.3e rho %.4e; host cycle %.0f us, pair %.1f us, low-water %d\n",
                                     snap.iter, snap.iter, snap.ch_next, snap.ch_kind, done, rem, rate, ahead, np, launched, seq, snap.budget[0], snap.budget[1], snap.tol_abs, snap.rho_bar, 1e6 * cycle_s, 1e6 * pair_s, kLow);
   }
-  be::sync(d_);
-  be::ctl_download(d_, &c);
+  if (have_export) c = snap;
+  else if (can_export) { be::sol_export(d_); be::sol_export_wait(d_, pol_.end_wait > 0 ? std::max(pol_.poll_sleep_us, 1) : 0, &c, &ex, &ey); }
+  else { be::sync(d_); be::ctl_download(d_, &c); }
+  if (c.status == CTL_DONE) { sol_ex_x_ = ex; sol_ex_y_ = ey; }
+  slot_enq_ += 2 * launched;
+  { long used = 0; for (int k = 0; k < std::min(std::max(c.boundaries, 0), (int)kCtlHist); k++) used += c.hist[k];
+    stats_.slot_launches_idle = (double)std::max(0L, slot_enq_ - used); }
   for (int q = 0; q < R_COUNT; q++) res[q] = c.res[q];
   for (int q = 0; q < F_COUNT; q++) flags[q] = c.last_flags[q];
   for (int k = 0; k < 3; k++) if (c.kind_n[k] > 0) slot_pred_[k] = c.kind_sum[k] / c.kind_n[k];
@@ -731,6 +754,8 @@
   ctl_setup();
   sync_graph_scalars();
   be::zero(d_, d_.flags + F_STAT_SUM, sizeof(int) * (F_COUNT - F_STAT_SUM));
+  if (d_.ctl) be::zero(d_, reinterpret_cast<char *>(d_.ctl) + offsetof(Ctl, seq_end), sizeof(int));
+  slot_enq_ = 0; sol_ex_x_ = sol_ex_y_ = nullptr;
   {
     double r0[R_COUNT];
     be::residuals(d_); be::fetch_res(d_, r0);
@@ -757,7 +782,8 @@
       }
       const int lim = c.budget[c.ch_tight], tight = c.ch_tight;
       const double rho_was = rho_bar_;
-      exec_chunk_sync(c.ch_next - c.iter, lim, c.ch_at_check && !ckpt_chunk, c.ch_kind, res, flags);
+      const int recorded = (first_chunk && device_driven && c.escalations == 0 && !feed_hist_.empty()) ? feed_hist_[0] : 0;
+      exec_chunk_sync(c.ch_next - c.iter, lim, c.ch_at_check && !ckpt_chunk, c.ch_kind, res, flags, recorded);
       cg_budget_ = lim;
       if (ckpt_chunk) {
         if (lim >= c.cap && flags[F_STAT_STAG] * 2 > std::max(1, flags[F_STAT_N])) {
@@ -767,7 +793,7 @@
           be::init_iterates(d_, 0);
           c.cap = std::min(kMaxCg, 4 * c.cap); c.budget[0] = c.budget[1] = c.cap;
           c.escalations += 1;
-          stats_.kernel_launches = 0; stats_.graph_launches = 0;
+          stats_.kernel_launches = 0; stats_.graph_launches = 0; slot_enq_ = 0;
           continue;
         }
         if (c.ch_at_check) { be::residuals(d_); be::fetch_res(d_, res); }
@@ -859,6 +885,7 @@
 
 void Engine::polish() {
   const double tp = now_s();
+  sol_ex_x_ = sol_ex_y_ = nullptr;
   ensure_host_vectors();
   std::vector<double> z(m), y(m);
   be::d2h(d_, z.data(), d_.z, sizeof(double) * m);
@@ -922,7 +949,13 @@
   const bool pinf = term_is_pinf(st), dinf = term_is_dinf(st);
   const bool unsc = settings.scaling && !settings.scaled_termination;
   std::fill(sol_pc_.begin(), sol_pc_.end(), kNaN); std::fill(sol_dc_.begin(), sol_dc_.end(), kNaN);
-  if (!pinf && !dinf) {
+  if (!pinf && !dinf && sol_ex_x_ && sol_ex_y_) {
+    const double *ex = sol_ex_x_, *ey = sol_ex_y_;
+    if (settings.scaling) {
+      for (int j = 0; j < n; j++) sol_x_[j] = ex[j] * D_[j];
+      for (int i = 0; i < m; i++) sol_y_[i] = ey[i] * (cinv_ * E_[i]);
+    } else { std::copy(ex, ex + n, sol_x_.begin()); std::copy(ey, ey + m, sol_y_.begin()); }
+  } else if (!pinf && !dinf) {
     be::d2h(d_, sol_x_.data(), d_.x, sizeof(double) * n);
     be::d2h(d_, sol_y_.data(), d_.y, sizeof(double) * m);
     if (settings.scaling) {
@@ -939,6 +972,7 @@
       if (unsc) for (int j = 0; j < n; j++) sol_dc_[j] *= D_[j];
     }
   }
+  sol_ex_x_ = sol_ex_y_ = nullptr;
   if (reordered_) {
     std::vector<double> o;
     auto back = [&o](std::vector<double> &v, const std::vector<int> &perm) { o.resize(v.size()); for (size_t k = 0; k < v.size(); k++) o[perm[k]] = v[k]; std::copy(o.begin(), o.end(), v.begin()); };
diff --git a/osqp-python_amd/csrc/engine.hpp b/osqp-python_amd/csrc/engine.hpp
--- a/osqp-python_amd/csrc/engine.hpp
+++ b/osqp-python_amd/csrc/engine.hpp
@@ -259,9 +259,11 @@
   void ctl_setup();
   void apply_rho(double rho);
   void info_from_ctl();
-  void exec_chunk_sync(int cnt, int lim, bool with_res, int kind, double *res, int *flags);
+  void exec_chunk_sync(int cnt, int lim, bool with_res, int kind, double *res, int *flags, int recorded = 0);
   int run_device_driven(double t0, double *res, int *flags);
   void run_group(int diagonal);
+  long slot_enq_ = 0;
+  const double *sol_ex_x_ = nullptr, *sol_ex_y_ = nullptr;
   std::vector<int> feed_hist_;
   void polish();
   struct RecurrenceSave { OSQPHipStats stats; double rho, alpha, eq_factor; int eq_from_cnt; double pred[3]; };
diff --git a/osqp-python_amd/csrc/hip_common.h b/osqp-python_amd/csrc/hip_common.h
--- a/osqp-python_amd/csrc/hip_common.h
+++ b/osqp-python_amd/csrc/hip_common.h
@@ -57,6 +57,10 @@
   int epoch = 0;
   void *blas = nullptr;
   void *dev_block = nullptr; unsigned char *pin_block = nullptr; unsigned char *shadow_block = nullptr;
+  Ctl *pin_ctl3 = nullptr; double *pin_sol = nullptr; size_t pin_sol_doubles = 0;
+  hipEvent_t ev_exp = nullptr, ev_up = nullptr;
+  bool up_pending = false;
+  long syncs = 0;
 };
 inline Impl &im(Dev &d) { return *static_cast<Impl *>(d.impl); }
 inline hipStream_t st(Dev &d) { return static_cast<hipStream_t>(d.stream); }
diff --git a/osqp-python_amd/osqp_amd/_lib.py b/osqp-python_amd/osqp_amd/_lib.py
--- a/osqp-python_amd/osqp_amd/_lib.py
+++ b/osqp-python_amd/osqp_amd/_lib.py
@@ -52,7 +52,7 @@
 class StatsStruct(C.Structure):
     _fields_ = [(k, C.c_double) for k in ('pcg_iters_total', 'pcg_iters_max', 'pcg_unconverged', 'kernel_launches',
                                           'graph_launches', 'gpu_solve_ms', 'nnzA', 'nnzB', 'pcg_fused', 'batch_direct_bw',
-                                          'cg_cap_escalations', 'windowed_blocks', 'row_blocks', 'slot_topups', 'f1_replicas', 'woodbury_rows', 'woodbury_direct', 'preconditioner', 'woodbury_factorisations', 'woodbury_factor_ms', 'reordered', 'reorder_ms', 'woodbury_cache_hits', 'f1_far_columns', 'woodbury_dual_cols', 'woodbury_fused_iteration', 'woodbury_one_launch', 'kform_nnz', 'batch_wave_split')]
+                                          'cg_cap_escalations', 'windowed_blocks', 'row_blocks', 'slot_topups', 'f1_replicas', 'woodbury_rows', 'woodbury_direct', 'preconditioner', 'woodbury_factorisations', 'woodbury_factor_ms', 'reordered', 'reorder_ms', 'woodbury_cache_hits', 'f1_far_columns', 'woodbury_dual_cols', 'woodbury_fused_iteration', 'woodbury_one_launch', 'kform_nnz', 'batch_wave_split', 'slot_launches_idle', 'host_syncs')]
 
 
 class PolicyStruct(C.Structure):
@@ -61,7 +61,7 @@
                  ('rho_tol_exp', C.c_double), ('budget_tolerate', C.c_double), ('budget_sigma', C.c_double), ('budget_slack', C.c_int), ('budget_full', C.c_int),
                  ('cg_escalate', C.c_int), ('stall', C.c_int), ('polish_delta_floor', C.c_double), ('polish_pcg_tol', C.c_double), ('slot_poll', C.c_int), ('poll_low', C.c_int), ('poll_first', C.c_double),
                  ('poll_frac', C.c_double), ('poll_wait', C.c_double), ('finish_pairs', C.c_int), ('poll_sleep_us', C.c_int),
-                 ('slot_log', C.c_int), ('setup_timing', C.c_int), ('batch_timing', C.c_int), ('woodbury_log', C.c_int), ('woodbury_direct_tol', C.c_double), ('woodbury_fused', C.c_int), ('debug_fail_refactor', C.c_int), ('reorder', C.c_int), ('woodbury_cache', C.c_int), ('kform', C.c_int), ('woodbury_dual', C.c_int), ('woodbury_vendor', C.c_int), ('batch_wave', C.c_int)])
+                 ('slot_log', C.c_int), ('setup_timing', C.c_int), ('batch_timing', C.c_int), ('woodbury_log', C.c_int), ('woodbury_direct_tol', C.c_double), ('woodbury_fused', C.c_int), ('debug_fail_refactor', C.c_int), ('reorder', C.c_int), ('woodbury_cache', C.c_int), ('kform', C.c_int), ('woodbury_dual', C.c_int), ('woodbury_vendor', C.c_int), ('batch_wave', C.c_int), ('end_wait', C.c_int)])
 
 
 class DenseTestStruct(C.Structure):
```
